# siyi-wind/MDViT

Measured on AMD Instinct MI355X. Metric: 512x512 images/sec MDViT train step (fwd+bwd, two-sweep, AdamW), higher is better.
Workload: dtype bf16x3 (fp32 storage; GEMM operands split hi+lo bf16, fp32 accumulate); 1 GPU; MDViT Sup+MLPFM train step, 4 domain(s) x bs=4 per GPU, 512x512, drop_rate=0.1 drop_path=0.1, bf16x3 GEMMs, data-parallel x1

## Files before the change

include/mdvit_hip.h:

```cpp
#ifndef MDVIT_HIP_H
#define MDVIT_HIP_H

#include <stddef.h>
#include <stdint.h>

#ifdef __cplusplus
extern "C" {
#endif

#define MDVIT_ABI_VERSION 1

enum {
    MDVIT_OK = 0,
    MDVIT_E_SHAPE = 1,
    MDVIT_E_DTYPE = 2,
    MDVIT_E_ALIGN = 3,
    MDVIT_E_WORKSPACE = 4,
    MDVIT_E_HIP = 5
};

enum { MDVIT_EPI_NONE = 0, MDVIT_EPI_GELU_DUAL = 1, MDVIT_EPI_DGELU = 2 };
enum { MDVIT_ACT_NONE = 0, MDVIT_ACT_HSWISH = 1, MDVIT_ACT_RELU = 2 };

const char* mdvit_last_error(void);
int mdvit_version(void);

int mdvit_event_create(void** out_event);
int mdvit_event_destroy(void* event);
int mdvit_event_elapsed_ms(void* start_event, void* stop_event, float* ms);
int mdvit_timing_arm(void* start_event, void* stop_event);

size_t mdvit_partials_ws_bytes(int32_t n_outputs);

typedef struct MdvitGemmDesc {
    const float* A; const float* B; float* C; float* C2;
    int64_t lda, ldb, ldc;
    int32_t M, N, K;
    int32_t trans_a, trans_b;
    const float* bias;
    int32_t epi;
    float e_drop_p; uint32_t e_key0, e_key1;
    const float* e_rowscale; int32_t e_rows_per_scale;
    const float* residual; int64_t ldr;
    const float* gelu_u; int64_t ldu;
    int32_t allow_split;
    void* ws; uint64_t ws_bytes;
    int32_t accumulate;
    float* colsum_a;
    int32_t precision;
    const uint32_t* drop_seed;
    const float* rc_a; int64_t rc_lda; const float* rc_b; int64_t rc_ldb; const float* rc_bias; int32_t rc_k;
    int32_t conv_c, conv_h, conv_w, conv_ho, conv_wo, conv_stride, conv_dilation;
    int32_t conv_up;
    int32_t a_bf16, b_bf16;
    int32_t conv_wgrad_nchw;
} MdvitGemmDesc;
size_t mdvit_gemm_ws_bytes(const MdvitGemmDesc* desc);
#define MDVIT_GEMM_MAX_GROUPS 8
int mdvit_gemm_f32_grouped(const MdvitGemmDesc* desc, int32_t G, const void* const* A, const void* const* B, void* const* C, void* stream);
int mdvit_gemm_f32_grouped_bias(const MdvitGemmDesc* desc, int32_t G, const void* const* A, const void* const* B, void* const* C, const void* const* bias, void* stream);
int mdvit_compose_bias(int32_t n, const void* const* W, int64_t ldw, const void* const* b, void* const* out, int32_t rows, int32_t cols, void* stream);
int mdvit_compose_bias_bwd(int32_t n, const void* const* W, int64_t ldw, const void* const* b, const void* const* dout, void* const* dW, int64_t lddw,
                           void* const* db, int32_t db_accumulate, int32_t rows, int32_t cols, void* stream);
int mdvit_gemm_plan(const MdvitGemmDesc* desc, int32_t* tile_m, int32_t* tile_n, int32_t* splits);
int mdvit_transpose_f32(const float* in, int64_t ld_in, float* out, int32_t rows, int32_t cols, void* stream);
int mdvit_transpose_batch(int32_t n, const void* const* in, const int64_t* ld_in, void* const* out, const int32_t* rows, const int32_t* cols, void* stream);
int mdvit_transpose_many(const void* items_dev, int32_t n, int32_t blocks_per_item, void* stream);
int mdvit_gemm_force_plan(int32_t cfg, int32_t splits);
int mdvit_gemm_kernel_name(const MdvitGemmDesc* d, char* out, int32_t cap);
int mdvit_gemm_tn_config(int32_t enable, int32_t cfg, int32_t splits);
int mdvit_gemm_tn_grid_order(int32_t mode);
int mdvit_gemm_f32(const MdvitGemmDesc* desc, void* stream);
int mdvit_conv_weight_relayout(const float* w, float* out, int32_t Cout, int32_t Cin, int32_t mode, void* stream);
int mdvit_conv_weight_relayout_many(const void* items_dev, int32_t n, int32_t blocks_per_item, void* stream);

typedef struct MdvitPlaneGemmDesc {
    const void* A; int64_t lda; int64_t a_plane; int32_t a_f32;
    const void* B; int64_t ldb; int64_t b_plane;
    int32_t planes;
    int32_t trans;
    int32_t M, N, K;
    float* C; int64_t ldc;
    void* Cp; int64_t ldcp; int64_t c_plane;
    float* U; int64_t ldu_out;
    const float* bias;
    int32_t epi;
    float e_drop_p; uint32_t e_key0, e_key1;
    const float* e_rowscale; int32_t e_rows_per_scale;
    const float* residual; int64_t ldr;
    const float* gelu_u; int64_t ldu;
    const void* rc_a; int64_t rc_lda; int64_t rc_a_plane; const void* rc_b; int64_t rc_ldb; int64_t rc_b_plane; const float* rc_bias; int32_t rc_k;
    int32_t allow_split; void* ws; uint64_t ws_bytes;
    int32_t accumulate;
    const uint32_t* drop_seed;
} MdvitPlaneGemmDesc;
size_t mdvit_gemm_planes_ws_bytes(const MdvitPlaneGemmDesc* desc);
int mdvit_gemm_planes_plan(const MdvitPlaneGemmDesc* desc, int32_t* tile_m, int32_t* tile_n, int32_t* splits);
int mdvit_gemm_planes_force_plan(int32_t cfg, int32_t splits);
int mdvit_gemm_planes(const MdvitPlaneGemmDesc* desc, void* stream);
int mdvit_gemm_ph_prefers(int32_t M, int32_t N, int32_t K, int32_t planes);
int mdvit_gemm_ph_prefers_epi(int32_t M, int32_t N, int32_t K, int32_t planes, int32_t epi_reads);
int mdvit_gemm_ph_config(int32_t mode);
int mdvit_gemm_pm_prefers(int32_t M, int32_t N, int32_t K, int32_t planes, int32_t a_f32);
int mdvit_gemm_pm_config(int32_t mode);
int mdvit_gemm_pm_splits(int32_t M, int32_t N, int32_t K, int32_t planes, int32_t a_f32);
int mdvit_split_planes(const float* in, int64_t ld_in, void* out, int64_t ld_out, int64_t plane_stride, int64_t rows, int32_t cols, int32_t planes, void* stream);
int mdvit_split_planes_t(const float* in, int64_t ld_in, void* out, int64_t ld_out, int64_t plane_stride, int32_t rows, int32_t cols, int32_t transpose,
                         int32_t planes, void* stream);
int mdvit_split_planes_many(const void* items_dev, int32_t n, int32_t blocks_per_item, int32_t planes, void* stream);

int mdvit_mlp_fwd_f32(const float* x, const float* W1, const float* b1, const float* W2, const float* b2, const float* res,
                      const float* rowscale , int32_t rows_per_scale, float* h, float* y, int32_t M, int32_t C, int32_t hidden,
                      float drop_p, uint32_t key1_0, uint32_t key1_1, uint32_t key2_0, uint32_t key2_1, const uint32_t* drop_seed, void* stream);

int mdvit_mlp_config(int32_t wide_min_tokens, int32_t ablate);

int mdvit_mlp_bwd_dgrad_f32(const float* gm, const float* x, const float* W1, const float* b1, const float* W2t, const float* W1t,
                            float* du , float* dx, int32_t M, int32_t C, int32_t hidden, float drop_p,
                            uint32_t key1_0, uint32_t key1_1, const uint32_t* drop_seed, void* stream);

int mdvit_mlp_rc_fwd(const float* x, const void* W1p, const float* b1, const void* W2p, const float* b2, const float* res,
                     const float* rowscale , int32_t rows_per_scale, float* y, int32_t M, int32_t C, int32_t hidden,
                     float drop_p, uint32_t key1_0, uint32_t key1_1, uint32_t key2_0, uint32_t key2_1, const uint32_t* drop_seed, void* stream);
int mdvit_mlp_rc_dgrad(const float* gm, const float* x, const void* W1p, const float* b1, const void* W2tp, const void* W1tp, float* dx,
                       int32_t M, int32_t C, int32_t hidden, float drop_p, uint32_t key1_0, uint32_t key1_1, const uint32_t* drop_seed, void* stream);
int mdvit_linear_rc(const float* x, int64_t lda, const void* Wp, int64_t wplane, const float* bias, float* y, int64_t ldc, int32_t M, int32_t N, int32_t K,
                    float drop_p, uint32_t key0, uint32_t key1, const float* rowscale, int32_t rows_per_scale, const float* residual, int64_t ldr,
                    const uint32_t* drop_seed, void* stream);
int mdvit_linear_rc_ln(const float* x, const float* gamma, const float* beta, int32_t groups, float eps, float* mean, float* rstd, float* ln_out,
                       const void* Wp, int64_t wplane, const float* bias, float* y, int64_t ldc, int32_t M, int32_t N, int32_t K, void* stream);
int mdvit_mlp_rc16_fwd(const float* x, const void* W1p, const float* b1, const void* W2p, const float* b2, const float* res, const float* rowscale,
                       int32_t rows_per_scale, float* h, float* y, int32_t M, int32_t C, int32_t Hd, float drop_p, uint32_t key1_0, uint32_t key1_1,
                       uint32_t key2_0, uint32_t key2_1, const uint32_t* drop_seed, void* stream);
int mdvit_mlp_rc_fwd_ln(const float* x2, const float* gamma, const float* beta, int32_t groups, float eps, float* mean, float* rstd, float* ln_out,
                        const void* W1p, const float* b1, const void* W2p, const float* b2, const float* rowscale, int32_t rows_per_scale, float* h, float* y,
                        int32_t M, int32_t C, int32_t Hd, float drop_p, uint32_t key1_0, uint32_t key1_1, uint32_t key2_0, uint32_t key2_1,
                        const uint32_t* drop_seed, void* stream);
int mdvit_mlp_rc16_dgrad(const float* gm, const float* x, const void* W1p, const float* b1, const void* W2tp, const void* W1tp, float* du, float* dx,
                         int32_t M, int32_t C, int32_t Hd, float drop_p, uint32_t key1_0, uint32_t key1_1, const uint32_t* drop_seed, void* stream);
int mdvit_mlp_rc16_fwd_hbf16(const float* x, const void* W1p, const float* b1, const void* W2p, const float* b2, const float* res, const float* rowscale,
                             int32_t rows_per_scale, float* h, float* y, int32_t M, int32_t C, int32_t Hd, float drop_p, uint32_t key1_0, uint32_t key1_1,
                             uint32_t key2_0, uint32_t key2_1, const uint32_t* drop_seed, void* stream);
int mdvit_mlp_rc_fwd_ln_hbf16(const float* x2, const float* gamma, const float* beta, int32_t groups, float eps, float* mean, float* rstd, float* ln_out,
                              const void* W1p, const float* b1, const void* W2p, const float* b2, const float* rowscale, int32_t rows_per_scale, float* h, float* y,
                              int32_t M, int32_t C, int32_t Hd, float drop_p, uint32_t key1_0, uint32_t key1_1, uint32_t key2_0, uint32_t key2_1,
                              const uint32_t* drop_seed, void* stream);
int mdvit_mlp_rc16_dgrad_hbf16(const float* gm, const float* x, const void* W1p, const float* b1, const void* W2tp, const void* W1tp, float* du, float* dx,
                               int32_t M, int32_t C, int32_t Hd, float drop_p, uint32_t key1_0, uint32_t key1_1, const uint32_t* drop_seed, void* stream);
int mdvit_mlp_rc_bwd(const float* gm, const float* x, const void* W1p, const float* b1, const void* W2tp, const void* W1tp, float* dx_parts, float* dW1, float* db1,
                     float* dW2, void* ws, size_t ws_bytes, int32_t M, int32_t C, int32_t hidden, float drop_p, uint32_t key1_0, uint32_t key1_1,
                     const uint32_t* drop_seed, int32_t accumulate, void* stream);
size_t mdvit_mlp_rc_wgrad_ws_bytes(int32_t M, int32_t C, int32_t hidden);
int mdvit_gemm_ledger(int32_t enable);
int mdvit_gemm_ledger_read(int32_t index, char* name, int32_t cap, int64_t* launches, double* flop, double* bytes);
int mdvit_gemm_sampler(const char* symbol, int32_t stride);
int mdvit_gemm_sampler_read(int32_t index, char* name, int32_t cap, int64_t* seen, int64_t* timed, double* ms);
int mdvit_mlp_rc_config(int32_t fwd_variant);
int mdvit_mlp_rc_planes(int32_t planes);
int mdvit_block_config(int32_t mlp_bwd_fused);
int mdvit_mlp_rc_wgrad(const float* gm, const float* x, const void* W1p, const float* b1, const void* W2tp, float* dW1, float* db1, float* dW2,
                       void* ws, size_t ws_bytes, int32_t M, int32_t C, int32_t hidden, float drop_p, uint32_t key1_0, uint32_t key1_1,
                       const uint32_t* drop_seed, int32_t accumulate, void* stream);

typedef struct MdvitBlockDesc {
    int32_t B, H, W, C, heads, hidden, s3, s5, s7, ln_groups, D, da_hidden, precision;
    float eps, drop_p;
    uint32_t key_proj[2], key_fc1[2], key_fc2[2];
    const uint32_t* drop_seed;
    const float* rowscale1; const float* rowscale2;
    const float* label;
    const float *cpe_w, *cpe_b, *n1_g, *n1_b, *qkv_w, *qkv_b, *w3, *b3, *w5, *b5, *w7, *b7, *da_w1, *da_b1, *da_w2, *da_b2, *proj_w, *proj_b, *n2_g, *n2_b, *fc1_w, *fc1_b,
        *fc2_w, *fc2_b;
    const float *qkv_wt, *proj_wt, *fc1_wt, *fc2_wt;
    const void *fc1_p, *fc2_p, *fc2t_p, *fc1t_p;
    const void *qkv_p, *proj_p, *projt_p, *qkvt_p;
    int32_t store_bf16;
    const float* a_pre;
    int32_t attn_kind;
} MdvitBlockDesc;
typedef struct MdvitBlockGrads {
    float *cpe_w, *cpe_b, *n1_g, *n1_b, *qkv_w, *qkv_b, *w3, *b3, *w5, *b5, *w7, *b7, *da_w1, *da_b1, *da_w2, *da_b2, *proj_w, *proj_b, *n2_g, *n2_b, *fc1_w, *fc1_b, *fc2_w,
        *fc2_b;
    int32_t accumulate, dgrad_only, aux_first;
    int32_t ln_accumulate;
    float* e_out;
} MdvitBlockGrads;
typedef struct MdvitBlockStreams {
    void* main; void* side;
    void** events; int32_t n_events; int32_t* next_event;
} MdvitBlockStreams;
size_t mdvit_block_save_bytes(const MdvitBlockDesc* d);
size_t mdvit_block_fwd_ws_bytes(const MdvitBlockDesc* d);
int mdvit_block_fwd(const MdvitBlockDesc* d, const float* x, float* y, void* save, size_t save_bytes, void* ws, size_t ws_bytes, void* stream);
size_t mdvit_block_bwd_ws_bytes(const MdvitBlockDesc* d, const MdvitBlockGrads* g, int32_t with_side_stream, size_t* side_bytes);
int mdvit_block_bwd(const MdvitBlockDesc* d, const MdvitBlockGrads* g, const MdvitBlockStreams* st, const float* x, const void* save, size_t save_bytes,
                    const float* dy, float* dx , void* ws, size_t ws_bytes, void* ws_side, size_t ws_side_bytes);

int mdvit_rowdot_fwd(const float* x, int64_t ldx, const float* w, const float* b, float* y,
                     int32_t M, int32_t K, int32_t accumulate, void* stream);
int mdvit_rowdot_bwd(const float* x, int64_t ldx, const float* w, const float* dy, float* dx, int64_t lddx,
                     float* dw, float* db, void* ws , size_t ws_bytes, int32_t M, int32_t K, void* stream);

int mdvit_colsum_f32(const float* A, int64_t lda, float* out, float* masked, void* ws , size_t ws_bytes, int32_t M, int32_t N,
                     float drop_p, uint32_t key0, uint32_t key1, const float* rowscale, int32_t rows_per_scale,
                     int32_t accumulate, const uint32_t* drop_seed, void* stream);

int mdvit_layernorm_fwd(const float* x, const float* gamma, const float* beta, float* y, float* mean, float* rstd,
                        int32_t M, int32_t C, int32_t groups, float eps, void* stream);
int mdvit_layernorm_bwd(const float* dy, const float* x, const float* gamma, const float* mean, const float* rstd,
                        const float* add, float* dx, float* dgamma, float* dbeta, void* ws , size_t ws_bytes,
                        int32_t M, int32_t C, int32_t groups, void* stream);
int mdvit_layernorm_bwd_masked(const float* dy, const float* x, const float* gamma, const float* mean, const float* rstd, const float* add, float* dx,
                               float* dx_masked, float* dgamma, float* dbeta, void* ws, size_t ws_bytes, int32_t M, int32_t C, int32_t groups,
                               float drop_p, uint32_t key0, uint32_t key1, const float* rowscale, int32_t rows_per_scale, const uint32_t* seed, void* stream);

int mdvit_dwconv3x3_fwd(const float* x, const float* w, const float* bias, float* y,
                        int32_t B, int32_t Hi, int32_t Wi, int32_t C, int32_t stride, int32_t add_input, void* stream);
int mdvit_dwconv3x3_bwd(const float* dy, const float* x, const float* w, float* dx, float* dw, float* dbias,
                        void* ws , size_t ws_bytes,
                        int32_t B, int32_t Hi, int32_t Wi, int32_t C, int32_t stride, int32_t add_input,
                        int32_t accumulate , void* stream);
int mdvit_gconv2_3x3_fwd(const float* skip, const float* up, const float* w, float* y,
                         int32_t B, int32_t H, int32_t W, int32_t C, void* stream);
int mdvit_gconv2_3x3_bwd(const float* dy, const float* skip, const float* up, const float* w,
                         float* dskip, float* dup, float* dw, void* ws , size_t ws_bytes,
                         int32_t B, int32_t H, int32_t W, int32_t C, int32_t accumulate , void* stream);
int mdvit_im2col3x3(const float* x, float* col, int32_t B, int32_t Hi, int32_t Wi, int32_t Cin, int32_t stride, int32_t dilation, void* stream);
int mdvit_col2im3x3(const float* dcol, float* dx, int32_t B, int32_t Hi, int32_t Wi, int32_t Cin, int32_t stride, int32_t dilation, void* stream);
int mdvit_dropout_f32(const float* x, float* y, int64_t n, float p, uint32_t key0, uint32_t key1, const uint32_t* drop_seed, void* stream);
int mdvit_stemconv_fwd(const float* img, const float* w, float* y, int32_t B, int32_t H, int32_t W, int32_t Cin, int32_t Cout, void* stream);
int mdvit_stemconv_wgrad(const float* img, const float* dy, float* dw, void* ws , size_t ws_bytes,
                         int32_t B, int32_t H, int32_t W, int32_t Cin, int32_t Cout, int32_t accumulate , void* stream);

size_t mdvit_bn_ws_bytes(int32_t M, int32_t C, int32_t groups);
int mdvit_bn_stats(const float* y, void* ws, size_t ws_bytes, float* mean, float* rstd, float* running_mean, float* running_var,
                   int64_t* num_batches_tracked, int32_t M, int32_t C, int32_t groups, int32_t per_group_affine, float eps,
                   float momentum, void* stream);
int mdvit_bn_eval_prep(const float* running_mean, const float* running_var, float* mean, float* rstd, int32_t C, float eps, void* stream);
int mdvit_bn_apply(const float* y, const float* mean, const float* rstd, const float* gamma, const float* beta, float* z,
                   int32_t M, int32_t C, int32_t groups, int32_t per_group_affine, int32_t act, float drop2d_p, uint32_t key0,
                   uint32_t key1, const uint32_t* drop_seed, int32_t rows_per_sample, void* stream);
int mdvit_bn_bwd(const float* dz, const float* y, const float* mean, const float* rstd, const float* gamma, const float* beta,
// ... 144 lines not shown
```

mdvit_amd/_lib.py:

```python
from __future__ import annotations

import ctypes as C
import os
import re
from typing import List

_HERE = os.path.dirname(os.path.abspath(__file__))
LIB_PATH = os.environ.get("MDVIT_HIP_LIB") or os.path.join(_HERE, "lib", "libmdvit_hip.so")
HEADER_PATH = os.path.join(_HERE, "..", "include", "mdvit_hip.h")

EPI_NONE, EPI_GELU_DUAL, EPI_DGELU = 0, 1, 2
ACT_NONE, ACT_HSWISH, ACT_RELU = 0, 1, 2

f32p = C.c_void_p
vp = C.c_void_p
i32 = C.c_int32
i64 = C.c_int64
u32 = C.c_uint32
f32 = C.c_float


class GemmDesc(C.Structure):
    _fields_ = [
        ("A", vp), ("B", vp), ("C", vp), ("C2", vp),
        ("lda", i64), ("ldb", i64), ("ldc", i64),
        ("M", i32), ("N", i32), ("K", i32),
        ("trans_a", i32), ("trans_b", i32),
        ("bias", vp),
        ("epi", i32),
        ("e_drop_p", f32), ("e_key0", u32), ("e_key1", u32),
        ("e_rowscale", vp), ("e_rows_per_scale", i32),
        ("residual", vp), ("ldr", i64),
        ("gelu_u", vp), ("ldu", i64),
        ("allow_split", i32),
        ("ws", vp), ("ws_bytes", C.c_uint64),
        ("accumulate", i32),
        ("colsum_a", vp),
        ("precision", i32),
        ("drop_seed", vp),
        ("rc_a", vp), ("rc_lda", i64), ("rc_b", vp), ("rc_ldb", i64), ("rc_bias", vp), ("rc_k", i32),
        ("conv_c", i32), ("conv_h", i32), ("conv_w", i32), ("conv_ho", i32), ("conv_wo", i32), ("conv_stride", i32), ("conv_dilation", i32),
        ("conv_up", i32),
        ("a_bf16", i32), ("b_bf16", i32), ("conv_wgrad_nchw", i32),
    ]


class PlaneGemmDesc(C.Structure):
    _fields_ = [
        ("A", vp), ("lda", i64), ("a_plane", i64), ("a_f32", i32),
        ("B", vp), ("ldb", i64), ("b_plane", i64),
        ("planes", i32), ("trans", i32),
        ("M", i32), ("N", i32), ("K", i32),
        ("C", vp), ("ldc", i64),
        ("Cp", vp), ("ldcp", i64), ("c_plane", i64),
        ("U", vp), ("ldu_out", i64),
        ("bias", vp),
        ("epi", i32),
        ("e_drop_p", f32), ("e_key0", u32), ("e_key1", u32),
        ("e_rowscale", vp), ("e_rows_per_scale", i32),
        ("residual", vp), ("ldr", i64),
        ("gelu_u", vp), ("ldu", i64),
        ("rc_a", vp), ("rc_lda", i64), ("rc_a_plane", i64), ("rc_b", vp), ("rc_ldb", i64), ("rc_b_plane", i64), ("rc_bias", vp), ("rc_k", i32),
        ("allow_split", i32), ("ws", vp), ("ws_bytes", C.c_uint64),
        ("accumulate", i32),
        ("drop_seed", vp),
    ]


class BlockDesc(C.Structure):
    _fields_ = ([(n, i32) for n in ("B", "H", "W", "C", "heads", "hidden", "s3", "s5", "s7", "ln_groups", "D", "da_hidden", "precision")]
                + [("eps", f32), ("drop_p", f32), ("key_proj", u32 * 2), ("key_fc1", u32 * 2), ("key_fc2", u32 * 2), ("drop_seed", vp),
                   ("rowscale1", vp), ("rowscale2", vp), ("label", vp)]
                + [(n, vp) for n in ("cpe_w", "cpe_b", "n1_g", "n1_b", "qkv_w", "qkv_b", "w3", "b3", "w5", "b5", "w7", "b7", "da_w1", "da_b1", "da_w2", "da_b2",
                                     "proj_w", "proj_b", "n2_g", "n2_b", "fc1_w", "fc1_b", "fc2_w", "fc2_b")]
                + [(n, vp) for n in ("qkv_wt", "proj_wt", "fc1_wt", "fc2_wt", "fc1_p", "fc2_p", "fc2t_p", "fc1t_p", "qkv_p", "proj_p", "projt_p", "qkvt_p")]
                + [("store_bf16", i32), ("a_pre", vp), ("attn_kind", i32)])


BLOCK_PARAMS = ("cpe_w", "cpe_b", "n1_g", "n1_b", "qkv_w", "qkv_b", "w3", "b3", "w5", "b5", "w7", "b7", "da_w1", "da_b1", "da_w2", "da_b2",
                "proj_w", "proj_b", "n2_g", "n2_b", "fc1_w", "fc1_b", "fc2_w", "fc2_b")


DA_MANY_MAX = 32


class DaMany(C.Structure):
    _fields_ = [("n", i32), ("hid", i32 * DA_MANY_MAX), ("C", i32 * DA_MANY_MAX), ("heads", i32 * DA_MANY_MAX), ("W1", vp * DA_MANY_MAX), ("b1", vp * DA_MANY_MAX),
                ("W2", vp * DA_MANY_MAX), ("b2", vp * DA_MANY_MAX), ("a", vp * DA_MANY_MAX)]


class DaManyGrads(C.Structure):
    _fields_ = [("e", vp * DA_MANY_MAX), ("dW1", vp * DA_MANY_MAX), ("db1", vp * DA_MANY_MAX), ("dW2", vp * DA_MANY_MAX), ("db2", vp * DA_MANY_MAX)]


class BlockGrads(C.Structure):
    _fields_ = [(n, vp) for n in BLOCK_PARAMS] + [("accumulate", i32), ("dgrad_only", i32), ("aux_first", i32), ("ln_accumulate", i32), ("e_out", vp)]


class SeAdapterDesc(C.Structure):
    _fields_ = [("kind", i32), ("B", i32), ("N", i32), ("C", i32), ("r", i32), ("W1", vp), ("b1", vp), ("W2", vp), ("b2", vp), ("Wg", vp), ("bg", vp)]


SE_DASE, SE_USE = 0, 1


class BlockStreams(C.Structure):
    _fields_ = [("main", vp), ("side", vp), ("events", C.POINTER(vp)), ("n_events", i32), ("next_event", C.POINTER(i32))]


_SIGS = {
    "mdvit_block_fwd": [C.POINTER(BlockDesc), vp, vp, vp, C.c_size_t, vp, C.c_size_t, vp],
    "mdvit_block_bwd": [C.POINTER(BlockDesc), C.POINTER(BlockGrads), C.POINTER(BlockStreams), vp, vp, C.c_size_t, vp, vp, vp, C.c_size_t, vp, C.c_size_t],
    "mdvit_gemm_planes": [C.POINTER(PlaneGemmDesc), vp],
    "mdvit_gemm_planes_plan": [C.POINTER(PlaneGemmDesc), C.POINTER(i32), C.POINTER(i32), C.POINTER(i32)],
    "mdvit_gemm_planes_force_plan": [i32, i32],
    "mdvit_gemm_ph_config": [i32],
    "mdvit_gemm_pm_config": [i32],
    "mdvit_da_fwd_many": [C.POINTER(DaMany), vp, i32, i32, vp],
    "mdvit_da_bwd_many": [C.POINTER(DaMany), C.POINTER(DaManyGrads), vp, f32, vp, C.c_size_t, i32, i32, vp],
    "mdvit_gemm_pm_prefers": [i32, i32, i32, i32, i32],
    "mdvit_gemm_pm_splits": [i32, i32, i32, i32, i32],
    "mdvit_gemm_f32_grouped": [C.POINTER(GemmDesc), i32, C.POINTER(vp), C.POINTER(vp), C.POINTER(vp), vp],
    "mdvit_gemm_f32_grouped_bias": [C.POINTER(GemmDesc), i32, C.POINTER(vp), C.POINTER(vp), C.POINTER(vp), C.POINTER(vp), vp],
    "mdvit_transpose_batch": [i32, C.POINTER(vp), C.POINTER(i64), C.POINTER(vp), C.POINTER(i32), C.POINTER(i32), vp],
    "mdvit_compose_bias": [i32, C.POINTER(vp), i64, C.POINTER(vp), C.POINTER(vp), i32, i32, vp],
    "mdvit_compose_bias_bwd": [i32, C.POINTER(vp), i64, C.POINTER(vp), C.POINTER(vp), C.POINTER(vp), i64, C.POINTER(vp), i32, i32, i32, vp],
    "mdvit_gemm_ph_prefers": [i32, i32, i32, i32],
    "mdvit_gemm_ph_prefers_epi": [i32, i32, i32, i32, i32],
    "mdvit_mlp_config": [i32, i32],
    "mdvit_mlp_rc_config": [i32],
    "mdvit_mlp_rc_planes": [i32],
    "mdvit_block_config": [i32],
    "mdvit_gemm_ledger": [i32],
    "mdvit_gemm_ledger_read": [i32, C.c_char_p, i32, C.POINTER(i64), C.POINTER(C.c_double), C.POINTER(C.c_double)],
    "mdvit_gemm_sampler": [C.c_char_p, i32],
    "mdvit_gemm_sampler_read": [i32, C.c_char_p, i32, C.POINTER(i64), C.POINTER(i64), C.POINTER(C.c_double)],
    "mdvit_mlp_rc_fwd": [vp, vp, vp, vp, vp, vp, vp, i32, vp, i32, i32, i32, f32, u32, u32, u32, u32, vp, vp],
    "mdvit_linear_rc": [vp, i64, vp, i64, vp, vp, i64, i32, i32, i32, f32, u32, u32, vp, i32, vp, i64, vp, vp],
    "mdvit_linear_rc_ln": [vp, vp, vp, i32, f32, vp, vp, vp, vp, i64, vp, vp, i64, i32, i32, i32, vp],
    "mdvit_mlp_rc_fwd_ln": [vp, vp, vp, i32, f32, vp, vp, vp, vp, vp, vp, vp, vp, i32, vp, vp, i32, i32, i32, f32, u32, u32, u32, u32, vp, vp],
    "mdvit_mlp_rc16_fwd": [vp, vp, vp, vp, vp, vp, vp, i32, vp, vp, i32, i32, i32, f32, u32, u32, u32, u32, vp, vp],
    "mdvit_mlp_rc_dgrad": [vp, vp, vp, vp, vp, vp, vp, i32, i32, i32, f32, u32, u32, vp, vp],
    "mdvit_mlp_rc16_dgrad": [vp, vp, vp, vp, vp, vp, vp, vp, i32, i32, i32, f32, u32, u32, vp, vp],
    "mdvit_mlp_rc_fwd_ln_hbf16": [vp, vp, vp, i32, f32, vp, vp, vp, vp, vp, vp, vp, vp, i32, vp, vp, i32, i32, i32, f32, u32, u32, u32, u32, vp, vp],
    "mdvit_mlp_rc16_fwd_hbf16": [vp, vp, vp, vp, vp, vp, vp, i32, vp, vp, i32, i32, i32, f32, u32, u32, u32, u32, vp, vp],
    "mdvit_mlp_rc16_dgrad_hbf16": [vp, vp, vp, vp, vp, vp, vp, vp, i32, i32, i32, f32, u32, u32, vp, vp],
    "mdvit_mlp_rc_wgrad": [vp, vp, vp, vp, vp, vp, vp, vp, vp, C.c_size_t, i32, i32, i32, f32, u32, u32, vp, i32, vp],
    "mdvit_mlp_rc_bwd": [vp, vp, vp, vp, vp, vp, vp, vp, vp, vp, vp, C.c_size_t, i32, i32, i32, f32, u32, u32, vp, i32, vp],
    "mdvit_imgconv_fwd": [vp, vp, vp, i32, i32, i32, i32, i32, i32, vp],
    "mdvit_imgconv_wgrad": [vp, vp, vp, vp, C.c_size_t, i32, i32, i32, i32, i32, i32, i32, vp],
    "mdvit_maxpool3x3s2_fwd": [vp, vp, vp, i32, i32, i32, i32, vp],
    "mdvit_maxpool3x3s2_bwd": [vp, vp, vp, i32, i32, i32, i32, vp],
    "mdvit_resize_ac_fwd": [vp, vp, i32, i32, i32, i32, i32, i32, vp],
    "mdvit_resize_ac_bwd": [vp, vp, i32, i32, i32, i32, i32, i32, vp],
    "mdvit_ew": [vp, vp, vp, i64, i32, vp],
    "mdvit_add3": [vp, vp, vp, vp, i64, vp],
    "mdvit_add_parts": [vp, vp, C.POINTER(vp), i32, i64, vp, vp],
    "mdvit_add_bcast": [vp, vp, vp, i32, i64, vp],
    "mdvit_sum_batch": [vp, vp, i32, i64, vp],
    "mdvit_gate_fwd": [vp, vp, vp, i32, i64, i32, i32, vp],
    "mdvit_gate_bwd": [vp, vp, vp, vp, vp, vp, C.c_size_t, i32, i64, i32, i32, vp],
    "mdvit_imgconv_im2col": [vp, vp, i32, i32, i32, i32, i32, i32, vp],
    "mdvit_chanpool_fwd": [vp, vp, vp, i64, i32, vp],
    "mdvit_chanpool_bwd": [vp, vp, vp, i64, i32, vp],
    "mdvit_conv7x7_2to1_fwd": [vp, vp, vp, i32, i32, i32, vp],
    "mdvit_conv7x7_2to1_bwd": [vp, vp, vp, vp, vp, i32, i32, i32, vp],
    "mdvit_bn1_fwd": [vp, vp, vp, vp, vp, vp, vp, vp, i64, i32, i32, f32, f32, vp],
    "mdvit_bn1_bwd": [vp, vp, vp, vp, vp, vp, i64, i32, i32, vp],
    "mdvit_subsample2": [vp, vp, i32, i32, i32, i32, i32, vp],
    "mdvit_patchify": [vp, vp, i32, i32, i32, i32, i32, vp],
    "mdvit_dropout2d": [vp, vp, i32, i64, i32, f32, u32, u32, vp, vp],
    "mdvit_sdpa_fwd": [vp, vp, vp, vp, i32, i32, i32, i32, vp],
    "mdvit_sdpa_bwd": [vp, vp, vp, vp, vp, vp, vp, vp, i32, i32, i32, i32, vp],
    "mdvit_sdpa_mfma_fwd": [vp, vp, vp, vp, i32, i32, i32, i32, vp],
    "mdvit_sdpa_mfma_bwd": [vp, vp, vp, vp, vp, vp, vp, vp, i32, i32, i32, i32, vp],
    "mdvit_structure_weight": [vp, vp, vp, i32, i32, i32, vp],
    "mdvit_structure_loss_fwd": [vp, vp, vp, vp, vp, i32, i64, vp],
    "mdvit_structure_loss_bwd": [vp, vp, vp, vp, vp, vp, i32, i64, vp],
    "mdvit_split_planes": [vp, i64, vp, i64, i64, i64, i32, i32, vp],
    "mdvit_split_planes_many": [vp, i32, i32, i32, vp],
    "mdvit_split_planes_t": [vp, i64, vp, i64, i64, i32, i32, i32, i32, vp],
    "mdvit_event_create": [C.POINTER(vp)],
    "mdvit_event_destroy": [vp],
    "mdvit_event_elapsed_ms": [vp, vp, C.POINTER(f32)],
    "mdvit_timing_arm": [vp, vp],
    "mdvit_gemm_f32": [C.POINTER(GemmDesc), vp],
    "mdvit_gemm_plan": [C.POINTER(GemmDesc), C.POINTER(i32), C.POINTER(i32), C.POINTER(i32)],
    "mdvit_gemm_force_plan": [i32, i32],
    "mdvit_conv_weight_relayout": [vp, vp, i32, i32, i32, vp],
    "mdvit_conv_weight_relayout_many": [vp, i32, i32, vp],
    "mdvit_gemm_kernel_name": [vp, C.c_char_p, i32],
    "mdvit_gemm_tn_config": [i32, i32, i32],
    "mdvit_gemm_tn_grid_order": [i32],
    "mdvit_transpose_f32": [vp, i64, vp, i32, i32, vp],
    "mdvit_mlp_bwd_dgrad_f32": [vp, vp, vp, vp, vp, vp, vp, vp, i32, i32, i32, f32, u32, u32, vp, vp],
    "mdvit_mlp_fwd_f32": [vp, vp, vp, vp, vp, vp, vp, i32, vp, vp, i32, i32, i32, f32, u32, u32, u32, u32, vp, vp],
    "mdvit_transpose_many": [vp, i32, i32, vp],
    "mdvit_rowdot_fwd": [vp, i64, vp, vp, vp, i32, i32, i32, vp],
    "mdvit_rowdot_bwd": [vp, i64, vp, vp, vp, i64, vp, vp, vp, C.c_size_t, i32, i32, vp],
    "mdvit_colsum_f32": [vp, i64, vp, vp, vp, C.c_size_t, i32, i32, f32, u32, u32, vp, i32, i32, vp, vp],
    "mdvit_layernorm_fwd": [vp, vp, vp, vp, vp, vp, i32, i32, i32, f32, vp],
    "mdvit_layernorm_bwd": [vp, vp, vp, vp, vp, vp, vp, vp, vp, vp, C.c_size_t, i32, i32, i32, vp],
    "mdvit_layernorm_bwd_masked": [vp, vp, vp, vp, vp, vp, vp, vp, vp, vp, vp, C.c_size_t, i32, i32, i32, f32, u32, u32, vp, i32, vp, vp],
    "mdvit_dwconv3x3_fwd": [vp, vp, vp, vp, i32, i32, i32, i32, i32, i32, vp],
    "mdvit_dwconv3x3_bwd": [vp, vp, vp, vp, vp, vp, vp, C.c_size_t, i32, i32, i32, i32, i32, i32, i32, vp],
    "mdvit_gconv2_3x3_fwd": [vp, vp, vp, vp, i32, i32, i32, i32, vp],
    "mdvit_gconv2_3x3_bwd": [vp, vp, vp, vp, vp, vp, vp, vp, C.c_size_t, i32, i32, i32, i32, i32, vp],
    "mdvit_im2col3x3": [vp, vp, i32, i32, i32, i32, i32, i32, vp],
    "mdvit_col2im3x3": [vp, vp, i32, i32, i32, i32, i32, i32, vp],
    "mdvit_dropout_f32": [vp, vp, i64, f32, u32, u32, vp, vp],
    "mdvit_stemconv_fwd": [vp, vp, vp, i32, i32, i32, i32, i32, vp],
    "mdvit_stemconv_wgrad": [vp, vp, vp, vp, C.c_size_t, i32, i32, i32, i32, i32, i32, vp],
    "mdvit_bn_rowdot_fwd": [vp, vp, vp, vp, vp, vp, vp, vp, i32, i32, i32, f32, u32, u32, vp, i32, vp],
    "mdvit_bn_rowdot_bwd": [vp, vp, vp, vp, vp, vp, vp, vp, vp, vp, vp, vp, vp, C.c_size_t, i32, i32, i32, i32, f32, u32, u32, vp, i32, vp],
    "mdvit_bn_stats": [vp, vp, C.c_size_t, vp, vp, vp, vp, vp, i32, i32, i32, i32, f32, f32, vp],
# ... 13 lines not shown
    "mdvit_seg_losses_fwd": [vp, vp, vp, vp, vp, i64, vp],
    "mdvit_adamw_step": [vp, i32, i32, vp, vp, f32, f32, f32, f32, i32, vp],
    "mdvit_seg_metrics": [vp, vp, vp, vp, vp, i64, vp],
    "mdvit_eval_accumulate": [vp, vp, vp, C.POINTER(i32), C.POINTER(i32), i32, i64, i32, vp, vp, vp, vp, C.c_size_t, vp],
    "mdvit_eval_table": [vp, i32, vp, vp],
    "mdvit_image_normalize_u8": [vp, vp, i32, i32, i32, vp],
    "mdvit_augment_normalize_u8": [vp, vp, vp, vp, vp, vp, i32, i32, i32, vp],
    "mdvit_augment_probe_taps": [f32, f32, i32, i32, C.POINTER(i32), C.POINTER(f32)],
    "mdvit_seg_losses_sums": [vp, vp, vp, vp, i64, vp],
    "mdvit_seg_losses_final": [vp, vp, i64, i32, vp],
    "mdvit_seg_losses_bwd": [vp, vp, vp, vp, vp, vp, vp, i64, f32, vp],
    "mdvit_seg_losses_bwd3": [vp, vp, vp, vp, vp, vp, vp, vp, vp, i64, f32, vp],
    "mdvit_seg_losses_groups_sums": [vp, vp, vp, vp, i64, i32, vp],
    "mdvit_seg_losses_groups_final": [vp, vp, vp, i64, i32, i32, vp],
    "mdvit_seg_losses_groups_bwd": [vp, vp, vp, vp, vp, vp, vp, vp, vp, i64, i32, f32, vp],
    "mdvit_se_adapter_fwd": [C.POINTER(SeAdapterDesc), vp, vp, vp, vp, C.c_size_t, vp],
    "mdvit_se_adapter_bwd": [C.POINTER(SeAdapterDesc)] + [vp] * 10 + [vp, C.c_size_t, vp],
}

_lib = None


class MdvitHipError(RuntimeError):
    pass


def declared_symbols() -> List[str]:
    with open(HEADER_PATH) as f:
        text = f.read()
    text = re.sub(r"/\*.*?\*/", "", text, flags=re.S)
    return sorted(set(re.findall(r"\b(mdvit_[a-z0-9_]+)\s*\(", text)))


_on_load = []


def on_load(fn):
    if _lib is not None:
        fn(_lib)
    else:
        _on_load.append(fn)


def load():
    global _lib
    if _lib is not None:
        return _lib
    if not os.path.exists(LIB_PATH):
        raise MdvitHipError(
            f"{LIB_PATH} is missing: build it with `python -m mdvit_amd.build` (hipcc, gfx950). "
            "mdvit_amd has no CPU or PyTorch fallback.")
    lib = C.CDLL(LIB_PATH)
    try:
        _attach_prototypes(lib)
    except AttributeError as e:
        raise MdvitHipError(f"{LIB_PATH} is stale ({e}): rebuild it with `python -m mdvit_amd.build`.") from None
    _lib = lib
    while _on_load:
        _on_load.pop(0)(lib)
    return lib


def _attach_prototypes(lib):
    lib.mdvit_last_error.restype = C.c_char_p
    lib.mdvit_last_error.argtypes = []
    lib.mdvit_version.restype = C.c_int
    lib.mdvit_version.argtypes = []
    lib.mdvit_factoratt_ws_bytes.restype = C.c_size_t
    lib.mdvit_factoratt_ws_bytes.argtypes = [i32, i32, i32, i32]
    lib.mdvit_gemm_ws_bytes.restype = C.c_size_t
    lib.mdvit_gemm_ws_bytes.argtypes = [C.POINTER(GemmDesc)]
    lib.mdvit_gate_bwd_ws_bytes.restype = C.c_size_t
    lib.mdvit_gate_bwd_ws_bytes.argtypes = [i32, i64, i32, i32]
    lib.mdvit_gemm_planes_ws_bytes.restype = C.c_size_t
    lib.mdvit_gemm_planes_ws_bytes.argtypes = [C.POINTER(PlaneGemmDesc)]
    lib.mdvit_bn_rowdot_ws_bytes.restype = C.c_size_t
    lib.mdvit_bn_rowdot_ws_bytes.argtypes = [i32, i32]
    lib.mdvit_bn_ws_bytes.restype = C.c_size_t
    lib.mdvit_bn_ws_bytes.argtypes = [i32, i32, i32]
    lib.mdvit_upsample_multi_bwd_ws_bytes.restype = C.c_size_t
    lib.mdvit_upsample_multi_bwd_ws_bytes.argtypes = [vp, i32, i32, i32, i32]
    lib.mdvit_upsample_bwd_ws_bytes.restype = C.c_size_t
    lib.mdvit_upsample_bwd_ws_bytes.argtypes = [i32] * 6
    lib.mdvit_partials_ws_bytes.restype = C.c_size_t
    lib.mdvit_partials_ws_bytes.argtypes = [i32]
    lib.mdvit_mlp_rc_wgrad_ws_bytes.restype = C.c_size_t
    lib.mdvit_mlp_rc_wgrad_ws_bytes.argtypes = [i32, i32, i32]
    lib.mdvit_block_save_bytes.restype = C.c_size_t
    lib.mdvit_block_save_bytes.argtypes = [C.POINTER(BlockDesc)]
    lib.mdvit_block_fwd_ws_bytes.restype = C.c_size_t
    lib.mdvit_block_fwd_ws_bytes.argtypes = [C.POINTER(BlockDesc)]
    lib.mdvit_block_bwd_ws_bytes.restype = C.c_size_t
    lib.mdvit_block_bwd_ws_bytes.argtypes = [C.POINTER(BlockDesc), C.POINTER(BlockGrads), i32, C.POINTER(C.c_size_t)]
    lib.mdvit_da_ws_bytes.restype = C.c_size_t
    lib.mdvit_da_ws_bytes.argtypes = [i32, i32, i32]
    lib.mdvit_da_many_ws_bytes.restype = C.c_size_t
    lib.mdvit_da_many_ws_bytes.argtypes = [C.POINTER(DaMany), i32]
    lib.mdvit_se_adapter_save_bytes.restype = C.c_size_t
    lib.mdvit_se_adapter_save_bytes.argtypes = [C.POINTER(SeAdapterDesc)]
    lib.mdvit_se_adapter_ws_bytes.restype = C.c_size_t
    lib.mdvit_se_adapter_ws_bytes.argtypes = [C.POINTER(SeAdapterDesc)]
    lib.mdvit_eval_ws_bytes.restype = C.c_size_t
    lib.mdvit_eval_ws_bytes.argtypes = [i32]
    for name, sig in _SIGS.items():
        try:
            fn = getattr(lib, name)
        except AttributeError:
            raise MdvitHipError(f"{LIB_PATH} is stale: it does not export `{name}` (built from an earlier tree). "
                                "Rebuild it with `python -m mdvit_amd.build`.") from None
        fn.restype = C.c_int
        fn.argtypes = sig


def check(code: int, what: str):
    if code != 0:
        msg = load().mdvit_last_error().decode(errors="replace")
        raise MdvitHipError(f"{what} failed (code {code}): {msg}")


def call(name: str, *args):
    lib = load()
    check(getattr(lib, name)(*args), name)
```

mdvit_amd/blocks.py:

```python
from __future__ import annotations

import math
from typing import Optional, Tuple

import torch
from torch import nn

from . import ops
from ._lib import ACT_HSWISH, ACT_NONE, ACT_RELU


class ConvParams(nn.Module):
    def __init__(self, out_ch, in_per_group, kh, kw, bias=True, groups=1):
        super().__init__()
        self.weight = nn.Parameter(torch.empty(out_ch, in_per_group, kh, kw))
        self.bias = nn.Parameter(torch.empty(out_ch)) if bias else None
        self.kernel_size, self.out_channels, self.groups = (kh, kw), out_ch, groups

    def forward(self, *a, **k):
        raise RuntimeError("ConvParams only holds parameters; compute goes through mdvit_amd.ops (HIP)")


class LinearParams(nn.Module):
    def __init__(self, in_f, out_f, bias=True):
# ... 148 lines not shown
            y = ops.conv3x3_dense(x, self.conv.weight, None, self.stride)
        return _pick(self, "bn", "bns")(y)


class DWConv2d_BN(nn.Module):

    def __init__(self, in_ch, out_ch, kernel_size=3, stride=1, norm_layer=nn.BatchNorm2d, act_layer=nn.Hardswish, dsn=0):
        super().__init__()
        _check_norm(norm_layer)
        assert kernel_size == 3
        self.dwconv = ConvParams(in_ch, 1, 3, 3, bias=False, groups=in_ch)
        self.pwconv = ConvParams(out_ch, in_ch, 1, 1, bias=False)
        if dsn:
            self.bns = _bank(lambda: BatchNormAct(out_ch, ACT_HSWISH), dsn)
        else:
            self.bn = BatchNormAct(out_ch, ACT_HSWISH)
        self.stride = stride

    def forward(self, x):
        t = ops.dwconv3x3(x, self.dwconv.weight, None, self.stride, False)
        return _pick(self, "bn", "bns")(ops.linear(t, self.pwconv.weight))


class DWCPatchEmbed(nn.Module):

    def __init__(self, in_chans=3, embed_dim=768, patch_size=16, stride=1, conv_norm=nn.BatchNorm2d, act_layer=nn.Hardswish, dsn=0):
        super().__init__()
        self.patch_conv = DWConv2d_BN(in_chans, embed_dim, kernel_size=patch_size, stride=stride, norm_layer=conv_norm, act_layer=act_layer,
                                      dsn=dsn)

    def forward(self, x):
        return self.patch_conv(x)


class DecoderDWConv2d_BN(nn.Module):

    def __init__(self, in_ch, out_ch, norm_layer=nn.BatchNorm2d, dsn=0):
        super().__init__()
        _check_norm(norm_layer)
        assert in_ch == 2 * out_ch
        self.dwconv = ConvParams(out_ch, 2, 3, 3, bias=False, groups=out_ch)
        self.pwconv = ConvParams(out_ch, out_ch, 1, 1, bias=False)
        if dsn:
            self.bns = _bank(lambda: BatchNormAct(out_ch, ACT_HSWISH), dsn)
        else:
            self.bn = BatchNormAct(out_ch, ACT_HSWISH)

    def forward(self, skip, up):
        t = ops.gconv2_3x3(skip, up, self.dwconv.weight)
        return _pick(self, "bn", "bns")(ops.linear(t, self.pwconv.weight))


class ConvPosEnc(nn.Module):

    def __init__(self, dim, k=3):
        super().__init__()
        assert k == 3
        self.proj = ConvParams(dim, 1, 3, 3, bias=True, groups=dim)

    def forward(self, x, size: Tuple[int, int]):
        B, N, Cn = x.shape
        H, W = size
        return ops.dwconv3x3(x.view(B, H, W, Cn), self.proj.weight, self.proj.bias, 1, True).view(B, N, Cn)


class ConvRelPosEnc(nn.Module):

    def __init__(self, Ch, h, window):
        super().__init__()
        if isinstance(window, int):
            window = {window: h}
        if sorted(window) != [3, 5, 7] or sum(window.values()) != h:
            raise NotImplementedError("the HIP attention kernel is built for the reference's {3:2, 5:3, 7:3}-style windows")
        self.window = dict(window)
        self.head_splits = [window[3], window[5], window[7]]
        self.conv_list = nn.ModuleList([ConvParams(window[k] * Ch, 1, k, k, bias=True, groups=window[k] * Ch) for k in (3, 5, 7)])

    def params(self):
        c = self.conv_list
        return (c[0].weight, c[0].bias, c[1].weight, c[1].bias, c[2].weight, c[2].bias)


class _FactorAttBase(nn.Module):
    def _attend(self, x, size, domain_label, da_params, res, rowscale):
        B, N, Cn = x.shape
        H, W = size
        qkv = ops.linear(x, self.qkv.weight, self.qkv.bias)
        y = ops.factor_att(qkv, self.crpe.params(), H, W, self.num_heads, self.crpe.head_splits, domain_label, da_params,
                           aux_first=getattr(self, "aux_first", False))
        return ops.linear(y, self.proj.weight, self.proj.bias, residual=res, rowscale=rowscale,
                          drop_p=self.proj_drop_p if self.training else 0.0, rows_per_scale=N)


class FactorAtt_ConvRelPosEnc(_FactorAttBase):

    def __init__(self, dim, num_heads=8, qkv_bias=False, qk_scale=None, attn_drop=0.0, proj_drop=0.0, shared_crpe=None):
        super().__init__()
        if qk_scale is not None:
            raise NotImplementedError("qk_scale override is not built")
        self.num_heads = num_heads
        self.qkv = LinearParams(dim, dim * 3, bias=qkv_bias)
        self.proj = LinearParams(dim, dim)
        self.proj_drop_p = proj_drop
        self.crpe = shared_crpe

    def forward(self, x, size, _res=None, _rowscale=None):
        return self._attend(x, size, None, None, _res, _rowscale)


class FactorAtt_ConvRelPosEnc_Sup(_FactorAttBase):

    def __init__(self, seq_length, dim, num_heads=8, qkv_bias=False, qk_scale=None, attn_drop=0.0, proj_drop=0.0,
                 shared_crpe=None, r=2, num_domains=4):
        super().__init__()
        if qk_scale is not None:
            raise NotImplementedError("qk_scale override is not built")
        self.num_heads = num_heads
        hidden = max(dim // r, 4)
        self.qkv = LinearParams(dim, dim * 3, bias=qkv_bias)
        self.proj = LinearParams(dim, dim)
        self.proj_drop_p = proj_drop
        self.domain_layer = nn.Sequential(LinearParams(num_domains, hidden), _NoParams(), LinearParams(hidden, dim))
        self.crpe = shared_crpe

    def forward(self, x, size, domain_label, _res=None, _rowscale=None):
        d0, d2 = self.domain_layer[0], self.domain_layer[2]
        return self._attend(x, size, domain_label, (d0.weight, d0.bias, d2.weight, d2.bias), _res, _rowscale)


class Mlp(nn.Module):

    def __init__(self, in_features, hidden_features=None, out_features=None, act_layer=nn.GELU, drop=0.0):
        super().__init__()
        out_features = out_features or in_features
        hidden_features = hidden_features or in_features
        assert out_features == in_features and act_layer is nn.GELU
        self.fc1 = LinearParams(in_features, hidden_features)
        self.fc2 = LinearParams(hidden_features, out_features)
        self.drop_p = drop

    def forward(self, x, _res=None, _rowscale=None):
        N = x.shape[1]
        res = _res if _res is not None else torch.zeros_like(x)
        return ops.mlp_residual(x, res, self.fc1.weight, self.fc1.bias, self.fc2.weight, self.fc2.bias, _rowscale,
                                self.drop_p if self.training else 0.0, N)


_droppath_pool = None


class droppath_pool:

    def __init__(self, n_blocks, B, keep, device, enabled=True):
        self.args = (n_blocks, B, keep, device, enabled)

    def __enter__(self):
        global _droppath_pool
        n, B, keep, device, enabled = self.args
        self.prev = _droppath_pool
        if enabled and keep < 1.0:
            m = ops.droppath_scales((n, 2, B), keep, device) if torch.device(device).type == "cuda" else (torch.rand((n, 2, B), device=device) < keep).float() / keep
            _droppath_pool = {"m": m, "keep": keep, "B": B, "next": 0}
        return self

    def __exit__(self, *exc):
        global _droppath_pool
        _droppath_pool = self.prev
        return False


class SerialBlock_adapt(nn.Module):

    def __init__(self, seq_length, dim, num_heads, mlp_ratio=4.0, qkv_bias=False, qk_scale=None, drop=0.0, attn_drop=0.0,
                 drop_path=0.0, act_layer=nn.GELU, norm_layer=None, shared_cpe=None, shared_crpe=None, adapt_method=None,
                 num_domains=4, base_semantics=False, dsn=0):
        super().__init__()
        self.cpe = shared_cpe
        if dsn:
            self.norm1s = _bank(lambda: LayerNormParams(dim, 1e-6), dsn)
        else:
            self.norm1 = LayerNormParams(dim, 1e-6)
        self.adapt_method = adapt_method
        self.base_semantics = base_semantics
        if adapt_method == "Sup":
            self.factoratt_crpe = FactorAtt_ConvRelPosEnc_Sup(seq_length, dim, num_heads=num_heads, qkv_bias=qkv_bias, qk_scale=qk_scale,
                                                              attn_drop=attn_drop, proj_drop=drop, shared_crpe=shared_crpe, num_domains=num_domains)
        else:
            self.factoratt_crpe = FactorAtt_ConvRelPosEnc(dim, num_heads=num_heads, qkv_bias=qkv_bias, qk_scale=qk_scale,
                                                          attn_drop=attn_drop, proj_drop=drop, shared_crpe=shared_crpe)
        self.drop_path_p = drop_path
        if dsn:
            self.norm2s = _bank(lambda: LayerNormParams(dim, 1e-6), dsn)
        else:
            self.norm2 = LayerNormParams(dim, 1e-6)
        self.mlp = Mlp(in_features=dim, hidden_features=int(dim * mlp_ratio), act_layer=act_layer, drop=drop)

    def _droppath_scales(self, B, device):
        if not self.training or self.drop_path_p <= 0.0:
            return None, None
        keep = 1.0 - self.drop_path_p
        pool = _droppath_pool
        if pool is not None and pool["keep"] == keep and pool["B"] == B and pool["next"] < pool["m"].shape[0]:
            m = pool["m"][pool["next"]]
            pool["next"] += 1
            return m[0], m[1]
        m = ops.droppath_scales((2, B), keep, device)
        return m[0], m[1]

    def _block_entry(self, x, size, domain_label, use_da):
        att, mlp = self.factoratt_crpe, self.mlp
        if not x.is_cuda or att.proj_drop_p != mlp.drop_p or att.qkv.bias is None:
            return None
        if not torch.is_grad_enabled():
            return None
        n1, n2 = _pick(self, "norm1", "norm1s"), _pick(self, "norm2", "norm2s")
        if isinstance(n1, _BankLN):
            (g1, b1), (g2, b2) = n1._params(), n2._params()
            groups, eps = g1.shape[0], n1.mods[0].eps
        else:
            g1, b1, g2, b2, groups, eps = n1.weight, n1.bias, n2.weight, n2.bias, 1, n1.eps
        da = [None] * 4
        if use_da:
            d0, d2 = att.domain_layer[0], att.domain_layer[2]
            da = [d0.weight, d0.bias, d2.weight, d2.bias]
        params = [self.cpe.proj.weight, self.cpe.proj.bias, g1, b1, att.qkv.weight, att.qkv.bias, *att.crpe.params(), *da, att.proj.weight, att.proj.bias,
                  g2, b2, mlp.fc1.weight, mlp.fc1.bias, mlp.fc2.weight, mlp.fc2.bias]
        if not ops.block_entry_ok(x.shape[-1], mlp.fc1.weight.shape[0], params):
            return None
        s1, s2 = self._droppath_scales(x.shape[0], x.device)
        meta = (int(size[0]), int(size[1]), att.num_heads, tuple(att.crpe.head_splits), float(eps), float(mlp.drop_p if self.training else 0.0), int(groups),
                bool(getattr(att, "aux_first", False)))
        return ops.serial_block(x, domain_label if use_da else None, s1, s2, meta, params)

    def forward(self, x, size: Tuple[int, int], domain_label=None):
        use_da = (domain_label is not None) if self.base_semantics else (self.adapt_method is not None and domain_label is not None)
        if use_da and not isinstance(self.factoratt_crpe, FactorAtt_ConvRelPosEnc_Sup):
            raise TypeError("forward() got a domain_label but this block was built without adapt_method='Sup' "
                            "(the reference raises here too: mdvit.py:350-351)")
        if not use_da and isinstance(self.factoratt_crpe, FactorAtt_ConvRelPosEnc_Sup):
            raise TypeError("adapt_method='Sup' blocks need a domain_label (mdvit.py:281)")
        y = self._block_entry(x, size, domain_label, use_da)
        if y is not None:
            return y
        x = self.cpe(x, size)
        s1, s2 = self._droppath_scales(x.shape[0], x.device)
        cur, x = _pick(self, "norm1", "norm1s").fork(x)
        if use_da:
            x = self.factoratt_crpe(cur, size, domain_label, _res=x, _rowscale=s1)
        else:
            x = self.factoratt_crpe(cur, size, _res=x, _rowscale=s1)
        cur, x = _pick(self, "norm2", "norm2s").fork(x)
        return self.mlp(cur, _res=x, _rowscale=s2)


class MHSA_stage_adapt(nn.Module):

    def __init__(self, seq_length, dim, num_layers, num_heads, mlp_ratio, qkv_bias=True, qk_scale=None, drop_rate=0.0,
                 attn_drop_rate=0.0, drop_path_rate=0.0, num_domains=4, norm_layer=None, adapt_method=None,
                 crpe_window={3: 2, 5: 3, 7: 3}, base_semantics=False, dsn=0):
        super().__init__()
        self.cpe = ConvPosEnc(dim, k=3)
        self.crpe = ConvRelPosEnc(Ch=dim // num_heads, h=num_heads, window=crpe_window)
        self.mhca_blks = nn.ModuleList([
            SerialBlock_adapt(seq_length, dim, num_heads, mlp_ratio, qkv_bias, qk_scale, drop_rate, attn_drop_rate, drop_path_rate,
                              nn.GELU, norm_layer, self.cpe, self.crpe, adapt_method, num_domains, base_semantics, dsn)
            for _ in range(num_layers)])

    def forward(self, input, H, W, domain_label=None):
        for blk in self.mhca_blks:
            input = blk(input, (H, W), domain_label)
        return input


def init_weights_(module: nn.Module):
    for m in module.modules():
        if isinstance(m, LinearParams):
            nn.init.trunc_normal_(m.weight, std=0.02)
            if m.bias is not None:
                nn.init.zeros_(m.bias)
        elif isinstance(m, LayerNormParams):
            nn.init.ones_(m.weight); nn.init.zeros_(m.bias)
        elif isinstance(m, ConvParams):
            out_ch, in_pg, kh, kw = m.weight.shape
            fan_out = kh * kw * out_ch // m.groups
            nn.init.normal_(m.weight, 0.0, math.sqrt(2.0 / fan_out))
            if m.bias is not None:
                nn.init.zeros_(m.bias)
        elif isinstance(m, BatchNormAct):
            nn.init.ones_(m.weight); nn.init.zeros_(m.bias)
```

mdvit_amd/csrc/block.hip:

```cpp
#include <stdlib.h>
#include "common.h"

namespace {

struct Arena {
    char* base; size_t off, cap; bool dry;
    float* take(size_t floats) {
        const size_t bytes = (floats * sizeof(float) + 255) & ~(size_t)255;
        float* p = dry ? nullptr : reinterpret_cast<float*>(base + off);
        off += bytes;
        return p;
    }
    void* take_bytes(size_t bytes) { return take((bytes + 3) / 4); }
};

enum { MLP_RC = 0, MLP_RECOMP = 1, MLP_STORED = 2 };

inline int mlp_mode(const MdvitBlockDesc& d) {
    if (d.precision == 1 && d.C == 64 && d.hidden % 256 == 0 && d.hidden <= 4096 && d.fc1_p && d.fc2_p && (long)d.B * d.H * d.W * d.hidden < (1L << 32)) return MLP_RC;
    if (d.precision >= 1 && d.C <= 128 && d.C % 32 == 0 && d.hidden % 4 == 0) return MLP_RECOMP;
    return MLP_STORED;
}
inline bool mlp_rc16(const MdvitBlockDesc& d) {
    return mlp_mode(d) == MLP_RECOMP && d.precision == 1 && d.C == 128 && d.hidden % 32 == 0 && d.hidden <= 4096 && d.fc1_p && d.fc2_p && d.fc1_b && d.fc2_b &&
           (long)d.B * d.H * d.W * d.hidden < (1L << 32);
}

inline bool hbf16(const MdvitBlockDesc& d) { return d.store_bf16 && mlp_rc16(d); }

struct Saved {
    float *x1, *mean1, *rstd1, *cur1, *qkv, *a, *att, *U, *kmax, *ksum, *Mmat, *x2, *mean2, *rstd2, *cur2, *h, *u, *lse;
};

inline bool sdpa_kind(const MdvitBlockDesc& d) { return d.attn_kind == 1; }

void layout_saved(const MdvitBlockDesc& d, Arena& A, Saved& s) {
    const long T = (long)d.B * d.H * d.W, C = d.C, Ch = d.C / d.heads;
    const int mode = mlp_mode(d);
    s.lse = nullptr;
    s.x1 = sdpa_kind(d) ? nullptr : A.take(T * C);
    s.mean1 = A.take(T); s.rstd1 = A.take(T); s.cur1 = A.take(T * C);
    s.qkv = A.take(T * 3 * C);
    s.a = d.label ? A.take((long)d.B * C) : nullptr;
    if (d.label && d.a_pre) s.a = const_cast<float*>(d.a_pre);
    s.att = A.take(T * C);
    if (sdpa_kind(d)) { s.U = s.kmax = s.ksum = s.Mmat = nullptr; s.lse = A.take((long)d.B * d.heads * d.H * d.W); }
    else {
    s.U = A.take(T * C);
    s.kmax = A.take((long)d.B * C); s.ksum = A.take((long)d.B * C); s.Mmat = A.take((long)d.B * C * Ch);
    }
    s.x2 = A.take(T * C); s.mean2 = A.take(T); s.rstd2 = A.take(T); s.cur2 = A.take(T * C);
    s.h = mode != MLP_RC ? A.take(hbf16(d) ? (T * d.hidden + 1) / 2 : T * d.hidden) : nullptr;
    s.u = mode == MLP_STORED ? A.take(T * d.hidden) : nullptr;
}

void gemm_init(MdvitGemmDesc& g, const MdvitBlockDesc& d) {
    memset(&g, 0, sizeof(g));
    g.precision = d.precision >= 1 ? 1 : 0;
    g.drop_seed = nullptr;
}

static int g_blk_mlp_bwd = 1;
extern "C" int mdvit_block_config(int32_t mlp_bwd_fused) {
    if (mlp_bwd_fused < 0 || mlp_bwd_fused > 2) return mdvit_set_error(MDVIT_E_SHAPE, "block_config: mlp_bwd_fused in 0..2");
    g_blk_mlp_bwd = mlp_bwd_fused;
    return MDVIT_OK;
}

#define BLK_RUN(call)                         \
    do {                                      \
        if (!A.dry) {                         \
            const int rc__ = (call);          \
            if (rc__ != MDVIT_OK) return rc__; \
        }                                     \
    } while (0)

bool ph_takes(const MdvitBlockDesc& d, const void* planes, int M, int N, int K, int epi_reads) {
    return d.precision == 1 && planes != nullptr && (mdvit_gemm_ph_prefers_epi(M, N, K, 2, epi_reads) != 0 || mdvit_gemm_pm_prefers(M, N, K, 2, 1) != 0);
}
int epi_reads_of(const MdvitGemmDesc& g) { return g.gelu_u != nullptr || g.residual != nullptr || g.accumulate != 0; }
bool pm_split_takes(const MdvitBlockDesc& d, const MdvitGemmDesc& g, const void* planes, int M, int N, int K) {
    return d.precision == 1 && planes != nullptr && g.allow_split && g.epi == MDVIT_EPI_NONE && !epi_reads_of(g) && !(g.e_drop_p > 0.f) && !g.e_rowscale && !g.rc_a &&
           mdvit_gemm_pm_splits(M, N, K, 2, 1) > 1;
}
int gemm_planes_nt(Arena& A, const MdvitGemmDesc& g, const void* planes, hipStream_t s, bool k_splits = false) {
    MdvitPlaneGemmDesc pd;
    memset(&pd, 0, sizeof(pd));
    pd.A = g.A; pd.lda = g.lda; pd.a_f32 = 1;
    pd.B = planes; pd.ldb = g.K; pd.b_plane = (int64_t)g.N * g.K;
    pd.planes = 2; pd.M = g.M; pd.N = g.N; pd.K = g.K;
    if (g.epi == MDVIT_EPI_GELU_DUAL && g.C2) { pd.U = g.C; pd.ldu_out = g.ldc; pd.C = g.C2; pd.ldc = g.ldc; }
    else { pd.C = g.C; pd.ldc = g.ldc; }
    pd.bias = g.bias; pd.epi = g.epi;
    pd.e_drop_p = g.e_drop_p; pd.e_key0 = g.e_key0; pd.e_key1 = g.e_key1; pd.e_rowscale = g.e_rowscale; pd.e_rows_per_scale = g.e_rows_per_scale;
    pd.residual = g.residual; pd.ldr = g.ldr; pd.gelu_u = g.gelu_u; pd.ldu = g.ldu;
    pd.drop_seed = g.drop_seed;
    pd.allow_split = k_splits ? 1 : 0;
    const size_t need = pd.allow_split ? mdvit_gemm_planes_ws_bytes(&pd) : 0;
    pd.ws = need ? A.take_bytes(need) : nullptr; pd.ws_bytes = need;
    BLK_RUN(mdvit_gemm_planes(&pd, s));
    return MDVIT_OK;
}

int gemm_fwd(Arena& A, MdvitGemmDesc& g, hipStream_t s, const MdvitBlockDesc* d = nullptr, const void* planes = nullptr) {
    if (d && ph_takes(*d, planes, g.M, g.N, g.K, epi_reads_of(g))) return gemm_planes_nt(A, g, planes, s);
    g.trans_a = 0; g.trans_b = 1; g.allow_split = 1;
    const size_t need = mdvit_gemm_ws_bytes(&g);
    g.ws = need ? A.take_bytes(need) : nullptr; g.ws_bytes = need;
    BLK_RUN(mdvit_gemm_f32(&g, s));
    return MDVIT_OK;
}

int gemm_dgrad(Arena& A, const MdvitBlockDesc& d, MdvitGemmDesc& g, const float* gy, const float* W, const float* Wt, float* dx, int M, int K, int N, hipStream_t s,
               const void* planes_t = nullptr) {
    g.A = gy; g.C = dx; g.M = M; g.N = K; g.K = N; g.lda = N; g.ldc = K;
    if (ph_takes(d, planes_t, M, K, N, epi_reads_of(g)) && !g.rc_a) return gemm_planes_nt(A, g, planes_t, s);
    if (pm_split_takes(d, g, planes_t, M, K, N)) return gemm_planes_nt(A, g, planes_t, s, true);
    if (d.precision >= 1) { g.B = Wt; g.ldb = N; g.trans_a = 0; g.trans_b = 1; g.precision = 1; }
    else { g.B = W; g.ldb = K; g.trans_a = 0; g.trans_b = 0; g.precision = 0; }
    const size_t need = g.allow_split ? mdvit_gemm_ws_bytes(&g) : 0;
    g.ws = need ? A.take_bytes(need) : nullptr; g.ws_bytes = need;
    BLK_RUN(mdvit_gemm_f32(&g, s));
    return MDVIT_OK;
}

int gemm_wgrad(Arena& A, const MdvitBlockDesc& d, const float* gy, const float* x, float* dW, float* db, int M, int N, int K, int accumulate, hipStream_t s,
               int gy_bf16 = 0, int x_bf16 = 0) {
    MdvitGemmDesc g;
    gemm_init(g, d);
    g.a_bf16 = gy_bf16; g.b_bf16 = x_bf16;
    g.A = gy; g.B = x; g.C = dW; g.M = N; g.N = K; g.K = M; g.lda = N; g.ldb = K; g.ldc = K;
    g.trans_a = 1; g.trans_b = 0; g.allow_split = 1; g.accumulate = accumulate; g.colsum_a = db;
    const size_t need = mdvit_gemm_ws_bytes(&g);
    g.ws = need ? A.take_bytes(need) : nullptr; g.ws_bytes = need;
    BLK_RUN(mdvit_gemm_f32(&g, s));
    return MDVIT_OK;
}

int fork_side(const MdvitBlockDesc& d, const MdvitBlockStreams& st, hipStream_t& side) {
    side = (hipStream_t)st.side;
    if (side == nullptr || side == (hipStream_t)st.main) { side = (hipStream_t)st.main; return MDVIT_OK; }
    if (st.n_events <= 0 || st.events == nullptr) return mdvit_set_error(MDVIT_E_SHAPE, "block: a side stream needs events");
    const int ei = *st.next_event;
    *st.next_event = (ei + 1) % st.n_events;
    hipEvent_t ev = (hipEvent_t)st.events[(ei % st.n_events + st.n_events) % st.n_events];
    hipError_t e = hipEventRecord(ev, (hipStream_t)st.main);
    if (e == hipSuccess) e = hipStreamWaitEvent(side, ev, 0);
    if (e != hipSuccess) return mdvit_set_error(MDVIT_E_HIP, "block: side-stream fork failed: %s", hipGetErrorString(e));
    return MDVIT_OK;
// ... 183 lines not shown
    }
    const bool masked1 = d.drop_p > 0.f || d.rowscale1 != nullptr;
    float* dx2 = masked1 ? A.take(T * C) : S.take(T * C);
    float* gm1 = masked1 ? S.take(T * C) : dx2;
    {
        const bool lnw = want_w || !fast_ln;
        const size_t pb = lnw ? mdvit_partials_ws_bytes(2 * C) : 0;
        void* pw = lnw ? A.take_bytes(pb) : nullptr;
        float* dg = want_w ? G.n2_g : (lnw ? A.take((long)d.ln_groups * C) : nullptr);
        float* db = want_w ? G.n2_b : (lnw ? A.take((long)d.ln_groups * C) : nullptr);
        if (!A.dry) mdvit_layernorm_bwd_next_dy2(dcur2_b);
        if (defer) {
            void* pws = S.take_bytes(pb);
            int nb = 0;
            BLK_RUN(mdvit_layernorm_bwd_parts(dcur2, sv.x2, d.n2_g, sv.mean2, sv.rstd2, dy, dx2, masked1 ? gm1 : nullptr, pws, pb, M, C, d.ln_groups, d.drop_p, d.key_proj[0],
                                              d.key_proj[1], d.rowscale1, N_tok, seed, s, &nb));
            late[n_late++] = Late{(const float*)pws, d.ln_groups, nb, C, dg, C, db};
        } else if (masked1 && fast_ln) {
            BLK_RUN(mdvit_layernorm_bwd_masked(dcur2, sv.x2, d.n2_g, sv.mean2, sv.rstd2, dy, dx2, gm1, dg, db, pw, pb, M, C, d.ln_groups, d.drop_p, d.key_proj[0],
                                               d.key_proj[1], d.rowscale1, N_tok, seed, s));
        } else {
            BLK_RUN(mdvit_layernorm_bwd(dcur2, sv.x2, d.n2_g, sv.mean2, sv.rstd2, dy, dx2, dg, db, pw, pb, M, C, d.ln_groups, s));
            if (masked1) BLK_RUN(mdvit_colsum_f32(dx2, C, nullptr, gm1, nullptr, 0, M, C, d.drop_p, d.key_proj[0], d.key_proj[1], d.rowscale1, N_tok, 0, seed, s));
        }
    }
    float* datt = tmp;
    {
        MdvitGemmDesc g;
        gemm_init(g, d);
        g.allow_split = 1;
        int rc = MDVIT_OK;
        if (d.precision == 1 && (C == 64 || C == 128) && d.projt_p && M >= 1024) {
            BLK_RUN(mdvit_linear_rc(gm1, C, d.projt_p, (long)C * C, nullptr, datt, C, M, C, C, 0.f, 0, 0, nullptr, 1, nullptr, 0, nullptr, s));
        } else {
            rc = gemm_dgrad(A, d, g, gm1, d.proj_w, d.proj_wt, datt, M, C, C, s, d.projt_p);
            if (rc != MDVIT_OK) return rc;
        }
        if (want_w) {
            if (!A.dry) { rc = fork_side(d, st, side); if (rc != MDVIT_OK) return rc; }
            rc = gemm_wgrad(S, d, gm1, sv.att, G.proj_w, G.proj_b, M, C, C, acc, side);
            if (rc != MDVIT_OK) return rc;
        }
    }
    float* e = !d.label ? nullptr : G.e_out ? G.e_out : A.take((long)B * C);
    float* dqkv = nullptr;
    if (sdpa_kind(d)) {
        dqkv = S.take(T * 3 * C);
        float* delta = A.take(2L * B * d.heads * N_tok);
        BLK_RUN(mdvit_sdpa_mfma_bwd(tmp, sv.qkv, sv.lse, sv.att, sv.a, dqkv, e, delta, B, N_tok, C, d.heads, s));
    } else {
    const size_t fab = mdvit_factoratt_ws_bytes(B, N_tok, C, d.heads);
    void* faws = S.take_bytes(fab);
    if (dgrad_only && G.aux_first && d.label) {
        BLK_RUN(mdvit_factoratt_bwd(datt, sv.qkv, sv.att, sv.U, d.w3, d.b3, d.w5, d.b5, d.w7, d.b7, sv.a, sv.kmax, sv.ksum, sv.Mmat, nullptr, e, nullptr, nullptr, nullptr,
                                    nullptr, nullptr, nullptr, faws, fab, B, H, W, C, d.heads, d.s3, d.s5, d.s7, s));
        if (!G.e_out) {
            const size_t dab = mdvit_da_ws_bytes(B, d.da_hidden, C);
            void* daws = A.take_bytes(dab);
            BLK_RUN(mdvit_da_bwd(d.label, d.da_w1, d.da_b1, d.da_w2, d.da_b2, sv.a, e, -1.0f, G.da_w1, G.da_b1, G.da_w2, G.da_b2, daws, dab, B, d.D, d.da_hidden, C, d.heads, s));
        }
        return MDVIT_OK;
    }
    dqkv = S.take(T * 3 * C);
    {
        const bool deferred = want_w && acc && have_side;
        const bool inl = want_w && !deferred;
        BLK_RUN(mdvit_factoratt_bwd(datt, sv.qkv, sv.att, sv.U, d.w3, d.b3, d.w5, d.b5, d.w7, d.b7, sv.a, sv.kmax, sv.ksum, sv.Mmat, dqkv, e, inl ? G.w3 : nullptr,
                                    inl ? G.b3 : nullptr, inl ? G.w5 : nullptr, inl ? G.b5 : nullptr, inl ? G.w7 : nullptr, inl ? G.b7 : nullptr, faws, fab, B, H, W, C,
                                    d.heads, d.s3, d.s5, d.s7, s));
        if (deferred) {
            if (!A.dry) { const int rc = fork_side(d, st, side); if (rc != MDVIT_OK) return rc; }
            BLK_RUN(mdvit_factoratt_wgrad(sv.qkv, faws, fab, G.w3, G.b3, G.w5, G.b5, G.w7, G.b7, B, H, W, C, d.heads, d.s3, d.s5, d.s7, 1, side));
        }
        if (inl && acc) return mdvit_set_error(MDVIT_E_SHAPE, "block_bwd: accumulating window-weight gradients need the side stream");
    }
    }
    if (d.label && !G.e_out) {
        const size_t dab = mdvit_da_ws_bytes(B, d.da_hidden, C);
        void* daws = A.take_bytes(dab);
        BLK_RUN(mdvit_da_bwd(d.label, d.da_w1, d.da_b1, d.da_w2, d.da_b2, sv.a, e, dgrad_only ? -1.0f : 1.0f, G.da_w1, G.da_b1, G.da_w2, G.da_b2, daws, dab, B, d.D,
                             d.da_hidden, C, d.heads, s));
    }
    float* dcur1 = tmp;
    {
        MdvitGemmDesc g;
        gemm_init(g, d);
        g.allow_split = 1;
        int rc = gemm_dgrad(A, d, g, dqkv, d.qkv_w, d.qkv_wt, dcur1, M, C, 3 * C, s, d.qkvt_p);
        if (rc != MDVIT_OK) return rc;
        if (want_w) {
            if (!A.dry) { rc = fork_side(d, st, side); if (rc != MDVIT_OK) return rc; }
            rc = gemm_wgrad(S, d, dqkv, sv.cur1, G.qkv_w, G.qkv_b, M, 3 * C, C, acc, side);
            if (rc != MDVIT_OK) return rc;
        }
    }
    float* dx1 = (sdpa_kind(d) && dx) ? dx : S.take(T * C);
    {
        const bool lnw = want_w || !fast_ln;
        const size_t pb = lnw ? mdvit_partials_ws_bytes(2 * C) : 0;
        void* pw = lnw ? A.take_bytes(pb) : nullptr;
        float* dg = want_w ? G.n1_g : (lnw ? A.take((long)d.ln_groups * C) : nullptr);
        float* db = want_w ? G.n1_b : (lnw ? A.take((long)d.ln_groups * C) : nullptr);
        if (defer) {
            void* pws = S.take_bytes(pb);
            int nb = 0;
            BLK_RUN(mdvit_layernorm_bwd_parts(dcur1, sv.x1, d.n1_g, sv.mean1, sv.rstd1, dx2, dx1, nullptr, pws, pb, M, C, d.ln_groups, 0.f, 0, 0, nullptr, 1, nullptr, s, &nb));
            late[n_late++] = Late{(const float*)pws, d.ln_groups, nb, C, dg, C, db};
        } else {
            BLK_RUN(mdvit_layernorm_bwd(dcur1, sv.x1, d.n1_g, sv.mean1, sv.rstd1, dx2, dx1, dg, db, pw, pb, M, C, d.ln_groups, s));
        }
    }
    if (n_late > 0 && !A.dry) {
        const int rcf = fork_side(d, st, side);
        if (rcf != MDVIT_OK) return rcf;
        for (int i = 0; i < n_late; ++i) {
            const Late& L = late[i];
            const int rc = mdvit_reduce_partials_batched2_acc(L.part, L.batches, L.nblk, L.n0, L.out0, L.n1, L.out1, 1, side);
            if (rc != MDVIT_OK) return rc;
        }
    }
    if (sdpa_kind(d)) return MDVIT_OK;
    if (dx) BLK_RUN(mdvit_dwconv3x3_bwd(dx1, x, d.cpe_w, dx, nullptr, nullptr, nullptr, 0, B, H, W, C, 1, 1, 0, s));
    if (want_w) {
        const size_t pb = mdvit_partials_ws_bytes(10 * C);
        void* pw = S.take_bytes(pb);
        if (acc && !A.dry) { const int rc = fork_side(d, st, side); if (rc != MDVIT_OK) return rc; }
        BLK_RUN(mdvit_dwconv3x3_bwd(dx1, x, d.cpe_w, nullptr, G.cpe_w, G.cpe_b, pw, pb, B, H, W, C, 1, 1, acc, acc ? side : s));
    }
    return MDVIT_OK;
}

int check_desc(const MdvitBlockDesc& d, const char* what) {
    MDVIT_CHECK_ARG(d.B > 0 && d.H > 0 && d.W > 0 && d.C > 0 && d.heads > 0 && d.C % d.heads == 0 && d.hidden > 0 && d.C % 4 == 0, MDVIT_E_SHAPE,
                    "%s: bad geometry B=%d H=%d W=%d C=%d heads=%d hidden=%d", what, d.B, d.H, d.W, d.C, d.heads, d.hidden);
    MDVIT_CHECK_ARG(d.precision == 0 || d.precision == 1, MDVIT_E_SHAPE, "%s: precision %d (0: fp32, 1: bf16x3)", what, d.precision);
    MDVIT_CHECK_ARG(d.ln_groups >= 1 && ((long)d.B * d.H * d.W) % d.ln_groups == 0, MDVIT_E_SHAPE, "%s: %d LayerNorm groups do not divide the rows", what, d.ln_groups);
    MDVIT_CHECK_ARG(d.attn_kind == 0 || d.attn_kind == 1, MDVIT_E_SHAPE, "%s: attn_kind %d (0: SerialBlock_adapt, 1: the DeiT Block_adapt)", what, d.attn_kind);
    if (d.attn_kind == 1)
        MDVIT_CHECK_ARG(d.H * d.W == 256 && d.heads <= 6 && d.C == 64 * d.heads && d.drop_p == 0.f && !d.rowscale1 && !d.rowscale2 && !d.store_bf16, MDVIT_E_SHAPE,
                        "%s: attn_kind 1 is built for 256 tokens, head dimension 64, <= 6 heads, no dropout (H=%d W=%d C=%d heads=%d)", what, d.H, d.W, d.C, d.heads);
    MDVIT_CHECK_ARG((d.attn_kind == 1 || (d.cpe_w && d.cpe_b && d.w3 && d.b3 && d.w5 && d.b5 && d.w7 && d.b7)) && d.n1_g && d.n1_b && d.qkv_w && d.proj_w && d.proj_b && d.n2_g &&
                        d.n2_b && d.fc1_w && d.fc1_b && d.fc2_w && d.fc2_b, MDVIT_E_SHAPE, "%s: null parameter", what);
    MDVIT_CHECK_ARG(!d.label || (d.da_w1 && d.da_b1 && d.da_w2 && d.da_b2 && d.D > 0 && d.da_hidden > 0), MDVIT_E_SHAPE, "%s: a domain label needs the adapter's parameters", what);
    return MDVIT_OK;
}

}

extern "C" size_t mdvit_block_save_bytes(const MdvitBlockDesc* d) {
    if (!d || check_desc(*d, "block_save_bytes") != MDVIT_OK) return 0;
    Arena SV{nullptr, 0, 0, true};
    Saved sv;
    layout_saved(*d, SV, sv);
    return SV.off;
}

extern "C" size_t mdvit_block_fwd_ws_bytes(const MdvitBlockDesc* d) {
    if (!d || check_desc(*d, "block_fwd_ws_bytes") != MDVIT_OK) return 0;
    Arena SV{nullptr, 0, 0, true}, A{nullptr, 0, 0, true};
    if (block_fwd(*d, nullptr, nullptr, SV, A, nullptr) != MDVIT_OK) return 0;
    return A.off + 256;
}

extern "C" int mdvit_block_fwd(const MdvitBlockDesc* d, const float* x, float* y, void* save, size_t save_bytes, void* ws, size_t ws_bytes, void* stream) {
    MDVIT_CHECK_ARG(d && x && y && save, MDVIT_E_SHAPE, "block_fwd: null argument");
    const int rc = check_desc(*d, "block_fwd");
    if (rc != MDVIT_OK) return rc;
    MDVIT_CHECK_ARG(aligned16(x) && aligned16(y) && (reinterpret_cast<uintptr_t>(save) & 255) == 0 && (!ws || (reinterpret_cast<uintptr_t>(ws) & 255) == 0), MDVIT_E_ALIGN,
                    "block_fwd: x / y must be 16-byte, save / ws 256-byte aligned");
    MDVIT_CHECK_ARG(save_bytes >= mdvit_block_save_bytes(d), MDVIT_E_WORKSPACE, "block_fwd: save buffer too small: need %zu bytes (mdvit_block_save_bytes), got %zu",
                    mdvit_block_save_bytes(d), save_bytes);
    const size_t need = mdvit_block_fwd_ws_bytes(d);
    MDVIT_CHECK_ARG(ws_bytes >= need && ws, MDVIT_E_WORKSPACE, "block_fwd: workspace too small: need %zu bytes (mdvit_block_fwd_ws_bytes), got %zu", need, ws_bytes);
    Arena SV{(char*)save, 0, save_bytes, false}, A{(char*)ws, 0, ws_bytes, false};
    return block_fwd(*d, x, y, SV, A, (hipStream_t)stream);
}

extern "C" size_t mdvit_block_bwd_ws_bytes(const MdvitBlockDesc* d, const MdvitBlockGrads* g, int32_t with_side_stream, size_t* side_bytes) {
    if (side_bytes) *side_bytes = 0;
    if (!d || !g || check_desc(*d, "block_bwd_ws_bytes") != MDVIT_OK) return 0;
    Arena SV{nullptr, 0, 0, true}, A{nullptr, 0, 0, true}, S{nullptr, 0, 0, true};
    MdvitBlockStreams st;
    memset(&st, 0, sizeof(st));
    st.main = (void*)1; st.side = with_side_stream ? (void*)2 : (void*)1;
    float dummy = 0.f;
    if (block_bwd(*d, *g, st, nullptr, &dummy, &dummy, SV, A, S) != MDVIT_OK) return 0;
    if (side_bytes) *side_bytes = S.off + 256;
    return A.off + 256;
}

extern "C" int mdvit_block_bwd(const MdvitBlockDesc* d, const MdvitBlockGrads* g, const MdvitBlockStreams* st, const float* x, const void* save, size_t save_bytes,
                               const float* dy, float* dx, void* ws, size_t ws_bytes, void* ws_side, size_t ws_side_bytes) {
    MDVIT_CHECK_ARG(d && g && st && x && save && dy && ws && ws_side, MDVIT_E_SHAPE, "block_bwd: null argument");
    mdvit_layernorm_bwd_next_dy2(nullptr);
    const int rc = check_desc(*d, "block_bwd");
    if (rc != MDVIT_OK) return rc;
    MDVIT_CHECK_ARG(aligned16(x) && aligned16(dy) && (!dx || aligned16(dx)) && (reinterpret_cast<uintptr_t>(save) & 255) == 0 && (reinterpret_cast<uintptr_t>(ws) & 255) == 0 &&
                        (reinterpret_cast<uintptr_t>(ws_side) & 255) == 0, MDVIT_E_ALIGN, "block_bwd: x / dy / dx must be 16-byte, save / ws 256-byte aligned");
    MDVIT_CHECK_ARG(save_bytes >= mdvit_block_save_bytes(d), MDVIT_E_WORKSPACE, "block_bwd: save buffer too small");
    size_t need_side = 0;
    const size_t need = mdvit_block_bwd_ws_bytes(d, g, st->side != nullptr && st->side != st->main, &need_side);
    MDVIT_CHECK_ARG(ws_bytes >= need && ws_side_bytes >= need_side, MDVIT_E_WORKSPACE,
                    "block_bwd: workspace too small: need %zu + %zu bytes (mdvit_block_bwd_ws_bytes), got %zu + %zu", need, need_side, ws_bytes, ws_side_bytes);
    if (!g->dgrad_only) {
        MDVIT_CHECK_ARG((d->attn_kind == 1 || (g->cpe_w && g->cpe_b && g->w3 && g->b3 && g->w5 && g->b5 && g->w7 && g->b7)) && g->n1_g && g->n1_b && g->qkv_w && g->proj_w &&
                            g->proj_b && g->n2_g && g->n2_b && g->fc1_w && g->fc1_b && g->fc2_w && g->fc2_b && (!d->qkv_b || g->qkv_b), MDVIT_E_SHAPE,
                        "block_bwd: null gradient output");
    }
    MDVIT_CHECK_ARG(!d->label || g->e_out || (g->da_w1 && g->da_b1 && g->da_w2 && g->da_b2), MDVIT_E_SHAPE, "block_bwd: the adapter's gradient outputs are missing");
    MDVIT_CHECK_ARG(d->precision == 0 || (d->qkv_wt && d->proj_wt && (mlp_mode(*d) == MLP_RC || (mlp_rc16(*d) && d->fc2t_p && d->fc1t_p) || (d->fc1_wt && d->fc2_wt))), MDVIT_E_SHAPE,
                    "block_bwd: the bf16x3 data-gradient GEMMs need the transposed weights");
    Arena SV{(char*)const_cast<void*>(save), 0, save_bytes, false}, A{(char*)ws, 0, ws_bytes, false}, S{(char*)ws_side, 0, ws_side_bytes, false};
    return block_bwd(*d, *g, *st, x, dy, dx, SV, A, S);
}
```

mdvit_amd/csrc/gemm.hip:

```cpp
#include "common.h"
#include <type_traits>
#ifndef MDVIT_NO_DB
#define MDVIT_NO_DB 0
#endif

typedef float f32x16 __attribute__((ext_vector_type(16)));
typedef __bf16 bf16x8_t __attribute__((ext_vector_type(8)));
typedef __bf16 bf16x2_t __attribute__((ext_vector_type(2)));
typedef float f32x2_t __attribute__((ext_vector_type(2)));

struct GemmGroups { int n; const float* A[MDVIT_GEMM_MAX_GROUPS]; const float* B[MDVIT_GEMM_MAX_GROUPS]; float* C[MDVIT_GEMM_MAX_GROUPS]; const float* bias[MDVIT_GEMM_MAX_GROUPS]; };
static thread_local GemmGroups g_groups = {0, {}, {}, {}, {}};
const GemmGroups* mdvit_gemm_groups_active() { return g_groups.n > 0 ? &g_groups : nullptr; }

namespace {

constexpr int BK = 32;
constexpr int NTHREADS = 256;

struct GemmArgs {
    const float* A; const float* B; float* C; float* C2;
    long lda, ldb, ldc;
    int M, N, K;
    const float* bias;
    int epi;
    int e_drop; uint32_t e_k0, e_k1, e_thresh; float e_inv_keep;
    const float* e_rowscale; int e_rows_per_scale;
    const float* residual; long ldr;
    const float* gelu_u; long ldu;
    const float* rc_a; long rc_lda; const float* rc_b; long rc_ldb; const float* rc_bias; int rc_k;
    int splits; int k_per_split;
    float* slab;
    int accumulate;
    float* colsum;
    int vec;
    const uint32_t* seed;
    int tiles_m, tiles_n;
    int conv_c, conv_h, conv_w, conv_ho, conv_wo, conv_stride, conv_dil, conv_up, conv_phase;
    int ngroups; const float* gA[MDVIT_GEMM_MAX_GROUPS]; const float* gB[MDVIT_GEMM_MAX_GROUPS]; float* gC[MDVIT_GEMM_MAX_GROUPS]; const float* gBias[MDVIT_GEMM_MAX_GROUPS];
};



__device__ __forceinline__ int xcd_remap(int bid, int nwg) {
    const int q = nwg >> 3, r = nwg & 7, xcd = bid & 7, idx = bid >> 3;
    return (xcd < r ? xcd * (q + 1) : r * (q + 1) + (xcd - r) * q) + idx;
}

enum { EPI_PLAIN = 0, EPI_GELU2 = 1, EPI_DGELU = 2, EPI_FULL = 3, EPI_DGELU_RC = 4 };

__device__ __forceinline__ void split_bf16x3(const float4 x, uint2& hi, uint2& lo) {
    f32x2_t a = {x.x, x.y}, b = {x.z, x.w};
    const bf16x2_t ha = __builtin_convertvector(a, bf16x2_t), hb = __builtin_convertvector(b, bf16x2_t);
    const uint32_t hau = __builtin_bit_cast(uint32_t, ha), hbu = __builtin_bit_cast(uint32_t, hb);
    f32x2_t la = {x.x - __uint_as_float(hau << 16), x.y - __uint_as_float(hau & 0xffff0000u)};
    f32x2_t lb = {x.z - __uint_as_float(hbu << 16), x.w - __uint_as_float(hbu & 0xffff0000u)};
    const bf16x2_t lab = __builtin_convertvector(la, bf16x2_t), lbb = __builtin_convertvector(lb, bf16x2_t);
    hi = make_uint2(hau, hbu);
    lo = make_uint2(__builtin_bit_cast(uint32_t, lab), __builtin_bit_cast(uint32_t, lbb));
}

__device__ __forceinline__ void split_pair_bf16x3(float x0, float x1, uint32_t& hi, uint32_t& lo) {
    f32x2_t a = {x0, x1};
    const uint32_t h = __builtin_bit_cast(uint32_t, __builtin_convertvector(a, bf16x2_t));
    f32x2_t l = {x0 - __uint_as_float(h << 16), x1 - __uint_as_float(h & 0xffff0000u)};
    hi = h;
    lo = __builtin_bit_cast(uint32_t, __builtin_convertvector(l, bf16x2_t));
}

template <int BM, int BN, int WAVES_M, int WAVES_N, bool TA, bool TB, int EPI, bool BF3>
__global__ __launch_bounds__(NTHREADS) __attribute__((amdgpu_waves_per_eu((BM == 256 && TA) ? 2 : 3, 8))) void gemm_f32_kernel(GemmArgs p) {
    constexpr bool CONV = false;
#include "gemm_body.inc"
}

template <int BM, int BN, int WAVES_M, int WAVES_N>
__global__ __launch_bounds__(NTHREADS) __attribute__((amdgpu_waves_per_eu(3, 8))) void gemm_conv3x3_kernel(GemmArgs p) {
    constexpr bool CONV = true, TA = false, TB = true, BF3 = true;
    constexpr int EPI = EPI_PLAIN;
#include "gemm_body.inc"
}

template <int R>
__global__ __launch_bounds__(256) void gemm_splitk_reduce_kernel(const float* __restrict__ slab, const float* __restrict__ bias,
                                                                 float* __restrict__ C, long ldc, int M, int N, int splits, int accumulate, int perm_cin) {
    const int NQ = N >> 2;
    const long total = (long)M * NQ, MN = (long)M * N;
    const int r = threadIdx.x % R;
    const long stride = (long)gridDim.x * blockDim.x / R;
    for (long e = ((long)blockIdx.x * blockDim.x + threadIdx.x) / R; e < total; e += stride) {
        const long m = e / NQ;
        const int n = (int)(e % NQ) * 4;
        float4 acc = make_float4(0.f, 0.f, 0.f, 0.f);
        const float* src = slab + m * N + n;
        for (int sidx = r; sidx < splits; sidx += R) {
            const float4 v = *reinterpret_cast<const float4*>(src + (long)sidx * MN);
            acc.x += v.x; acc.y += v.y; acc.z += v.z; acc.w += v.w;
        }
#pragma unroll
        for (int off = R / 2; off > 0; off >>= 1) {
            acc.x += __shfl_down(acc.x, off, R); acc.y += __shfl_down(acc.y, off, R);
            acc.z += __shfl_down(acc.z, off, R); acc.w += __shfl_down(acc.w, off, R);
        }
        if (r == 0) {
            if (bias) { acc.x += bias[n]; acc.y += bias[n + 1]; acc.z += bias[n + 2]; acc.w += bias[n + 3]; }
            if (perm_cin > 0) {
                const float a4[4] = {acc.x, acc.y, acc.z, acc.w};
#pragma unroll
                for (int j = 0; j < 4; ++j) {
                    const int nn = n + j, tap = nn / perm_cin, ci = nn - tap * perm_cin;
                    float* d1 = C + m * ldc + (long)ci * 9 + tap;
                    *d1 = accumulate ? *d1 + a4[j] : a4[j];
                }
                continue;
            }
            float* dst = C + m * ldc + n;
            if (accumulate) { acc.x += dst[0]; acc.y += dst[1]; acc.z += dst[2]; acc.w += dst[3]; }
            if (((ldc & 3) == 0) && ((reinterpret_cast<uintptr_t>(C) & 15) == 0)) *reinterpret_cast<float4*>(dst) = acc;
            else { dst[0] = acc.x; dst[1] = acc.y; dst[2] = acc.z; dst[3] = acc.w; }
        }
    }
}

template <int BM, int BN, int WM, int WN>
int launch_cfg(const GemmArgs& a, int ta, int tb, int epi, int bf3, hipStream_t s) {
    dim3 grid(a.tiles_m * a.tiles_n, a.splits, a.ngroups > 0 ? a.ngroups : 1), block(NTHREADS);
#define MDVIT_GEMM_LAUNCH(TA_, TB_, EPI_, BF3_) \
    MDVIT_TIMED_LAUNCH((gemm_f32_kernel<BM, BN, WM, WN, TA_, TB_, EPI_, BF3_>), grid, block, 0, s, a)
    if (a.conv_c > 0) {
        if (ta || !tb || !bf3 || epi != EPI_PLAIN) return 1;
        MDVIT_TIMED_LAUNCH((gemm_conv3x3_kernel<BM, BN, WM, WN>), grid, block, 0, s, a);
        return 0;
    }
    if (!ta && tb) {
        if (bf3) {
            if (epi == EPI_GELU2) MDVIT_GEMM_LAUNCH(false, true, EPI_GELU2, true);
            else if (epi == EPI_DGELU) MDVIT_GEMM_LAUNCH(false, true, EPI_DGELU, true);
            else if (epi == EPI_DGELU_RC) { if (BM == 64 && BN == 64) MDVIT_GEMM_LAUNCH(false, true, (BM == 64 && BN == 64 ? EPI_DGELU_RC : EPI_DGELU), true); else return 1; }
            else if (epi == EPI_FULL) MDVIT_GEMM_LAUNCH(false, true, EPI_FULL, true);
            else if (epi == EPI_PLAIN) MDVIT_GEMM_LAUNCH(false, true, EPI_PLAIN, true);
            else return 1;
        } else {
            if (epi == EPI_GELU2) MDVIT_GEMM_LAUNCH(false, true, EPI_GELU2, false);
            else if (epi == EPI_DGELU_RC) { if (BM == 64 && BN == 64) MDVIT_GEMM_LAUNCH(false, true, (BM == 64 && BN == 64 ? EPI_DGELU_RC : EPI_GELU2), false); else return 1; }
            else if (epi == EPI_FULL) MDVIT_GEMM_LAUNCH(false, true, EPI_FULL, false);
            else if (epi == EPI_PLAIN) MDVIT_GEMM_LAUNCH(false, true, EPI_PLAIN, false);
            else return 1;
        }
    } else if (bf3) {
        if (ta && !tb && epi == EPI_PLAIN) MDVIT_GEMM_LAUNCH(true, false, EPI_PLAIN, true);
        else return 1;
    } else if (!ta && !tb) {
        if (epi == EPI_DGELU) MDVIT_GEMM_LAUNCH(false, false, EPI_DGELU, false);
        else if (epi == EPI_PLAIN) MDVIT_GEMM_LAUNCH(false, false, EPI_PLAIN, false);
        else if (epi == EPI_FULL) MDVIT_GEMM_LAUNCH(false, false, EPI_FULL, false);
        else return 1;
    } else if (ta && !tb) {
        if (epi != EPI_PLAIN) return 1;
        MDVIT_GEMM_LAUNCH(true, false, EPI_PLAIN, false);
    } else {
        return 1;
    }
#undef MDVIT_GEMM_LAUNCH
    return 0;
}

struct GemmPlan { int cfg, tiles_m, tiles_n, splits, kps; };

int g_force_cfg = -1, g_force_splits = 0;

static const double g_split_penalty = [] { const char* e = getenv("MDVIT_SPLIT_PENALTY"); return e ? atof(e) : 12000.0; }();

GemmPlan plan_gemm(const MdvitGemmDesc* d) {
    static const int BMs[3] = {128, 256, 64}, BNs[3] = {128, 64, 64}, OCC[3] = {2, 2, 4};
    static const double EFF[3] = {0.8, 0.8, 1.0};
    static const int SPLITS[] = {1, 2, 3, 4, 6, 8, 12, 16, 24, 32, 48, 64, 96, 128, 192, 256};
    const bool plain = d->epi == MDVIT_EPI_NONE && !(d->e_drop_p > 0.f) && !d->e_rowscale && !d->residual;
    const bool can_split = d->allow_split && plain && d->K >= 512 && (d->N % 4 == 0);
    GemmPlan best; best.cfg = 0; best.tiles_m = cdiv(d->M, 128); best.tiles_n = cdiv(d->N, 128); best.splits = 1;
    best.kps = cdiv(d->K, BK) * BK;
    static const bool conv_rule = [] { const char* e = getenv("MDVIT_CONV_SPLIT_PLAN"); return !(e && e[0] == '0'); }();
    if (conv_rule && g_force_cfg < 0 && g_force_splits == 0 && d->conv_c > 0 && d->conv_up <= 1 && d->conv_stride == 1 && !d->trans_a && can_split && d->K >= 2304 && !d->rc_a) {
        const long tiles = (long)cdiv(d->M, 128) * cdiv(d->N, 128);
        if (tiles >= 64 && tiles <= 256) {
            const int want = (int)max(1L, min(4L, (512 + tiles / 2) / tiles));
            best.kps = cdiv(cdiv(d->K, want), BK) * BK;
            best.splits = cdiv(d->K, best.kps);
            return best;
        }
    }
    double best_cost = 1e300;
    for (int c = 0; c < 3; ++c) {
        if (g_force_cfg >= 0 && c != g_force_cfg && !d->rc_a) continue;
        if (d->rc_a && c != 2) continue;
        const long tm = cdiv(d->M, BMs[c]), tn = cdiv(d->N, BNs[c]);
        const long tiles = tm * tn;
        for (int si = 0; si < (int)(sizeof(SPLITS) / sizeof(int)); ++si) {
            const int want = SPLITS[si];
            if (want > 1 && (!can_split || want > d->K / 256)) break;
            if (g_force_splits > 0 && can_split && want != g_force_splits) continue;
            const int kps = cdiv(cdiv(d->K, want), BK) * BK;
            const int splits = cdiv(d->K, kps);
            const long wgs = tiles * splits;
            const long slots = 256L * OCC[c];
            const double rounds = wgs <= slots ? 1.0 : (double)wgs / (double)slots;
            const bool loads_epi = (d->epi == MDVIT_EPI_DGELU && !d->rc_a) || d->residual != nullptr;
            const double epi_cycles = (loads_epi && c != 2 ? 30.0 : 6.0) * BMs[c] * BNs[c] / 64.0;
            const double wg_cycles = d->precision == 1
                ? 0.0015 * BMs[c] * BNs[c] * (double)kps + (d->trans_a ? 0.12 : 0.06) * (BMs[c] + BNs[c]) * (double)kps + 800.0 + epi_cycles
                : 2.0 * BMs[c] * BNs[c] * (double)kps / (180.0 * EFF[c]) + 800.0 + epi_cycles;
            double cost = rounds * OCC[c] * wg_cycles;
            if (splits > 1) cost += g_split_penalty + (double)(splits + 1) * d->M * d->N * 8.0 / 1250.0;
            if (cost < best_cost) {
                best_cost = cost;
                best.cfg = c; best.tiles_m = (int)tm; best.tiles_n = (int)tn; best.splits = splits; best.kps = kps;
            }
        }
    }
    return best;
}

}

int mdvit_gemm_splitk_reduce_perm(const float* slab, const float* bias, float* C, long ldc, int M, int N, int splits, int accumulate, int perm_cin, hipStream_t s);
int mdvit_gemm_splitk_reduce(const float* slab, const float* bias, float* C, long ldc, int M, int N, int splits, int accumulate, hipStream_t s) {
    return mdvit_gemm_splitk_reduce_perm(slab, bias, C, ldc, M, N, splits, accumulate, 0, s);
}
int mdvit_gemm_splitk_reduce_perm(const float* slab, const float* bias, float* C, long ldc, int M, int N, int splits, int accumulate, int perm_cin, hipStream_t s) {
    const long total = (long)M * N / 4;
#define MDVIT_REDUCE_LAUNCH(R_) \
    hipLaunchKernelGGL((gemm_splitk_reduce_kernel<R_>), dim3((int)min((total * R_ + 255) / 256, 4096L)), dim3(256), 0, s, \
                       slab, bias, C, ldc, M, N, splits, accumulate, perm_cin)
    if (total >= 65536 || splits < 4) MDVIT_REDUCE_LAUNCH(1);
    else if (total >= 16384 || splits < 16) MDVIT_REDUCE_LAUNCH(4);
    else if (total >= 4096 || splits < 64) MDVIT_REDUCE_LAUNCH(16);
    else MDVIT_REDUCE_LAUNCH(64);
#undef MDVIT_REDUCE_LAUNCH
    MDVIT_LAUNCH_CHECK();
    return MDVIT_OK;
}

bool mdvit_gemm_tn_applies(const MdvitGemmDesc* d);
size_t mdvit_gemm_tn_ws_bytes(const MdvitGemmDesc* d);
void mdvit_gemm_tn_plan(const MdvitGemmDesc* d, int* tile_m, int* tile_n, int* splits);
int mdvit_gemm_tn_launch(const MdvitGemmDesc* d, hipStream_t s);

#include <mutex>
namespace {
struct LedgerRow { char name[160]; long launches; double flop, bytes; };
constexpr int LEDGER_ROWS = 512;
LedgerRow g_ledger[LEDGER_ROWS];
int g_ledger_n = 0;
bool g_ledger_on = false, g_ledger_shapes = false;
std::mutex g_ledger_mu;
}
extern "C" int mdvit_gemm_kernel_name(const MdvitGemmDesc* d, char* out, int32_t cap);
extern "C" int mdvit_gemm_ledger(int32_t enable) {
    std::lock_guard<std::mutex> lk(g_ledger_mu);
    if (enable) g_ledger_n = 0;
    g_ledger_on = enable != 0;
    g_ledger_shapes = enable == 2;
    return MDVIT_OK;
}
extern "C" int mdvit_gemm_ledger_read(int32_t index, char* name, int32_t cap, int64_t* launches, double* flop, double* bytes) {
    std::lock_guard<std::mutex> lk(g_ledger_mu);
    MDVIT_CHECK_ARG(name && cap > 0 && launches && flop && bytes, MDVIT_E_SHAPE, "gemm_ledger_read: null argument");
    if (index < 0 || index >= g_ledger_n) return MDVIT_E_SHAPE;
    snprintf(name, cap, "%s", g_ledger[index].name);
    *launches = g_ledger[index].launches; *flop = g_ledger[index].flop; *bytes = g_ledger[index].bytes;
    return MDVIT_OK;
}
static void ledger_note(const MdvitGemmDesc* d) {
    char nm[160];
    if (mdvit_gemm_kernel_name(d, nm, sizeof(nm)) != MDVIT_OK) return;
    if (char* plus = strchr(nm, '+')) *plus = 0;
    std::lock_guard<std::mutex> lk(g_ledger_mu);
    if (g_ledger_shapes) {
        const size_t n = strlen(nm);
        snprintf(nm + n, sizeof(nm) - n, " M=%d N=%d K=%d ta=%d tb=%d%s%s%s%s", d->M, d->N, d->K, (int)d->trans_a, (int)d->trans_b, d->C2 ? " +C2" : "", d->residual ? " +res" : "",
                 d->gelu_u ? " +u" : "", d->rc_a ? " +rc" : "");
    }
    int i = 0;
    while (i < g_ledger_n && strcmp(g_ledger[i].name, nm) != 0) ++i;
    if (i == g_ledger_n) {
        if (g_ledger_n == LEDGER_ROWS) return;
        snprintf(g_ledger[i].name, sizeof(g_ledger[i].name), "%s", nm);
        g_ledger[i].launches = 0; g_ledger[i].flop = 0.0; g_ledger[i].bytes = 0.0;
        ++g_ledger_n;
    }
    const double M = d->M, N = d->N, K = d->K;
    g_ledger[i].launches += 1;
    g_ledger[i].flop += 2.0 * M * N * K;
    g_ledger[i].bytes += 4.0 * (M * K + N * K + M * N * (1 + (d->C2 != nullptr) + (d->residual != nullptr) + (d->gelu_u != nullptr))) + (d->rc_a ? 4.0 * (M + N) * d->rc_k : 0.0);
}

namespace {
constexpr int SAMP_MAX = 4096, SAMP_SYMS = 128;
struct SampSym { char name[160]; long seen, timed; double ms; };
SampSym g_samp_sym[SAMP_SYMS];
int g_samp_nsym = 0, g_samp_stride = 0, g_samp_n = 0;
char g_samp_only[160] = {0};
hipEvent_t g_samp_ev[SAMP_MAX][2];
int g_samp_ev_made = 0, g_samp_of[SAMP_MAX];
bool g_samp_folded = true;
}
extern "C" int mdvit_gemm_sampler(const char* symbol, int32_t stride) {
    g_samp_stride = stride > 0 ? stride : 0;
    g_samp_nsym = 0; g_samp_n = 0; g_samp_folded = false;
    snprintf(g_samp_only, sizeof(g_samp_only), "%s", symbol ? symbol : "");
    return MDVIT_OK;
}
extern "C" int mdvit_gemm_sampler_read(int32_t index, char* name, int32_t cap, int64_t* seen, int64_t* timed, double* ms) {
    MDVIT_CHECK_ARG(name && cap > 0 && seen && timed && ms, MDVIT_E_SHAPE, "gemm_sampler_read: null argument");
    if (!g_samp_folded) {
        g_samp_stride = 0;
        for (int i = 0; i < g_samp_n; ++i) {
            float t = 0.f;
            if (hipEventSynchronize(g_samp_ev[i][1]) != hipSuccess || hipEventElapsedTime(&t, g_samp_ev[i][0], g_samp_ev[i][1]) != hipSuccess) { (void)hipGetLastError(); continue; }
            g_samp_sym[g_samp_of[i]].timed += 1; g_samp_sym[g_samp_of[i]].ms += t;
        }
        g_samp_folded = true;
    }
    if (index < 0 || index >= g_samp_nsym) return MDVIT_E_SHAPE;
    snprintf(name, cap, "%s", g_samp_sym[index].name);
    *seen = g_samp_sym[index].seen; *timed = g_samp_sym[index].timed; *ms = g_samp_sym[index].ms;
    return MDVIT_OK;
}
static void sampler_note(const MdvitGemmDesc* d) {
    char nm[160];
    if (mdvit_gemm_kernel_name(d, nm, sizeof(nm)) != MDVIT_OK) return;
    if (char* plus = strchr(nm, '+')) *plus = 0;
    if (g_samp_only[0] && strcmp(g_samp_only, nm) != 0) return;
    int i = 0;
    while (i < g_samp_nsym && strcmp(g_samp_sym[i].name, nm) != 0) ++i;
    if (i == g_samp_nsym) {
        if (g_samp_nsym == SAMP_SYMS) return;
        snprintf(g_samp_sym[i].name, sizeof(g_samp_sym[i].name), "%s", nm);
        g_samp_sym[i].seen = 0; g_samp_sym[i].timed = 0; g_samp_sym[i].ms = 0.0;
        ++g_samp_nsym;
    }
    const long n = g_samp_sym[i].seen++;
    if (g_samp_n >= SAMP_MAX || (g_samp_stride > 1 && (((unsigned long)n * 2654435761UL) >> 7) % (unsigned long)g_samp_stride != 0)) return;
    if (g_samp_n >= g_samp_ev_made) {
        if (hipEventCreate(&g_samp_ev[g_samp_n][0]) != hipSuccess || hipEventCreate(&g_samp_ev[g_samp_n][1]) != hipSuccess) { (void)hipGetLastError(); return; }
        g_samp_ev_made = g_samp_n + 1;
    }
    g_samp_of[g_samp_n] = i;
    g_mdvit_t0 = g_samp_ev[g_samp_n][0]; g_mdvit_t1 = g_samp_ev[g_samp_n][1];
    ++g_samp_n;
}

extern "C" int mdvit_gemm_f32(const MdvitGemmDesc* d, void* stream) {
    hipStream_t s = (hipStream_t)stream;
    MDVIT_CHECK_ARG(d != nullptr, MDVIT_E_SHAPE, "gemm: null descriptor");
    MDVIT_CHECK_ARG(d->M > 0 && d->N > 0 && d->K > 0, MDVIT_E_SHAPE, "gemm: bad shape M=%d N=%d K=%d", d->M, d->N, d->K);
    if (g_ledger_on) ledger_note(d);
    if (g_samp_stride > 0 && d->A && d->B && d->C) sampler_note(d);
    MDVIT_CHECK_ARG(d->A && d->B && d->C, MDVIT_E_SHAPE, "gemm: null operand");
    MDVIT_CHECK_ARG(aligned16(d->A) && aligned16(d->B) && (d->lda % 4 == 0) && (d->ldb % 4 == 0), MDVIT_E_ALIGN,
                    "gemm: operands must be 16-byte aligned with leading dimensions %% 4 == 0 (lda=%ld ldb=%ld)", d->lda, d->ldb);
    MDVIT_CHECK_ARG(d->trans_a ? (d->M % 4 == 0) : (d->K % 4 == 0), MDVIT_E_ALIGN, "gemm: contiguous extent of A must be %% 4 (M=%d K=%d ta=%d)", d->M, d->K, d->trans_a);
    MDVIT_CHECK_ARG(d->trans_b ? (d->K % 4 == 0) : (d->N % 4 == 0), MDVIT_E_ALIGN, "gemm: contiguous extent of B must be %% 4 (N=%d K=%d tb=%d)", d->N, d->K, d->trans_b);
    MDVIT_CHECK_ARG(d->epi != MDVIT_EPI_DGELU || d->gelu_u || d->rc_a, MDVIT_E_SHAPE, "gemm: DGELU needs gelu_u (or rc_a/rc_b to recompute it)");
    if (d->rc_a) {
        MDVIT_CHECK_ARG(d->epi == MDVIT_EPI_DGELU && !d->gelu_u && d->rc_b && d->rc_k > 0 && !d->trans_a && d->trans_b, MDVIT_E_SHAPE,
                        "gemm: rc_a/rc_b (recomputed pre-activation) go with the NT DGELU epilogue and no gelu_u");
        MDVIT_CHECK_ARG(aligned16(d->rc_a) && aligned16(d->rc_b) && d->rc_lda % 4 == 0 && d->rc_ldb % 4 == 0 && d->rc_k % BK == 0 &&
                        (!d->rc_bias || aligned16(d->rc_bias)), MDVIT_E_ALIGN, "gemm: rc operands must be 16-byte aligned, leading dimensions %% 4 == 0, rc_k %% 32 == 0");
    }
    MDVIT_CHECK_ARG(!(d->e_drop_p > 0.f) || (long)d->M * d->N < (1L << 32), MDVIT_E_SHAPE, "gemm: dropout index space exceeds 2^32");

    GemmArgs a;
    memset(&a, 0, sizeof(a));
    a.A = d->A; a.B = d->B; a.C = d->C; a.C2 = d->C2;
    a.lda = d->lda; a.ldb = d->ldb; a.ldc = d->ldc; a.M = d->M; a.N = d->N; a.K = d->K;
    a.bias = d->bias;
    a.epi = d->epi;
    a.e_drop = d->e_drop_p > 0.f; a.e_k0 = d->e_key0; a.e_k1 = d->e_key1;
    a.e_thresh = mdvit_drop_thresh(d->e_drop_p); a.e_inv_keep = 1.f / (1.f - d->e_drop_p);
    a.e_rowscale = d->e_rowscale; a.e_rows_per_scale = d->e_rows_per_scale > 0 ? d->e_rows_per_scale : 1;
    a.residual = d->residual; a.ldr = d->ldr; a.gelu_u = d->gelu_u; a.ldu = d->ldu;
    a.rc_a = d->rc_a; a.rc_lda = d->rc_lda; a.rc_b = d->rc_b; a.rc_ldb = d->rc_ldb; a.rc_bias = d->rc_bias; a.rc_k = d->rc_k;
    a.accumulate = d->accumulate;
    a.colsum = d->colsum_a;
    MDVIT_CHECK_ARG(!d->colsum_a || (d->trans_a && !d->trans_b), MDVIT_E_SHAPE, "gemm: colsum_a rides on the TN (wgrad) layout only");
    a.seed = d->drop_seed;
    if (d->conv_c > 0) {
        MDVIT_CHECK_ARG(d->precision >= 1 && d->epi == MDVIT_EPI_NONE && !(d->e_drop_p > 0.f) && !d->e_rowscale && !d->residual && !d->rc_a, MDVIT_E_SHAPE,
                        "gemm: the implicit 3x3 convolution is built for precision >= 1 and the plain epilogue");
        MDVIT_CHECK_ARG(d->conv_c % BK == 0 && d->conv_h > 0 && d->conv_w > 0 && d->conv_ho > 0 && d->conv_wo > 0 && d->conv_stride >= 1 && d->conv_dilation >= 1,
                        MDVIT_E_SHAPE, "gemm: implicit convolution needs conv_c %% 32 == 0 and positive extents (conv_c=%d)", d->conv_c);
        if (d->trans_a && !d->trans_b) {
            MDVIT_CHECK_ARG(d->N == 9 * d->conv_c && d->K % (d->conv_ho * d->conv_wo) == 0 && mdvit_gemm_tn_applies(d), MDVIT_E_SHAPE,
                            "gemm: implicit-convolution weight gradient needs N == 9 conv_c, K == B conv_ho conv_wo (N=%d K=%d conv_c=%d)", d->N, d->K, d->conv_c);
        } else {
            MDVIT_CHECK_ARG(!d->trans_a && d->trans_b && d->K == 9 * d->conv_c && d->M % (d->conv_ho * d->conv_wo) == 0, MDVIT_E_SHAPE,
                            "gemm: implicit convolution (NT) needs K == 9 conv_c, M == B conv_ho conv_wo (M=%d K=%d conv_c=%d)", d->M, d->K, d->conv_c);
            a.conv_c = d->conv_c; a.conv_h = d->conv_h; a.conv_w = d->conv_w; a.conv_ho = d->conv_ho; a.conv_wo = d->conv_wo;
            a.conv_stride = d->conv_stride; a.conv_dil = d->conv_dilation; a.conv_up = d->conv_up > 1 ? d->conv_up : 1;
            MDVIT_CHECK_ARG(a.conv_up == 1 || d->conv_stride == 1, MDVIT_E_SHAPE, "gemm: conv_up (transposed convolution) goes with conv_stride == 1");
        }
    }
    if (mdvit_gemm_tn_applies(d)) return mdvit_gemm_tn_launch(d, s);
    MDVIT_CHECK_ARG(!d->a_bf16 && !d->b_bf16, MDVIT_E_SHAPE, "gemm: bf16-stored operands are a layout of the weight-gradient (TN, precision 1) kernel only");

    const GemmPlan pl = plan_gemm(d);
    a.tiles_m = pl.tiles_m; a.tiles_n = pl.tiles_n; a.splits = pl.splits; a.k_per_split = pl.kps;
    if (g_groups.n > 0) {
        MDVIT_CHECK_ARG(pl.splits == 1 && d->epi == MDVIT_EPI_NONE && !d->residual && !d->rc_a && d->conv_c <= 0 && !(d->e_drop_p > 0.f) && !d->e_rowscale,
                        MDVIT_E_SHAPE, "gemm (grouped): one K range, plain epilogue");
        a.ngroups = g_groups.n;
        for (int g = 0; g < g_groups.n; ++g) { a.gA[g] = g_groups.A[g]; a.gB[g] = g_groups.B[g]; a.gC[g] = g_groups.C[g]; a.gBias[g] = g_groups.bias[g]; }
    }
    if (pl.splits > 1) {
        const size_t need = sizeof(float) * (size_t)pl.splits * d->M * d->N;
        MDVIT_CHECK_ARG(d->ws != nullptr && d->ws_bytes >= need, MDVIT_E_WORKSPACE,
                        "gemm: split reduction needs %zu bytes of workspace (mdvit_gemm_ws_bytes), got %zu", need, (size_t)d->ws_bytes);
        a.slab = (float*)d->ws;
        a.bias = nullptr;
    }
    int epi = EPI_PLAIN;
    if (d->epi == MDVIT_EPI_GELU_DUAL) epi = EPI_GELU2;
    else if (d->epi == MDVIT_EPI_DGELU) epi = d->rc_a ? EPI_DGELU_RC : EPI_DGELU;
    else if (a.e_drop || d->e_rowscale || d->residual) epi = EPI_FULL;
    a.vec = ((d->N & 3) == 0) && ((d->ldc & 3) == 0) && aligned16(d->C);
    if (epi != EPI_PLAIN) {
        MDVIT_CHECK_ARG(a.vec && (!d->bias || aligned16(d->bias)) && (!d->C2 || aligned16(d->C2)) &&
                        (!d->residual || (aligned16(d->residual) && d->ldr % 4 == 0)) && (!d->gelu_u || (aligned16(d->gelu_u) && d->ldu % 4 == 0)),
                        MDVIT_E_ALIGN, "gemm: fused epilogues need N %% 4 == 0 and 16-byte aligned C / bias / residual / gelu_u rows");
        MDVIT_CHECK_ARG(!d->accumulate, MDVIT_E_SHAPE, "gemm: accumulate is only defined for the plain epilogue");
    } else if (d->bias && !aligned16(d->bias)) {
        a.vec = 0;
    }
    bool conv_phase_on = d->conv_c > 0 && a.conv_up == 2;
    if (conv_phase_on) { const char* e = getenv("MDVIT_CONV_PHASE"); conv_phase_on = !(e && e[0] == '0'); }
    a.conv_phase = (conv_phase_on && a.conv_ho == 2 * a.conv_h && a.conv_wo == 2 * a.conv_w && (d->M & 3) == 0 && (d->M >> 2) % 256 == 0 &&
                    pl.splits == 1 && a.vec && !d->accumulate) ? 1 : 0;
    int rc;
    if (pl.cfg == 0) rc = launch_cfg<128, 128, 2, 2>(a, d->trans_a, d->trans_b, epi, d->precision, s);
    else if (pl.cfg == 1) rc = launch_cfg<256, 64, 4, 1>(a, d->trans_a, d->trans_b, epi, d->precision, s);
    else rc = launch_cfg<64, 64, 2, 2>(a, d->trans_a, d->trans_b, epi, d->precision, s);
    MDVIT_CHECK_ARG(rc == 0, MDVIT_E_SHAPE, "gemm: this (trans_a=%d, trans_b=%d, epilogue=%d, precision=%d) combination is not built", d->trans_a, d->trans_b, epi, d->precision);
    if (pl.splits > 1) {
        const long total = (long)d->M * d->N / 4;
#define MDVIT_REDUCE_LAUNCH(R_) \
    hipLaunchKernelGGL((gemm_splitk_reduce_kernel<R_>), dim3((int)min((total * R_ + 255) / 256, 4096L)), dim3(256), 0, s, \
                       a.slab, d->bias, d->C, (long)d->ldc, d->M, d->N, pl.splits, d->accumulate, 0)
        if (total >= 65536 || pl.splits < 4) MDVIT_REDUCE_LAUNCH(1);
        else if (total >= 16384 || pl.splits < 16) MDVIT_REDUCE_LAUNCH(4);
        else if (total >= 4096 || pl.splits < 64) MDVIT_REDUCE_LAUNCH(16);
        else MDVIT_REDUCE_LAUNCH(64);
#undef MDVIT_REDUCE_LAUNCH
    }
    MDVIT_LAUNCH_CHECK();
    return MDVIT_OK;
}

__global__ __launch_bounds__(256) void conv_weight_relayout_kernel(const float* __restrict__ w, float* __restrict__ out, int Cout, int Cin, int mode) {
    const long total = (long)Cout * Cin * 9;
    for (long e = (long)blockIdx.x * blockDim.x + threadIdx.x; e < total; e += (long)gridDim.x * blockDim.x) {
        if (mode == 0) {
            const int ci = (int)(e % Cin); const int t = (int)((e / Cin) % 9); const int co = (int)(e / (9L * Cin));
            out[e] = w[((long)co * Cin + ci) * 9 + t];
        } else if (mode == 1) {
            const int co = (int)(e % Cout); const int t = (int)((e / Cout) % 9); const int ci = (int)(e / (9L * Cout));
            out[e] = w[((long)co * Cin + ci) * 9 + (8 - t)];
        } else {
            const int t = (int)(e % 9); const int ci = (int)((e / 9) % Cin); const int co = (int)(e / (9L * Cin));
            const float v = w[((long)co * 9 + t) * Cin + ci];
            out[e] = mode == 3 ? out[e] + v : v;
        }
    }
}

__global__ __launch_bounds__(256) void conv_weight_relayout_many_kernel(const long long* __restrict__ items) {
    __shared__ float s_t[32 * 73];
    const long long* it = items + 5 * (long)blockIdx.y;
    const float* w = reinterpret_cast<const float*>(it[0]);
    float* out = reinterpret_cast<float*>(it[1]);
    const int Cout = (int)it[2], Cin = (int)it[3], mode = (int)it[4];
    const int tid = threadIdx.x;
    if (mode == 0) {
        const int nch = (Cin + 255) / 256, ntiles = Cout * nch;
        for (int tile = blockIdx.x; tile < ntiles; tile += gridDim.x) {
            const int co = tile / nch, ci0 = (tile % nch) * 256, nci = min(256, Cin - ci0);
            const float* src = w + ((long)co * Cin + ci0) * 9;
            for (int i = tid; i < nci * 9; i += 256) s_t[i] = src[i];
            __syncthreads();
            for (int i = tid; i < nci * 9; i += 256) {
                const int t = i / nci, c = i - t * nci;
                out[((long)co * 9 + t) * Cin + ci0 + c] = s_t[c * 9 + t];
            }
            __syncthreads();
        }
    } else {
        const int ncb = (Cout + 31) / 32, nib = (Cin + 7) / 8, ntiles = ncb * nib;
        for (int tile = blockIdx.x; tile < ntiles; tile += gridDim.x) {
            const int co0 = (tile / nib) * 32, ci0 = (tile % nib) * 8, ncl = min(32, Cout - co0), run = min(8, Cin - ci0) * 9;
            for (int i = tid; i < ncl * 72; i += 256) {
                const int c = i / 72, r = i - c * 72;
                if (r < run) s_t[c * 73 + r] = w[((long)(co0 + c) * Cin + ci0) * 9 + r];
            }
            __syncthreads();
            for (int i = tid; i < 72 * 32; i += 256) {
                const int c = i & 31, r = i >> 5, k = r / 9, tp = r - k * 9;
                if (c < ncl && k * 9 < run) out[((long)(ci0 + k) * 9 + tp) * Cout + co0 + c] = s_t[c * 73 + k * 9 + 8 - tp];
            }
            __syncthreads();
// ... 62 lines not shown
extern "C" int mdvit_transpose_many(const void* items_dev, int32_t n, int32_t blocks_per_item, void* stream) {
    MDVIT_CHECK_ARG(items_dev && n > 0 && blocks_per_item > 0, MDVIT_E_SHAPE, "transpose_many: bad arguments");
    hipLaunchKernelGGL(transpose_many_kernel, dim3(blocks_per_item, n), dim3(256), 0, (hipStream_t)stream, (const long long*)items_dev);
    MDVIT_LAUNCH_CHECK();
    return MDVIT_OK;
}

namespace {
constexpr int TB_MAX = 24;
struct TransposeBatchArgs { const float* in[TB_MAX]; float* out[TB_MAX]; long ld[TB_MAX]; int rows[TB_MAX]; int cols[TB_MAX]; };
__global__ __launch_bounds__(256) void transpose_batch_kernel(TransposeBatchArgs a) {
    __shared__ float tile[32][33];
    const float* in = a.in[0]; float* out = a.out[0]; long ld_in = a.ld[0]; int rows = a.rows[0], cols = a.cols[0];
    const int y = blockIdx.y;
#pragma unroll
    for (int i = 1; i < TB_MAX; ++i)
        if (y == i) { in = a.in[i]; out = a.out[i]; ld_in = a.ld[i]; rows = a.rows[i]; cols = a.cols[i]; }
    const int tiles_x = (cols + 31) / 32, tiles_y = (rows + 31) / 32;
    const int tx = threadIdx.x & 31, ty = threadIdx.x >> 5;
    for (int tidx = blockIdx.x; tidx < tiles_x * tiles_y; tidx += gridDim.x) {
        const int r0 = (tidx / tiles_x) * 32, c0 = (tidx % tiles_x) * 32;
#pragma unroll
        for (int i = 0; i < 4; ++i) {
            const int r = r0 + ty + 8 * i, c = c0 + tx;
            tile[ty + 8 * i][tx] = (r < rows && c < cols) ? in[(long)r * ld_in + c] : 0.f;
        }
        __syncthreads();
#pragma unroll
        for (int i = 0; i < 4; ++i) {
            const int c = c0 + ty + 8 * i, r = r0 + tx;
            if (c < cols && r < rows) out[(long)c * rows + r] = tile[tx][ty + 8 * i];
        }
        __syncthreads();
    }
}
}

extern "C" int mdvit_transpose_batch(int32_t n, const void* const* in, const int64_t* ld_in, void* const* out, const int32_t* rows, const int32_t* cols, void* stream) {
    MDVIT_CHECK_ARG(n >= 1 && n <= TB_MAX && in && ld_in && out && rows && cols, MDVIT_E_SHAPE, "transpose_batch: 1 <= n <= %d items", TB_MAX);
    TransposeBatchArgs a; memset(&a, 0, sizeof(a));
    int tiles = 1;
    for (int i = 0; i < n; ++i) {
        MDVIT_CHECK_ARG(in[i] && out[i] && rows[i] > 0 && cols[i] > 0 && ld_in[i] >= cols[i], MDVIT_E_SHAPE, "transpose_batch: item %d: bad shape", i);
        a.in[i] = (const float*)in[i]; a.out[i] = (float*)out[i]; a.ld[i] = (long)ld_in[i]; a.rows[i] = rows[i]; a.cols[i] = cols[i];
        tiles = max(tiles, cdiv(rows[i], 32) * cdiv(cols[i], 32));
    }
    hipLaunchKernelGGL(transpose_batch_kernel, dim3(min(tiles, 64), n), dim3(256), 0, (hipStream_t)stream, a);
    MDVIT_LAUNCH_CHECK();
    return MDVIT_OK;
}

extern "C" int mdvit_transpose_f32(const float* in, int64_t ld_in, float* out, int32_t rows, int32_t cols, void* stream) {
    MDVIT_CHECK_ARG(in && out && rows > 0 && cols > 0 && ld_in >= cols, MDVIT_E_SHAPE, "transpose: bad shape rows=%d cols=%d ld=%ld", rows, cols, (long)ld_in);
    hipLaunchKernelGGL(transpose_kernel, dim3(cdiv(cols, 32), cdiv(rows, 32)), dim3(256), 0, (hipStream_t)stream, in, (long)ld_in, out, rows, cols);
    MDVIT_LAUNCH_CHECK();
    return MDVIT_OK;
}

extern "C" int mdvit_gemm_force_plan(int32_t cfg, int32_t splits) {
    g_force_cfg = (cfg >= 0 && cfg <= 2) ? cfg : -1;
    g_force_splits = splits > 0 ? splits : 0;
    return MDVIT_OK;
}

extern "C" int mdvit_gemm_plan(const MdvitGemmDesc* d, int32_t* tile_m, int32_t* tile_n, int32_t* splits) {
    MDVIT_CHECK_ARG(d != nullptr && d->M > 0 && d->N > 0 && d->K > 0, MDVIT_E_SHAPE, "gemm_plan: bad descriptor");
    if (mdvit_gemm_tn_applies(d)) { mdvit_gemm_tn_plan(d, tile_m, tile_n, splits); return MDVIT_OK; }
    const GemmPlan pl = plan_gemm(d);
    if (tile_m) *tile_m = pl.cfg == 0 ? 128 : (pl.cfg == 1 ? 256 : 64);
    if (tile_n) *tile_n = pl.cfg == 0 ? 128 : 64;
    if (splits) *splits = pl.splits;
    return MDVIT_OK;
}

void mdvit_gemm_tn_name(const MdvitGemmDesc* d, char* out, int cap);
extern "C" int mdvit_gemm_kernel_name(const MdvitGemmDesc* d, char* out, int32_t cap) {
    MDVIT_CHECK_ARG(d != nullptr && out != nullptr && cap > 0 && d->M > 0 && d->N > 0 && d->K > 0, MDVIT_E_SHAPE, "gemm_kernel_name: bad arguments");
    if (mdvit_gemm_tn_applies(d)) { mdvit_gemm_tn_name(d, out, cap); return MDVIT_OK; }
    const GemmPlan pl = plan_gemm(d);
    const bool drop = d->e_drop_p > 0.f;
    int epi = EPI_PLAIN;
    if (d->epi == MDVIT_EPI_GELU_DUAL) epi = EPI_GELU2;
    else if (d->epi == MDVIT_EPI_DGELU) epi = d->rc_a ? EPI_DGELU_RC : EPI_DGELU;
    else if (drop || d->e_rowscale || d->residual) epi = EPI_FULL;
    const int bm = pl.cfg == 0 ? 128 : (pl.cfg == 1 ? 256 : 64), bn = pl.cfg == 0 ? 128 : 64;
    if (d->conv_c > 0) {
        snprintf(out, cap, "gemm_conv3x3_kernel<%d, %d, %s>%s", bm, bn, pl.cfg == 1 ? "4, 1" : "2, 2", pl.splits > 1 ? "+splitk_reduce" : "");
        return MDVIT_OK;
    }
    snprintf(out, cap, "gemm_f32_kernel<%d, %d, %s, %s, %s, %d, %s>%s", bm, bn, pl.cfg == 1 ? "4, 1" : "2, 2", d->trans_a ? "true" : "false",
             d->trans_b ? "true" : "false", epi, d->precision ? "true" : "false", pl.splits > 1 ? "+splitk_reduce" : "");
    return MDVIT_OK;
}

extern "C" size_t mdvit_gemm_ws_bytes(const MdvitGemmDesc* d) {
    if (d == nullptr || d->M <= 0 || d->N <= 0 || d->K <= 0) return 0;
    if (mdvit_gemm_tn_applies(d)) return mdvit_gemm_tn_ws_bytes(d);
    const GemmPlan pl = plan_gemm(d);
    return pl.splits > 1 ? sizeof(float) * (size_t)pl.splits * d->M * d->N : 0;
}

extern "C" int mdvit_gemm_f32_grouped(const MdvitGemmDesc* desc, int32_t G, const void* const* A, const void* const* B, void* const* C, void* stream) {
    MDVIT_CHECK_ARG(desc != nullptr && G >= 1 && G <= MDVIT_GEMM_MAX_GROUPS && A && B && C, MDVIT_E_SHAPE, "gemm (grouped): 1 <= G <= %d operand triples", MDVIT_GEMM_MAX_GROUPS);
    MdvitGemmDesc d = *desc;
    d.allow_split = 0; d.ws = nullptr; d.ws_bytes = 0;
    d.A = (const float*)A[0]; d.B = (const float*)B[0]; d.C = (float*)C[0];
    for (int g = 0; g < G; ++g) {
        MDVIT_CHECK_ARG(A[g] && B[g] && C[g] && aligned16(A[g]) && aligned16(B[g]), MDVIT_E_ALIGN, "gemm (grouped): group %d: null or unaligned operand", g);
        MDVIT_CHECK_ARG(aligned16(C[g]) == aligned16(C[0]), MDVIT_E_ALIGN, "gemm (grouped): the outputs must share their 16-byte alignment class");
        g_groups.A[g] = (const float*)A[g]; g_groups.B[g] = (const float*)B[g]; g_groups.C[g] = (float*)C[g];
    }
    for (int g = 0; g < G; ++g) g_groups.bias[g] = nullptr;
    g_groups.n = G;
    const int rc = mdvit_gemm_f32(&d, stream);
    g_groups.n = 0;
    return rc;
}

extern "C" int mdvit_gemm_f32_grouped_bias(const MdvitGemmDesc* desc, int32_t G, const void* const* A, const void* const* B, void* const* C, const void* const* bias,
                                           void* stream) {
    MDVIT_CHECK_ARG(desc != nullptr && G >= 1 && G <= MDVIT_GEMM_MAX_GROUPS && A && B && C && bias, MDVIT_E_SHAPE, "gemm (grouped): 1 <= G <= %d operand triples", MDVIT_GEMM_MAX_GROUPS);
    MDVIT_CHECK_ARG(!desc->trans_a, MDVIT_E_SHAPE, "gemm (grouped, bias): NN / NT only");
    MdvitGemmDesc d = *desc;
    d.allow_split = 0; d.ws = nullptr; d.ws_bytes = 0; d.bias = nullptr;
    d.A = (const float*)A[0]; d.B = (const float*)B[0]; d.C = (float*)C[0];
    for (int g = 0; g < G; ++g) {
        MDVIT_CHECK_ARG(A[g] && B[g] && C[g] && bias[g] && aligned16(A[g]) && aligned16(B[g]) && aligned16(bias[g]), MDVIT_E_ALIGN, "gemm (grouped): group %d: null or unaligned operand", g);
        MDVIT_CHECK_ARG(aligned16(C[g]) == aligned16(C[0]), MDVIT_E_ALIGN, "gemm (grouped): the outputs must share their 16-byte alignment class");
        g_groups.A[g] = (const float*)A[g]; g_groups.B[g] = (const float*)B[g]; g_groups.C[g] = (float*)C[g]; g_groups.bias[g] = (const float*)bias[g];
    }
    g_groups.n = G;
    const int rc = mdvit_gemm_f32(&d, stream);
    g_groups.n = 0;
    return rc;
}
```

mdvit_amd/csrc/gemm_body.inc:

```
    constexpr bool A_PAIR = BF3 && TA, B_PAIR = BF3 && !TB;
    static_assert(!BF3 || !(TA && TB), "bf16x3: TT is not a layout of this model");
    constexpr int LDSA = TA ? BM + 4 : BM + 1, LDSB = TB ? BN + 1 : BN + 4;
    constexpr int LDKB = 80;
    constexpr int SMEM_FLOATS = BF3 ? (BM + BN) * 2 * LDKB / 4 : BK * LDSA + BK * LDSB;
    constexpr int WTM = BM / WAVES_M / 32, WTN = BN / WAVES_N / 32;
    constexpr int A_V4 = BM * BK / 4 / NTHREADS, B_V4 = BN * BK / 4 / NTHREADS;
    constexpr int KT = BK / 4;
    constexpr bool DB = (BM == 64 && BN == 64 && !TA) && !MDVIT_NO_DB;
    __shared__ __attribute__((aligned(16))) float smem[DB ? 2 * SMEM_FLOATS : SMEM_FLOATS];
    float* As = smem;
    float* Bs = smem + BK * LDSA;
    char* sb = reinterpret_cast<char*>(smem);
    char* Ahi = sb; char* Alo = sb + BM * LDKB; char* Bhi = sb + 2 * BM * LDKB; char* Blo = Bhi + BN * LDKB;
    auto stage = [&](int b) {
        float* base = smem + b * SMEM_FLOATS;
        As = base; Bs = base + BK * LDSA;
        sb = reinterpret_cast<char*>(base);
        Ahi = sb; Alo = sb + BM * LDKB; Bhi = sb + 2 * BM * LDKB; Blo = Bhi + BN * LDKB;
    };

    const int tid = threadIdx.x, lane = tid & 63, wave = tid >> 6;
    uint32_t s0 = 0, s1 = 0;
    if (p.seed) { s0 = p.seed[0]; s1 = p.seed[1]; }
    const uint32_t ek0 = p.e_k0 ^ s0, ek1 = p.e_k1 + s1;
// ... 348 lines not shown
            mma_into(acc);
        }
    };
    if (DB && !PF2) {
        int buf = 0;
        load_a(kbeg, SET0{}); load_b(kbeg, SET0{});
        store_smem(SET0{}, kbeg);
        __syncthreads();
        if (kbeg + BK < kend) { load_a(kbeg + BK, SET0{}); load_b(kbeg + BK, SET0{}); }
        for (int k0 = kbeg; k0 < kend; k0 += BK) {
            if (k0 + BK < kend) {
                stage(buf ^ 1);
                store_smem(SET0{}, k0 + BK);
                stage(buf);
                if (k0 + 2 * BK < kend) { load_a(k0 + 2 * BK, SET0{}); load_b(k0 + 2 * BK, SET0{}); }
            }
            mma(k0);
            __syncthreads();
            buf ^= 1;
            stage(buf);
        }
        stage(0);
    } else if (DB) {
        int buf = 0;
        load_a(kbeg, SET0{}); load_b(kbeg, SET0{});
        using SETB = std::integral_constant<int, PF2 ? 1 : 0>;
        load_a(kbeg + BK, SETB{}); load_b(kbeg + BK, SETB{});
        store_smem(SET0{}, kbeg);
        __syncthreads();
        load_a(kbeg + 2 * BK, SET0{}); load_b(kbeg + 2 * BK, SET0{});
        auto step = [&](int k0, auto setc) __attribute__((always_inline)) {
            stage(buf ^ 1);
            store_smem(setc, k0 + BK);
            stage(buf);
            load_a(k0 + 3 * BK, setc); load_b(k0 + 3 * BK, setc);
            __builtin_amdgcn_sched_barrier(0);
            mma(k0);
            __syncthreads();
            buf ^= 1;
            stage(buf);
        };
        for (int k0 = kbeg; k0 < kend; k0 += 2 * BK) {
            step(k0, SETB{});
            step(k0 + BK, SET0{});
        }
        stage(0);
    } else {
        load_a(kbeg, SET0{}); load_b(kbeg, SET0{});
        store_smem(SET0{}, kbeg);
        __syncthreads();
        for (int k0 = kbeg; k0 < kend; k0 += BK) {
            const bool more = (k0 + BK) < kend;
            if (more) { load_a(k0 + BK, SET0{}); load_b(k0 + BK, SET0{}); }
            mma(k0);
            __syncthreads();
            if (more) {
                store_smem(SET0{}, k0 + BK);
                __syncthreads();
            }
        }
    }

    if (TA && do_cs) {
        float* s_cs = smem;
        for (int i = tid; i < BM; i += NTHREADS) s_cs[i] = 0.f;
        __syncthreads();
        if (A_PAIR) {
#pragma unroll
            for (int v = 0; v < A_V4 / 2; ++v) {
                const int mq = (tid >> 4) + 16 * v;
                atomicAdd(&s_cs[4 * mq + 0], cs[v].x); atomicAdd(&s_cs[4 * mq + 1], cs[v].y);
                atomicAdd(&s_cs[4 * mq + 2], cs[v].z); atomicAdd(&s_cs[4 * mq + 3], cs[v].w);
            }
        } else {
            const int c = (tid % (BM / 4)) * 4;
            atomicAdd(&s_cs[c + 0], cs[0].x); atomicAdd(&s_cs[c + 1], cs[0].y);
            atomicAdd(&s_cs[c + 2], cs[0].z); atomicAdd(&s_cs[c + 3], cs[0].w);
        }
        __syncthreads();
        for (int i = tid; i < BM; i += NTHREADS)
            if (m0 + i < p.M) atomicAdd(&p.colsum[m0 + i], s_cs[i]);
    }

    const bool split = (EPI == EPI_PLAIN) && p.splits > 1;
    float* slab = split ? p.slab + (long)blockIdx.y * p.M * p.N : nullptr;
    if (EPI == EPI_PLAIN && !split && !p.vec) {
#pragma unroll
        for (int i = 0; i < WTM; ++i) {
            const int row = m0 + wm0 + i * 32 + l31;
            if (row >= p.M) continue;
#pragma unroll
            for (int j = 0; j < WTN; ++j) {
#pragma unroll
                for (int q = 0; q < 4; ++q) {
                    const int col = n0 + wn0 + j * 32 + 8 * q + 4 * lhi;
                    if (col >= p.N) continue;
                    float* dst = gC + (long)row * p.ldc + col;
                    const float vv[4] = {acc[i][j][4 * q + 0], acc[i][j][4 * q + 1], acc[i][j][4 * q + 2], acc[i][j][4 * q + 3]};
                    const int nv = min(4, p.N - col);
#pragma unroll 1
                    for (int t = 0; t < nv; ++t) {
                        float o = vv[t] + (gBias ? gBias[col + t] : 0.f);
                        if (p.accumulate) o += dst[t];
                        dst[t] = o;
                    }
                }
            }
        }
        return;
    }
    const float* any_p = reinterpret_cast<const float*>(gB);
    const bool use_bias = gBias != nullptr;
    const float* bias_p = use_bias ? gBias : any_p;
    float4 bq[WTN][4];
#pragma unroll
    for (int j = 0; j < WTN; ++j)
#pragma unroll
        for (int q = 0; q < 4; ++q) {
            const int col = min(n0 + wn0 + j * 32 + 8 * q + 4 * lhi, p.N - 4);
            const float4 b4 = *reinterpret_cast<const float4*>(bias_p + (use_bias ? col : 0));
            bq[j][q] = use_bias ? b4 : make_float4(0.f, 0.f, 0.f, 0.f);
        }
    float rscs[WTM];
#pragma unroll
    for (int i = 0; i < WTM; ++i) rscs[i] = 1.f;
    if constexpr (EPI == EPI_FULL) {
        const bool use_rs = p.e_rowscale != nullptr;
        const float* rs_p = use_rs ? p.e_rowscale : any_p;
#pragma unroll
        for (int i = 0; i < WTM; ++i) {
            const int row = min(m0 + wm0 + i * 32 + l31, p.M - 1);
            const float v = rs_p[use_rs ? row / p.e_rows_per_scale : 0];
            rscs[i] = use_rs ? v : 1.f;
        }
    }
    constexpr bool HAS_IN = EPI == EPI_PLAIN || ((EPI == EPI_DGELU || EPI == EPI_FULL) && !EPRE);
    const bool use_in = EPI == EPI_PLAIN ? (p.accumulate != 0 && !split) : (EPI == EPI_DGELU ? true : p.residual != nullptr);
    const float* in_p = EPI == EPI_PLAIN ? gC : (EPI == EPI_DGELU ? p.gelu_u : p.residual);
    const long in_ld = EPI == EPI_PLAIN ? p.ldc : (EPI == EPI_DGELU ? p.ldu : p.ldr);
    if (!use_in || in_p == nullptr) in_p = any_p;
    float4 inq[2][4];
    auto load_in = [&](int ij) __attribute__((always_inline)) {
        if constexpr (HAS_IN) {
            const int i = ij / WTN, j = ij % WTN;
            const int row = min(m0 + wm0 + i * 32 + l31, p.M - 1);
#pragma unroll
            for (int q = 0; q < 4; ++q) {
                const int col = min(n0 + wn0 + j * 32 + 8 * q + 4 * lhi, p.N - 4);
                inq[ij & 1][q] = *reinterpret_cast<const float4*>(in_p + (use_in ? (long)row * in_ld + col : 0L));
            }
        }
    };
    load_in(0);
#pragma unroll
    for (int ij = 0; ij < WTM * WTN; ++ij) {
        const int i = ij / WTN, j = ij % WTN;
        if (ij + 1 < WTM * WTN) load_in(ij + 1);
        const int row = m0 + wm0 + i * 32 + l31;
        const bool row_ok = row < p.M;
#pragma unroll
        for (int q = 0; q < 4; ++q) {
            const int col = n0 + wn0 + j * 32 + 8 * q + 4 * lhi;
            const bool ok = row_ok && col < p.N;
            float4 v = make_float4(acc[i][j][4 * q + 0], acc[i][j][4 * q + 1], acc[i][j][4 * q + 2], acc[i][j][4 * q + 3]);
            float* dst = gC + (long)out_row(row) * p.ldc + col;
            if (split) { if (ok) *reinterpret_cast<float4*>(slab + (long)row * p.N + col) = v; continue; }
// ... 44 lines not shown
```

mdvit_amd/ops.py:

```python
from __future__ import annotations

import ctypes as C
import itertools
import os
import weakref
from typing import Optional, Tuple

import torch

from . import _lib
from ._lib import GemmDesc, call

_key_counter = itertools.count(1)
_POISON = os.environ.get("MDVIT_POISON", "0") == "1"


def _empty(*a, **k):
    t = torch.empty(*a, **k)
    if _POISON and t.is_floating_point():
        t.fill_(float("nan"))
    return t


def _empty_like(x):
    t = torch.empty_like(x)
    if _POISON and t.is_floating_point():
        t.fill_(float("nan"))
    return t


def _next_key() -> Tuple[int, int]:
    n = next(_key_counter)
    seed = torch.initial_seed() & 0xFFFFFFFF
    k0 = (seed * 2654435761 + n * 0x9E3779B1) & 0xFFFFFFFF
    k1 = ((n * 0x85EBCA6B) ^ (seed >> 3) ^ 0xC2B2AE35) & 0xFFFFFFFF
    return k0, k1


_seed_buf = None


def enable_device_seed(flag: bool = True):
    global _seed_buf
    global _SEED_STEP
    _seed_buf = torch.tensor([0x1234567, 0x89ABCDE], dtype=torch.int32, device="cuda") if flag else None
    _SEED_STEP = torch.tensor([-1640531527, 2135587861], dtype=torch.int32, device="cuda") if flag else None


def bump_seed():
    if _seed_buf is not None:
        _seed_buf.add_(_SEED_STEP)


_SEED_STEP = None


def _seed_ptr():
    return None if _seed_buf is None else C.c_void_p(_seed_buf.data_ptr())


def _p(t: Optional[torch.Tensor]):
    return None if t is None else t.data_ptr()


def _partials_ws(n: int, device):
    nbytes = _lib.load().mdvit_partials_ws_bytes(int(n))
    t = torch.empty((nbytes // 4,), device=device, dtype=torch.float32)
    return C.c_void_p(t.data_ptr()), nbytes, t


_raw_stream = torch._C._cuda_getCurrentRawStream
_cur_device = torch._C._cuda_getDevice


def _stream():
    return _raw_stream(_cur_device())


_set_stream_raw = torch._C._cuda_setStream
_get_stream_raw = torch._C._cuda_getCurrentStream
_stream_objs = {}
_ev_ring, _ev_next = [], 0


def current_stream_obj():
    sid, di, dt = _get_stream_raw(_cur_device())
    st = _stream_objs.get((sid, di))
# ... 653 lines not shown
    torch.cuda.synchronize()
    table = {}
    ms = C.c_float()
    for name, flop, nbytes, e0, e1 in ev:
        r = table.setdefault(name, {"n": 0, "ms": 0.0, "flop": 0.0, "bytes": 0.0, "timer": "event pair around the launch"})
        r["n"] += 1
        if isinstance(e0, int):
            call("mdvit_event_elapsed_ms", e0, e1, C.byref(ms))
            r["ms"] += ms.value
            r["timer"] = "kernel begin/end timestamps (hipExtLaunchKernelGGL start/stop events)"
        else:
            r["ms"] += e0.elapsed_time(e1)
        r["flop"] += flop
        r["bytes"] += nbytes
    _lib_events_release()
    ovh = event_pair_overhead_ms()
    for name, r in table.items():
        r["launches"] = _events_seen.get(name, r["n"])
        r["event_pair_overhead_ms"] = ovh if r["timer"].startswith("event pair") else 0.0
    return table


_lib_event_pool = []


def _lib_event() -> int:
    h = C.c_void_p()
    call("mdvit_event_create", C.byref(h))
    _lib_event_pool.append(h.value)
    return h.value


def _lib_events_release():
    while _lib_event_pool:
        call("mdvit_event_destroy", _lib_event_pool.pop())


def event_pair_overhead_ms(n: int = 32) -> float:
    torch.cuda.synchronize()
    pairs = []
    for _ in range(n):
        e0, e1 = torch.cuda.Event(enable_timing=True), torch.cuda.Event(enable_timing=True)
        e0.record(); e1.record()
        pairs.append((e0, e1))
    torch.cuda.synchronize()
    v = sorted(a.elapsed_time(b) for a, b in pairs)
    return v[len(v) // 2]


def _ld_view(t: torch.Tensor) -> Tuple[int, int, int]:
    if t.dim() == 4 and t.is_contiguous():
        return t.shape[0], t.numel() // t.shape[0], t.numel() // t.shape[0]
    if t.dim() != 2 or t.stride(1) != 1:
        raise _lib.MdvitHipError("expected a 2-D row-contiguous tensor")
    return t.shape[0], t.shape[1], t.stride(0)


class _Linear(torch.autograd.Function):
    @staticmethod
    def forward(ctx, x, W, b, residual, rowscale, drop_p, rows_per_scale):
        ctx.set_materialize_grads(False)
        _chk(x, b, residual, rowscale)
        M, K = x.shape
        N, K2, ldb = _ld_view(W)
        assert K == K2
        y = _empty((M, N), device=x.device, dtype=torch.float32)
        key = _next_key() if drop_p > 0 else (0, 0)
        if _lin_rc_ok(M, N, K) and ldb == K and (residual is not None or (drop_p == 0 and rowscale is None)):
            _linear_rc(x, W, False, b, y, M, N, K, drop_p, key, rowscale, rows_per_scale, residual)
        elif _plane_ok(M, N, K, residual is not None):
            gemm_nt(x, W, y, M, N, K, bias=b, e_drop=drop_p, e_key=key, e_rowscale=rowscale, e_rows_per_scale=rows_per_scale,
                    residual=residual, allow_split=True)
        else:
            gemm(_p(x), _p(W), _p(y), M, N, K, lda=K, ldb=ldb, ldc=N, bias=_p(b),
                 e_drop=drop_p, e_key=key, e_rowscale=_p(rowscale), e_rows_per_scale=rows_per_scale,
                 residual=_p(residual), ldr=N, allow_split=True)
        ctx.save_for_backward(x, W, rowscale)
        ctx.meta = (drop_p, key, rows_per_scale, b is not None, residual is not None)
        ctx.bias_ref = b if (b is not None and b.grad_fn is None) else None
        return y

    @staticmethod
    def backward(ctx, g):
        if g is None:
            return (None,) * 7
        x, W, rowscale = ctx.saved_tensors
        drop_p, key, rps, has_b, has_res = ctx.meta
        g = _c(g)
        M, K = x.shape
        N, _, ldb = _ld_view(W)
        dx = dW = db = None
        want_w = not _dgrad_only and (ctx.needs_input_grad[1] or (has_b and ctx.needs_input_grad[2]))
        sW = sb = None
        if want_w:
            sW = _sink_of(W)
            sb = _sink_of(ctx.bias_ref) if has_b else None
        sunk = want_w and sW is not None and (not has_b or sb is not None)
        want_b = want_w and has_b and (sunk or ctx.needs_input_grad[2])
        ride = want_b and (sunk or ctx.needs_input_grad[1])
        if want_b and not sunk:
            db = _zeros_once(N, x.device) if ride else _empty((N,), device=x.device, dtype=torch.float32)
        masked = drop_p > 0 or rowscale is not None
        gm = _empty_like(g) if masked else g
        if masked or (want_b and not ride):
            sums = want_b and not ride
            wsp, wsb, _keep = _partials_ws(N, g.device) if sums else (None, 0, None)
            call("mdvit_colsum_f32", _p(g), N, _p(sb if sunk else db) if sums else None, _p(gm) if masked else None, wsp, wsb, M, N,
                 drop_p, key[0], key[1], _p(rowscale), rps, int(sunk), _seed_ptr() if drop_p > 0 else None, _stream())
        if ctx.needs_input_grad[0]:
            dx = _empty_like(x)
            _dgrad(gm, W, dx, M, K, N, ldb, allow_split=True)
        if want_w:
            if sunk:
                with _on_side(gm, x):
                    gemm(_p(gm), _p(x), _p(sW), N, K, M, lda=N, ldb=K, ldc=K, trans_a=True, trans_b=False, allow_split=True, accumulate=True,
                         colsum_a=_p(sb) if ride else None)
                db = None
            elif ctx.needs_input_grad[1]:
                dW = _empty(tuple(W.shape) if W.dim() == 4 else (N, K), device=x.device, dtype=torch.float32)
                gemm(_p(gm), _p(x), _p(dW), N, K, M, lda=N, ldb=K, ldc=K, trans_a=True, trans_b=False, allow_split=True,
                     colsum_a=_p(db) if ride else None)
        return dx, dW, db, (g if has_res else None), None, None, None


def linear(x, W, b=None, residual=None, rowscale=None, drop_p: float = 0.0, rows_per_scale: int = 1):
    shp = x.shape
    x2 = _c(x).view(-1, shp[-1])
    if W.dim() == 4 and not W.is_contiguous():
        W = W.reshape(W.shape[0], -1)
    r2 = None if residual is None else _c(residual).view(-1, W.shape[0])
    y = _Linear.apply(x2, W, b, r2, rowscale, float(drop_p), int(rows_per_scale))
    return y.view(*shp[:-1], W.shape[0])


class _MatMul(torch.autograd.Function):

    @staticmethod
    def forward(ctx, A, B):
        ctx.set_materialize_grads(False)
        M, K, lda = _ld_view(A)
        K2, N, ldb = _ld_view(B)
        assert K == K2
        out = _empty((M, N), device=A.device, dtype=torch.float32)
        gemm(_p(A), _p(B), _p(out), M, N, K, lda=lda, ldb=ldb, ldc=N, trans_b=False, allow_split=True)
        ctx.save_for_backward(A, B)
        return out

    @staticmethod
    def backward(ctx, g):
        if g is None:
            return (None,) * 2
        if _dgrad_only:
            return None, None
        A, B = ctx.saved_tensors
        g = _c(g)
        M, K, lda = _ld_view(A)
        _, N, ldb = _ld_view(B)
        dA = dB = None
        if ctx.needs_input_grad[0]:
            dA = _empty((M, K), device=A.device, dtype=torch.float32)
            gemm(_p(g), _p(B), _p(dA), M, K, N, lda=N, ldb=ldb, ldc=K, trans_b=True, allow_split=True)
        if ctx.needs_input_grad[1]:
            dB = _empty((K, N), device=A.device, dtype=torch.float32)
            gemm(_p(A), _p(g), _p(dB), K, N, M, lda=lda, ldb=N, ldc=N, trans_a=True, trans_b=False, allow_split=True)
        return dA, dB


def matmul(A, B):
    return _MatMul.apply(A, B)


_zero_slab = [None, 0, None, None]


def _zeros_once(n: int, device):
    if torch.cuda.is_current_stream_capturing() or n > 16384:
        return torch.zeros((n,), device=device, dtype=torch.float32)
    slab, off, ev, fs = _zero_slab
    n4 = (n + 3) & ~3
    cur = current_stream_obj()
    if slab is None or slab.device != device or off + n4 > slab.numel():
        slab, off = torch.zeros((65536,), device=device, dtype=torch.float32), 0
        ev = torch.cuda.Event()
        ev.record(cur)
        fs = cur.cuda_stream
    elif ev is not None:
        if ev.query():
            ev = None
        elif cur.cuda_stream != fs:
            cur.wait_event(ev)
    if slab is not None and cur.cuda_stream != fs:
        slab.record_stream(cur)
# ... 331 lines not shown
        elif u is None and _mlp_rc16_ok(Cin, Hd, ctx.b1_ref, W1, W2, M):
            du = None if _dgrad_only else _empty_like(h)
            W1p, W2tp, W1tp = _wplanes(W1, False, 2), _wplanes(W2, True, 2), _wplanes(W1, True, 2)
            call("mdvit_mlp_rc16_dgrad", _p(gm), _p(x), _p(W1p), _p(ctx.b1_ref), _p(W2tp), _p(W1tp), _p(du), _p(dx), M, Cin, Hd,
                 drop_p, k1[0], k1[1], _seed_ptr() if drop_p > 0 else None, _stream())
            del W1p, W2tp, W1tp
        else:
            du = _empty_like(h)
            if u is None and (_plane_rc or _gemm_precision == 2) and _use_plane_gemm and Cin % 32 == 0 and W1.is_contiguous() and W2.is_contiguous():
                gemm_nt(to_planes(gm), W2, du, M, Hd, Cin, w_transposed=True, epi=_lib.EPI_DGELU, rc=(to_planes(x), W1, ctx.b1_ref, Cin),
                        e_drop=drop_p, e_key=k1)
            elif u is None:
                _dgrad(gm, W2, du, M, Hd, Cin, Hd, epi=_lib.EPI_DGELU, rc=(_p(x), Cin, _p(W1), Cin, _p(ctx.b1_ref), Cin), e_drop=drop_p, e_key=k1)
            else:
                _dgrad(gm, W2, du, M, Hd, Cin, Hd, epi=_lib.EPI_DGELU, gelu_u=_p(u), ldu=Hd, e_drop=drop_p, e_key=k1)
            _dgrad(du, W1, dx, M, Cin, Hd, Cin, allow_split=True)
        if not _dgrad_only:
            if sunk:
                dW1_, db1_, dW2_, _ = sinks
                with _on_side(gm, h, du, x):
                    gemm(_p(gm), _p(h), _p(dW2_), Cin, Hd, M, lda=Cin, ldb=Hd, ldc=Hd, trans_a=True, trans_b=False, allow_split=True, accumulate=True,
                         colsum_a=_p(sinks[3]))
                    gemm(_p(du), _p(x), _p(dW1_), Hd, Cin, M, lda=Hd, ldb=Cin, ldc=Cin, trans_a=True, trans_b=False, allow_split=True, accumulate=True,
                         colsum_a=_p(db1_))
                db2 = None
            else:
                dW2 = _empty_like(W2)
                gemm(_p(gm), _p(h), _p(dW2), Cin, Hd, M, lda=Cin, ldb=Hd, ldc=Hd, trans_a=True, trans_b=False, allow_split=True, colsum_a=_p(db2))
                dW1 = _empty_like(W1)
                db1 = torch.zeros((Hd,), device=dev, dtype=torch.float32)
                gemm(_p(du), _p(x), _p(dW1), Hd, Cin, M, lda=Hd, ldb=Cin, ldc=Cin, trans_a=True, trans_b=False, allow_split=True, colsum_a=_p(db1))
        return dx, g, dW1, db1, dW2, db2, None, None, None


def mlp_residual(x, res, W1, b1, W2, b2, rowscale=None, drop_p=0.0, rows_per_scale=1):
    shp = res.shape
    out = _MlpResidual.apply(_c(x).view(-1, shp[-1]), _c(res).view(-1, shp[-1]), W1, b1, W2, b2, rowscale,
                             float(drop_p), int(rows_per_scale))
    return out.view(shp)


class _LayerNorm(torch.autograd.Function):

    @staticmethod
    def forward(ctx, x, gamma, beta, eps, fork):
        ctx.set_materialize_grads(False)
        _chk(x, gamma, beta)
        M, Cn = x.shape
        groups = gamma.shape[0] if gamma.dim() == 2 else 1
        if M % groups:
            raise ValueError(f"layer_norm: {M} rows are not {groups} equal groups")
        y = _empty_like(x)
        mean = _empty((M,), device=x.device, dtype=torch.float32)
        rstd = _empty_like(mean)
        call("mdvit_layernorm_fwd", _p(x), _p(gamma), _p(beta), _p(y), _p(mean), _p(rstd), M, Cn, groups, eps, _stream())
        ctx.save_for_backward(x, gamma, mean, rstd)
        if fork:
            return y, x.view_as(x)
        return y

    @staticmethod
    def backward(ctx, g, g_pass=None):
        if g is None:
            return g_pass, None, None, None, None
        x, gamma, mean, rstd = ctx.saved_tensors
        g = _c(g)
        M, Cn = x.shape
        dx = _empty_like(x)
        gp = None if g_pass is None else _c(g_pass)
        fast = Cn in (64, 128, 320, 512)
        if _dgrad_only and fast:
            call("mdvit_layernorm_bwd", _p(g), _p(x), _p(gamma), _p(mean), _p(rstd), _p(gp), _p(dx), None, None, None, 0, M, Cn,
                 gamma.shape[0] if gamma.dim() == 2 else 1, _stream())
            return dx, None, None, None, None
        dg, db = _flat_like(gamma, gamma)
        wsp, wsb, _keep = _partials_ws(2 * Cn, x.device)
        call("mdvit_layernorm_bwd", _p(g), _p(x), _p(gamma), _p(mean), _p(rstd), _p(gp), _p(dx), _p(dg), _p(db), wsp, wsb, M, Cn,
             gamma.shape[0] if gamma.dim() == 2 else 1, _stream())
        if _dgrad_only:
            return dx, None, None, None, None
        return dx, dg, db, None, None


def layer_norm(x, gamma, beta, eps=1e-6):
    shp = x.shape
    return _LayerNorm.apply(_c(x).view(-1, shp[-1]), _c(gamma), _c(beta), float(eps), False).view(shp)


def layer_norm_fork(x, gamma, beta, eps=1e-6):
    shp = x.shape
    y, xr = _LayerNorm.apply(_c(x).view(-1, shp[-1]), _c(gamma), _c(beta), float(eps), True)
    return y.view(shp), xr.view(shp)


class _DwConv3x3(torch.autograd.Function):
    @staticmethod
    def forward(ctx, x, w, bias, stride, add_input):
        ctx.set_materialize_grads(False)
        _chk(x, w, bias)
        B, H, W_, Cn = x.shape
        Ho, Wo = (H - 1) // stride + 1, (W_ - 1) // stride + 1
        y = _empty((B, Ho, Wo, Cn), device=x.device, dtype=torch.float32)
        call("mdvit_dwconv3x3_fwd", _p(x), _p(w), _p(bias), _p(y), B, H, W_, Cn, stride, int(add_input), _stream())
        ctx.save_for_backward(x, w)
        ctx.meta = (stride, add_input, bias is not None)
        ctx.bias_ref = bias if (bias is not None and bias.grad_fn is None) else None
        return y

    @staticmethod
    def backward(ctx, g):
        if g is None:
            return (None,) * 5
        x, w = ctx.saved_tensors
        stride, add_input, has_b = ctx.meta
        g = _c(g)
        B, H, W_, Cn = x.shape
        dx = _empty_like(x) if ctx.needs_input_grad[0] else None
        dw = db = None
        if dx is not None:
            call("mdvit_dwconv3x3_bwd", _p(g), _p(x), _p(w), _p(dx), None, None, None, 0, B, H, W_, Cn, stride, int(add_input), 0, _stream())
        if not _dgrad_only:
            sw = _sink_of(w) if _side_stream is not None else None
            sb = _sink_of(ctx.bias_ref) if (has_b and sw is not None) else None
            if sw is not None and (not has_b or sb is not None):
                with _on_side(g, x) as _:
                    wsp, wsb, keep = _partials_ws(10 * Cn, x.device)
                    call("mdvit_dwconv3x3_bwd", _p(g), _p(x), _p(w), None, _p(sw), _p(sb), wsp, wsb, B, H, W_, Cn, stride, int(add_input), 1, _stream())
            else:
                dw, db = _flat_like(w, (Cn,) if has_b else None)
                wsp, wsb, _keep = _partials_ws(10 * Cn, x.device)
                call("mdvit_dwconv3x3_bwd", _p(g), _p(x), _p(w), None, _p(dw), _p(db), wsp, wsb, B, H, W_, Cn, stride, int(add_input), 0, _stream())
        return dx, dw, db, None, None


def dwconv3x3(x, w, bias=None, stride=1, add_input=False):
    return _DwConv3x3.apply(_c(x), w, bias, int(stride), bool(add_input))


class _GConv2(torch.autograd.Function):
    @staticmethod
    def forward(ctx, skip, up, w):
        ctx.set_materialize_grads(False)
        _chk(skip, up, w)
        B, H, W_, Cn = skip.shape
        y = _empty_like(skip)
        call("mdvit_gconv2_3x3_fwd", _p(skip), _p(up), _p(w), _p(y), B, H, W_, Cn, _stream())
        ctx.save_for_backward(skip, up, w)
        return y

    @staticmethod
    def backward(ctx, g):
        if g is None:
            return (None,) * 3
        skip, up, w = ctx.saved_tensors
        g = _c(g)
        B, H, W_, Cn = skip.shape
        dskip, dup = _empty_like(skip), _empty_like(up)
        sw = _sink_of(w) if (_side_stream is not None and not _dgrad_only) else None
        dw = None if (_dgrad_only or sw is not None) else _empty_like(w)
        wsp, wsb, _keep = _partials_ws(18 * Cn, g.device) if dw is not None else (None, 0, None)
        call("mdvit_gconv2_3x3_bwd", _p(g), _p(skip), _p(up), _p(w), _p(dskip), _p(dup), _p(dw), wsp, wsb, B, H, W_, Cn, 0, _stream())
        if sw is not None:
            with _on_side(g, skip, up):
                wsp, wsb, keep = _partials_ws(18 * Cn, g.device)
                call("mdvit_gconv2_3x3_bwd", _p(g), _p(skip), _p(up), _p(w), None, None, _p(sw), wsp, wsb, B, H, W_, Cn, 1, _stream())
        return dskip, dup, dw
# ... 1489 lines not shown
```

Before: 519.0 images/s.

## Fuse LayerNorm backward into QKV dgrad GEMM epilogue for small channel widths

```diff
diff --git a/include/mdvit_hip.h b/include/mdvit_hip.h
--- a/include/mdvit_hip.h
+++ b/include/mdvit_hip.h
@@ -19,7 +19,7 @@
     MDVIT_E_HIP = 5
 };
 
-enum { MDVIT_EPI_NONE = 0, MDVIT_EPI_GELU_DUAL = 1, MDVIT_EPI_DGELU = 2 };
+enum { MDVIT_EPI_NONE = 0, MDVIT_EPI_GELU_DUAL = 1, MDVIT_EPI_DGELU = 2, MDVIT_EPI_LN_BWD = 3 };
 enum { MDVIT_ACT_NONE = 0, MDVIT_ACT_HSWISH = 1, MDVIT_ACT_RELU = 2 };
 
 const char* mdvit_last_error(void);
@@ -54,8 +54,13 @@
     int32_t conv_up;
     int32_t a_bf16, b_bf16;
     int32_t conv_wgrad_nchw;
+    const float* ln_x; int64_t ln_ldx; const float* ln_mean; const float* ln_rstd; const float* ln_gamma; float* ln_part;
 } MdvitGemmDesc;
 size_t mdvit_gemm_ws_bytes(const MdvitGemmDesc* desc);
+int32_t mdvit_gemm_ln_bwd_rows(const MdvitGemmDesc* desc);
+size_t mdvit_qkv_ln_bwd_ws_bytes(int32_t M, int32_t C, int32_t want_params);
+int mdvit_qkv_ln_bwd(const float* dqkv, const float* Wt, const float* x, const float* mean, const float* rstd, const float* gamma, const float* add, float* dx1,
+                     float* dgamma, float* dbeta, void* ws, size_t ws_bytes, int32_t M, int32_t C, int32_t accumulate, void* stream);
 #define MDVIT_GEMM_MAX_GROUPS 8
 int mdvit_gemm_f32_grouped(const MdvitGemmDesc* desc, int32_t G, const void* const* A, const void* const* B, void* const* C, void* stream);
 int mdvit_gemm_f32_grouped_bias(const MdvitGemmDesc* desc, int32_t G, const void* const* A, const void* const* B, void* const* C, const void* const* bias, void* stream);
@@ -158,6 +163,7 @@
 int mdvit_mlp_rc_config(int32_t fwd_variant);
 int mdvit_mlp_rc_planes(int32_t planes);
 int mdvit_block_config(int32_t mlp_bwd_fused);
+int mdvit_block_qkv_ln(int32_t enable);
 int mdvit_mlp_rc_wgrad(const float* gm, const float* x, const void* W1p, const float* b1, const void* W2tp, float* dW1, float* db1, float* dW2,
                        void* ws, size_t ws_bytes, int32_t M, int32_t C, int32_t hidden, float drop_p, uint32_t key1_0, uint32_t key1_1,
                        const uint32_t* drop_seed, int32_t accumulate, void* stream);
diff --git a/mdvit_amd/_lib.py b/mdvit_amd/_lib.py
--- a/mdvit_amd/_lib.py
+++ b/mdvit_amd/_lib.py
@@ -9,7 +9,7 @@
 LIB_PATH = os.environ.get("MDVIT_HIP_LIB") or os.path.join(_HERE, "lib", "libmdvit_hip.so")
 HEADER_PATH = os.path.join(_HERE, "..", "include", "mdvit_hip.h")
 
-EPI_NONE, EPI_GELU_DUAL, EPI_DGELU = 0, 1, 2
+EPI_NONE, EPI_GELU_DUAL, EPI_DGELU, EPI_LN_BWD = 0, 1, 2, 3
 ACT_NONE, ACT_HSWISH, ACT_RELU = 0, 1, 2
 
 f32p = C.c_void_p
@@ -42,6 +42,7 @@
         ("conv_c", i32), ("conv_h", i32), ("conv_w", i32), ("conv_ho", i32), ("conv_wo", i32), ("conv_stride", i32), ("conv_dilation", i32),
         ("conv_up", i32),
         ("a_bf16", i32), ("b_bf16", i32), ("conv_wgrad_nchw", i32),
+        ("ln_x", vp), ("ln_ldx", i64), ("ln_mean", vp), ("ln_rstd", vp), ("ln_gamma", vp), ("ln_part", vp),
     ]
 
 
@@ -131,6 +132,8 @@
     "mdvit_mlp_rc_config": [i32],
     "mdvit_mlp_rc_planes": [i32],
     "mdvit_block_config": [i32],
+    "mdvit_block_qkv_ln": [i32],
+    "mdvit_qkv_ln_bwd": [vp, vp, vp, vp, vp, vp, vp, vp, vp, vp, vp, C.c_size_t, i32, i32, i32, vp],
     "mdvit_gemm_ledger": [i32],
     "mdvit_gemm_ledger_read": [i32, C.c_char_p, i32, C.POINTER(i64), C.POINTER(C.c_double), C.POINTER(C.c_double)],
     "mdvit_gemm_sampler": [C.c_char_p, i32],
@@ -310,6 +313,10 @@
     lib.mdvit_upsample_multi_bwd_ws_bytes.argtypes = [vp, i32, i32, i32, i32]
     lib.mdvit_upsample_bwd_ws_bytes.restype = C.c_size_t
     lib.mdvit_upsample_bwd_ws_bytes.argtypes = [i32] * 6
+    lib.mdvit_gemm_ln_bwd_rows.restype = i32
+    lib.mdvit_gemm_ln_bwd_rows.argtypes = [C.POINTER(GemmDesc)]
+    lib.mdvit_qkv_ln_bwd_ws_bytes.restype = C.c_size_t
+    lib.mdvit_qkv_ln_bwd_ws_bytes.argtypes = [i32, i32, i32]
     lib.mdvit_partials_ws_bytes.restype = C.c_size_t
     lib.mdvit_partials_ws_bytes.argtypes = [i32]
     lib.mdvit_mlp_rc_wgrad_ws_bytes.restype = C.c_size_t
diff --git a/mdvit_amd/blocks.py b/mdvit_amd/blocks.py
--- a/mdvit_amd/blocks.py
+++ b/mdvit_amd/blocks.py
@@ -254,10 +254,11 @@
 
 
 class _FactorAttBase(nn.Module):
-    def _attend(self, x, size, domain_label, da_params, res, rowscale):
-        B, N, Cn = x.shape
+    def _attend(self, x, size, domain_label, da_params, res, rowscale, qkv=None):
         H, W = size
-        qkv = ops.linear(x, self.qkv.weight, self.qkv.bias)
+        if qkv is None:
+            qkv = ops.linear(x, self.qkv.weight, self.qkv.bias)
+        N = qkv.shape[1]
         y = ops.factor_att(qkv, self.crpe.params(), H, W, self.num_heads, self.crpe.head_splits, domain_label, da_params,
                            aux_first=getattr(self, "aux_first", False))
         return ops.linear(y, self.proj.weight, self.proj.bias, residual=res, rowscale=rowscale,
@@ -276,8 +277,8 @@
         self.proj_drop_p = proj_drop
         self.crpe = shared_crpe
 
-    def forward(self, x, size, _res=None, _rowscale=None):
-        return self._attend(x, size, None, None, _res, _rowscale)
+    def forward(self, x, size, _res=None, _rowscale=None, _qkv=None):
+        return self._attend(x, size, None, None, _res, _rowscale, _qkv)
 
 
 class FactorAtt_ConvRelPosEnc_Sup(_FactorAttBase):
@@ -295,9 +296,9 @@
         self.domain_layer = nn.Sequential(LinearParams(num_domains, hidden), _NoParams(), LinearParams(hidden, dim))
         self.crpe = shared_crpe
 
-    def forward(self, x, size, domain_label, _res=None, _rowscale=None):
+    def forward(self, x, size, domain_label, _res=None, _rowscale=None, _qkv=None):
         d0, d2 = self.domain_layer[0], self.domain_layer[2]
-        return self._attend(x, size, domain_label, (d0.weight, d0.bias, d2.weight, d2.bias), _res, _rowscale)
+        return self._attend(x, size, domain_label, (d0.weight, d0.bias, d2.weight, d2.bias), _res, _rowscale, _qkv)
 
 
 class Mlp(nn.Module):
@@ -416,11 +417,16 @@
             return y
         x = self.cpe(x, size)
         s1, s2 = self._droppath_scales(x.shape[0], x.device)
-        cur, x = _pick(self, "norm1", "norm1s").fork(x)
+        n1, att = _pick(self, "norm1", "norm1s"), self.factoratt_crpe
+        cur = qkv = None
+        if isinstance(n1, LayerNormParams) and ops.ln_linear_ok(x, n1.weight, att.qkv.weight):
+            qkv, x = ops.ln_linear_fork(x, n1.weight, n1.bias, att.qkv.weight, att.qkv.bias, n1.eps)
+        else:
+            cur, x = n1.fork(x)
         if use_da:
-            x = self.factoratt_crpe(cur, size, domain_label, _res=x, _rowscale=s1)
-        else:
-            x = self.factoratt_crpe(cur, size, _res=x, _rowscale=s1)
+            x = att(cur, size, domain_label, _res=x, _rowscale=s1, _qkv=qkv)
+        else:
+            x = att(cur, size, _res=x, _rowscale=s1, _qkv=qkv)
         cur, x = _pick(self, "norm2", "norm2s").fork(x)
         return self.mlp(cur, _res=x, _rowscale=s2)
 
diff --git a/mdvit_amd/csrc/block.hip b/mdvit_amd/csrc/block.hip
--- a/mdvit_amd/csrc/block.hip
+++ b/mdvit_amd/csrc/block.hip
@@ -65,6 +65,25 @@
     if (mlp_bwd_fused < 0 || mlp_bwd_fused > 2) return mdvit_set_error(MDVIT_E_SHAPE, "block_config: mlp_bwd_fused in 0..2");
     g_blk_mlp_bwd = mlp_bwd_fused;
     return MDVIT_OK;
+}
+
+static int g_blk_qkv_ln = -1;
+static bool qkv_ln_on() {
+    static const bool env_on = [] { const char* e = getenv("MDVIT_BLK_QKV_LN"); return !(e && e[0] == '0'); }();
+    return g_blk_qkv_ln < 0 ? env_on : g_blk_qkv_ln != 0;
+}
+extern "C" int mdvit_block_qkv_ln(int32_t enable) {
+    if (enable < -1 || enable > 1) return mdvit_set_error(MDVIT_E_SHAPE, "block_qkv_ln: enable in -1..1");
+    g_blk_qkv_ln = enable;
+    return MDVIT_OK;
+}
+void qkv_ln_desc(MdvitGemmDesc& g, const float* dqkv, const float* Wt, const float* x, const float* mean, const float* rstd, const float* gamma, const float* add,
+                 float* dx1, float* part, int M, int C) {
+    memset(&g, 0, sizeof(g));
+    g.precision = 1; g.epi = MDVIT_EPI_LN_BWD;
+    g.A = dqkv; g.lda = 3 * C; g.B = Wt; g.ldb = 3 * C; g.C = dx1; g.ldc = C; g.M = M; g.N = C; g.K = 3 * C; g.trans_a = 0; g.trans_b = 1;
+    g.residual = add; g.ldr = C;
+    g.ln_x = x; g.ln_ldx = C; g.ln_mean = mean; g.ln_rstd = rstd; g.ln_gamma = gamma; g.ln_part = part;
 }
 
 #define BLK_RUN(call)                         \
@@ -414,11 +433,19 @@
                              d.da_hidden, C, d.heads, s));
     }
     float* dcur1 = tmp;
+    bool fuse_ln1 = false;
+    int ln1_rows = 0;
     {
         MdvitGemmDesc g;
         gemm_init(g, d);
         g.allow_split = 1;
-        int rc = gemm_dgrad(A, d, g, dqkv, d.qkv_w, d.qkv_wt, dcur1, M, C, 3 * C, s, d.qkvt_p);
+        if (qkv_ln_on() && (C == 64 || C == 128) && d.precision == 1 && d.ln_groups == 1 && !ph_takes(d, d.qkvt_p, M, C, 3 * C, 0) && !pm_split_takes(d, g, d.qkvt_p, M, C, 3 * C)) {
+            MdvitGemmDesc f;
+            qkv_ln_desc(f, nullptr, nullptr, nullptr, nullptr, nullptr, nullptr, nullptr, nullptr, nullptr, M, C);
+            ln1_rows = mdvit_gemm_ln_bwd_rows(&f);
+            fuse_ln1 = ln1_rows > 0 && (!want_w || ln1_rows <= MDVIT_MAX_PARTIAL_ROWS);
+        }
+        int rc = fuse_ln1 ? MDVIT_OK : gemm_dgrad(A, d, g, dqkv, d.qkv_w, d.qkv_wt, dcur1, M, C, 3 * C, s, d.qkvt_p);
         if (rc != MDVIT_OK) return rc;
         if (want_w) {
             if (!A.dry) { rc = fork_side(d, st, side); if (rc != MDVIT_OK) return rc; }
@@ -433,7 +460,14 @@
         void* pw = lnw ? A.take_bytes(pb) : nullptr;
         float* dg = want_w ? G.n1_g : (lnw ? A.take((long)d.ln_groups * C) : nullptr);
         float* db = want_w ? G.n1_b : (lnw ? A.take((long)d.ln_groups * C) : nullptr);
-        if (defer) {
+        if (fuse_ln1) {
+            void* pws = defer ? S.take_bytes(pb) : pw;
+            MdvitGemmDesc f;
+            qkv_ln_desc(f, dqkv, d.qkv_wt, sv.x1, sv.mean1, sv.rstd1, d.n1_g, dx2, dx1, want_w ? (float*)pws : nullptr, M, C);
+            BLK_RUN(mdvit_gemm_f32(&f, s));
+            if (defer) late[n_late++] = Late{(const float*)pws, 1, ln1_rows, C, dg, C, db};
+            else if (want_w) BLK_RUN(mdvit_reduce_partials_batched2((const float*)pws, 1, ln1_rows, C, dg, C, db, s));
+        } else if (defer) {
             void* pws = S.take_bytes(pb);
             int nb = 0;
             BLK_RUN(mdvit_layernorm_bwd_parts(dcur1, sv.x1, d.n1_g, sv.mean1, sv.rstd1, dx2, dx1, nullptr, pws, pb, M, C, d.ln_groups, 0.f, 0, 0, nullptr, 1, nullptr, s, &nb));
@@ -477,6 +511,42 @@
     return MDVIT_OK;
 }
 
+}
+
+extern "C" size_t mdvit_qkv_ln_bwd_ws_bytes(int32_t M, int32_t C, int32_t want_params) {
+    if (M <= 0 || C <= 0) return 0;
+    return (((size_t)M * C * sizeof(float) + 255) & ~(size_t)255) + (want_params ? mdvit_partials_ws_bytes(2 * C) : 0);
+}
+
+extern "C" int mdvit_qkv_ln_bwd(const float* dqkv, const float* Wt, const float* x, const float* mean, const float* rstd, const float* gamma, const float* add, float* dx1,
+                                float* dgamma, float* dbeta, void* ws, size_t ws_bytes, int32_t M, int32_t C, int32_t accumulate, void* stream) {
+    hipStream_t s = (hipStream_t)stream;
+    MDVIT_CHECK_ARG(dqkv && Wt && x && mean && rstd && gamma && dx1 && M > 0 && C > 0 && C % 4 == 0, MDVIT_E_SHAPE, "qkv_ln_bwd: null argument or bad shape (M=%d C=%d)", M, C);
+    MDVIT_CHECK_ARG((dgamma == nullptr) == (dbeta == nullptr), MDVIT_E_SHAPE, "qkv_ln_bwd: dgamma and dbeta go together");
+    const bool want = dgamma != nullptr;
+    MDVIT_CHECK_ARG(ws && (reinterpret_cast<uintptr_t>(ws) & 255) == 0 && ws_bytes >= mdvit_qkv_ln_bwd_ws_bytes(M, C, want), MDVIT_E_WORKSPACE,
+                    "qkv_ln_bwd: workspace too small or not 256-byte aligned: need %zu bytes (mdvit_qkv_ln_bwd_ws_bytes), got %zu", mdvit_qkv_ln_bwd_ws_bytes(M, C, want), ws_bytes);
+    float* dcur1 = (float*)ws;
+    const size_t pb = want ? mdvit_partials_ws_bytes(2 * C) : 0;
+    float* part = want ? reinterpret_cast<float*>((char*)ws + (((size_t)M * C * sizeof(float) + 255) & ~(size_t)255)) : nullptr;
+    MdvitGemmDesc g;
+    qkv_ln_desc(g, dqkv, Wt, x, mean, rstd, gamma, add, dx1, part, M, C);
+    const int rows = (qkv_ln_on() && (C == 64 || C == 128)) ? mdvit_gemm_ln_bwd_rows(&g) : 0;
+    if (rows > 0 && (!want || rows <= MDVIT_MAX_PARTIAL_ROWS)) {
+        const int rc = mdvit_gemm_f32(&g, s);
+        if (rc != MDVIT_OK || !want) return rc;
+        return mdvit_reduce_partials_batched2_acc(part, 1, rows, C, dgamma, C, dbeta, accumulate, s);
+    }
+    memset(&g, 0, sizeof(g));
+    g.precision = 1;
+    g.A = dqkv; g.lda = 3 * C; g.B = Wt; g.ldb = 3 * C; g.C = dcur1; g.ldc = C; g.M = M; g.N = C; g.K = 3 * C; g.trans_a = 0; g.trans_b = 1;
+    int rc = mdvit_gemm_f32(&g, s);
+    if (rc != MDVIT_OK) return rc;
+    if (!want) return mdvit_layernorm_bwd(dcur1, x, gamma, mean, rstd, add, dx1, nullptr, nullptr, nullptr, 0, M, C, 1, s);
+    int nb = 0;
+    rc = mdvit_layernorm_bwd_parts(dcur1, x, gamma, mean, rstd, add, dx1, nullptr, part, pb, M, C, 1, 0.f, 0, 0, nullptr, 1, nullptr, s, &nb);
+    if (rc != MDVIT_OK) return rc;
+    return mdvit_reduce_partials_batched2_acc(part, 1, nb, C, dgamma, C, dbeta, accumulate, s);
 }
 
 extern "C" size_t mdvit_block_save_bytes(const MdvitBlockDesc* d) {
diff --git a/mdvit_amd/csrc/gemm.hip b/mdvit_amd/csrc/gemm.hip
--- a/mdvit_amd/csrc/gemm.hip
+++ b/mdvit_amd/csrc/gemm.hip
@@ -29,6 +29,7 @@
     const float* residual; long ldr;
     const float* gelu_u; long ldu;
     const float* rc_a; long rc_lda; const float* rc_b; long rc_ldb; const float* rc_bias; int rc_k;
+    const float* ln_x; long ln_ldx; const float* ln_mean; const float* ln_rstd; const float* ln_gamma; float* ln_part;
     int splits; int k_per_split;
     float* slab;
     int accumulate;
@@ -47,7 +48,7 @@
     return (xcd < r ? xcd * (q + 1) : r * (q + 1) + (xcd - r) * q) + idx;
 }
 
-enum { EPI_PLAIN = 0, EPI_GELU2 = 1, EPI_DGELU = 2, EPI_FULL = 3, EPI_DGELU_RC = 4 };
+enum { EPI_PLAIN = 0, EPI_GELU2 = 1, EPI_DGELU = 2, EPI_FULL = 3, EPI_DGELU_RC = 4, EPI_LNBWD = 5 };
 
 __device__ __forceinline__ void split_bf16x3(const float4 x, uint2& hi, uint2& lo) {
     f32x2_t a = {x.x, x.y}, b = {x.z, x.w};
@@ -138,6 +139,7 @@
             else if (epi == EPI_DGELU) MDVIT_GEMM_LAUNCH(false, true, EPI_DGELU, true);
             else if (epi == EPI_DGELU_RC) { if (BM == 64 && BN == 64) MDVIT_GEMM_LAUNCH(false, true, (BM == 64 && BN == 64 ? EPI_DGELU_RC : EPI_DGELU), true); else return 1; }
             else if (epi == EPI_FULL) MDVIT_GEMM_LAUNCH(false, true, EPI_FULL, true);
+            else if (epi == EPI_LNBWD) MDVIT_GEMM_LAUNCH(false, true, EPI_LNBWD, true);
             else if (epi == EPI_PLAIN) MDVIT_GEMM_LAUNCH(false, true, EPI_PLAIN, true);
             else return 1;
         } else {
@@ -179,6 +181,7 @@
     const bool can_split = d->allow_split && plain && d->K >= 512 && (d->N % 4 == 0);
     GemmPlan best; best.cfg = 0; best.tiles_m = cdiv(d->M, 128); best.tiles_n = cdiv(d->N, 128); best.splits = 1;
     best.kps = cdiv(d->K, BK) * BK;
+    if (d->epi == MDVIT_EPI_LN_BWD && d->N != 128) { best.cfg = 1; best.tiles_m = cdiv(d->M, 256); best.tiles_n = cdiv(d->N, 64); }
     static const bool conv_rule = [] { const char* e = getenv("MDVIT_CONV_SPLIT_PLAN"); return !(e && e[0] == '0'); }();
     if (conv_rule && g_force_cfg < 0 && g_force_splits == 0 && d->conv_c > 0 && d->conv_up <= 1 && d->conv_stride == 1 && !d->trans_a && can_split && d->K >= 2304 && !d->rc_a) {
         const long tiles = (long)cdiv(d->M, 128) * cdiv(d->N, 128);
@@ -191,8 +194,9 @@
     }
     double best_cost = 1e300;
     for (int c = 0; c < 3; ++c) {
-        if (g_force_cfg >= 0 && c != g_force_cfg && !d->rc_a) continue;
+        if (g_force_cfg >= 0 && c != g_force_cfg && !d->rc_a && d->epi != MDVIT_EPI_LN_BWD) continue;
         if (d->rc_a && c != 2) continue;
+        if (d->epi == MDVIT_EPI_LN_BWD && BNs[c] != d->N) continue;
         const long tm = cdiv(d->M, BMs[c]), tn = cdiv(d->N, BNs[c]);
         const long tiles = tm * tn;
         for (int si = 0; si < (int)(sizeof(SPLITS) / sizeof(int)); ++si) {
@@ -204,7 +208,7 @@
             const long wgs = tiles * splits;
             const long slots = 256L * OCC[c];
             const double rounds = wgs <= slots ? 1.0 : (double)wgs / (double)slots;
-            const bool loads_epi = (d->epi == MDVIT_EPI_DGELU && !d->rc_a) || d->residual != nullptr;
+            const bool loads_epi = ((d->epi == MDVIT_EPI_DGELU && !d->rc_a) || d->residual != nullptr) && d->epi != MDVIT_EPI_LN_BWD;
             const double epi_cycles = (loads_epi && c != 2 ? 30.0 : 6.0) * BMs[c] * BNs[c] / 64.0;
             const double wg_cycles = d->precision == 1
                 ? 0.0015 * BMs[c] * BNs[c] * (double)kps + (d->trans_a ? 0.12 : 0.06) * (BMs[c] + BNs[c]) * (double)kps + 800.0 + epi_cycles
@@ -369,6 +373,14 @@
                         (!d->rc_bias || aligned16(d->rc_bias)), MDVIT_E_ALIGN, "gemm: rc operands must be 16-byte aligned, leading dimensions %% 4 == 0, rc_k %% 32 == 0");
     }
     MDVIT_CHECK_ARG(!(d->e_drop_p > 0.f) || (long)d->M * d->N < (1L << 32), MDVIT_E_SHAPE, "gemm: dropout index space exceeds 2^32");
+    if (d->epi == MDVIT_EPI_LN_BWD) {
+        MDVIT_CHECK_ARG(!d->trans_a && d->trans_b && d->precision == 1 && (d->N == 64 || d->N == 128) && !d->bias && !(d->e_drop_p > 0.f) && !d->e_rowscale && !d->accumulate &&
+                        d->conv_c <= 0 && g_groups.n == 0 && !d->rc_a && !d->gelu_u && !d->C2, MDVIT_E_SHAPE,
+                        "gemm: the LayerNorm-backward epilogue is built for the NT bf16x3 product with N = 64 / 128 and no other epilogue operand (N=%d)", d->N);
+        MDVIT_CHECK_ARG(d->ln_x && d->ln_mean && d->ln_rstd && d->ln_gamma, MDVIT_E_SHAPE, "gemm: the LayerNorm-backward epilogue needs ln_x / ln_mean / ln_rstd / ln_gamma");
+        MDVIT_CHECK_ARG(aligned16(d->ln_x) && d->ln_ldx % 4 == 0 && aligned16(d->ln_gamma) && (!d->ln_part || aligned16(d->ln_part)), MDVIT_E_ALIGN,
+                        "gemm: ln_x / ln_gamma / ln_part must be 16-byte aligned, ln_ldx %% 4 == 0");
+    }
 
     GemmArgs a;
     memset(&a, 0, sizeof(a));
@@ -381,6 +393,7 @@
     a.e_rowscale = d->e_rowscale; a.e_rows_per_scale = d->e_rows_per_scale > 0 ? d->e_rows_per_scale : 1;
     a.residual = d->residual; a.ldr = d->ldr; a.gelu_u = d->gelu_u; a.ldu = d->ldu;
     a.rc_a = d->rc_a; a.rc_lda = d->rc_lda; a.rc_b = d->rc_b; a.rc_ldb = d->rc_ldb; a.rc_bias = d->rc_bias; a.rc_k = d->rc_k;
+    if (d->epi == MDVIT_EPI_LN_BWD) { a.ln_x = d->ln_x; a.ln_ldx = d->ln_ldx; a.ln_mean = d->ln_mean; a.ln_rstd = d->ln_rstd; a.ln_gamma = d->ln_gamma; a.ln_part = d->ln_part; }
     a.accumulate = d->accumulate;
     a.colsum = d->colsum_a;
     MDVIT_CHECK_ARG(!d->colsum_a || (d->trans_a && !d->trans_b), MDVIT_E_SHAPE, "gemm: colsum_a rides on the TN (wgrad) layout only");
@@ -422,8 +435,10 @@
     int epi = EPI_PLAIN;
     if (d->epi == MDVIT_EPI_GELU_DUAL) epi = EPI_GELU2;
     else if (d->epi == MDVIT_EPI_DGELU) epi = d->rc_a ? EPI_DGELU_RC : EPI_DGELU;
+    else if (d->epi == MDVIT_EPI_LN_BWD) epi = EPI_LNBWD;
     else if (a.e_drop || d->e_rowscale || d->residual) epi = EPI_FULL;
     a.vec = ((d->N & 3) == 0) && ((d->ldc & 3) == 0) && aligned16(d->C);
+    MDVIT_CHECK_ARG(epi != EPI_LNBWD || (pl.tiles_n == 1 && pl.splits == 1 && (pl.cfg == 0 ? 128 : 64) == d->N), MDVIT_E_SHAPE, "gemm: the LayerNorm-backward epilogue needs one tile across the row in one K range");
     if (epi != EPI_PLAIN) {
         MDVIT_CHECK_ARG(a.vec && (!d->bias || aligned16(d->bias)) && (!d->C2 || aligned16(d->C2)) &&
                         (!d->residual || (aligned16(d->residual) && d->ldr % 4 == 0)) && (!d->gelu_u || (aligned16(d->gelu_u) && d->ldu % 4 == 0)),
@@ -652,6 +667,7 @@
     int epi = EPI_PLAIN;
     if (d->epi == MDVIT_EPI_GELU_DUAL) epi = EPI_GELU2;
     else if (d->epi == MDVIT_EPI_DGELU) epi = d->rc_a ? EPI_DGELU_RC : EPI_DGELU;
+    else if (d->epi == MDVIT_EPI_LN_BWD) epi = EPI_LNBWD;
     else if (drop || d->e_rowscale || d->residual) epi = EPI_FULL;
     const int bm = pl.cfg == 0 ? 128 : (pl.cfg == 1 ? 256 : 64), bn = pl.cfg == 0 ? 128 : 64;
     if (d->conv_c > 0) {
@@ -661,6 +677,11 @@
     snprintf(out, cap, "gemm_f32_kernel<%d, %d, %s, %s, %s, %d, %s>%s", bm, bn, pl.cfg == 1 ? "4, 1" : "2, 2", d->trans_a ? "true" : "false",
              d->trans_b ? "true" : "false", epi, d->precision ? "true" : "false", pl.splits > 1 ? "+splitk_reduce" : "");
     return MDVIT_OK;
+}
+
+extern "C" int32_t mdvit_gemm_ln_bwd_rows(const MdvitGemmDesc* d) {
+    if (d == nullptr || d->M <= 0 || d->K <= 0 || d->epi != MDVIT_EPI_LN_BWD || (d->N != 64 && d->N != 128)) return 0;
+    return plan_gemm(d).tiles_m;
 }
 
 extern "C" size_t mdvit_gemm_ws_bytes(const MdvitGemmDesc* d) {
diff --git a/mdvit_amd/csrc/gemm_body.inc b/mdvit_amd/csrc/gemm_body.inc
--- a/mdvit_amd/csrc/gemm_body.inc
+++ b/mdvit_amd/csrc/gemm_body.inc
@@ -454,6 +454,108 @@
             if (m0 + i < p.M) atomicAdd(&p.colsum[m0 + i], s_cs[i]);
     }
 
+    if constexpr (EPI == EPI_LNBWD) {
+        constexpr int WCOLS = BN / WAVES_N, CSLD = WCOLS + 4;
+        constexpr int RS_FLOATS = WAVES_N * BM * 2, CS_FLOATS = (NTHREADS / 64) * 32 * CSLD, PT_FLOATS = WAVES_M * 2 * BN;
+        static_assert(RS_FLOATS + CS_FLOATS + PT_FLOATS <= (DB ? 2 : 1) * SMEM_FLOATS, "LNBWD: the epilogue's LDS must fit the staging buffers");
+        float* s_rs = smem;
+        float* s_cs = smem + RS_FLOATS + wave * 32 * CSLD;
+        float* s_pt = smem + RS_FLOATS + CS_FLOATS;
+        const bool parts = p.ln_part != nullptr, use_res = p.residual != nullptr;
+        const float* res_p = use_res ? p.residual : gB;
+        const int wv_n = wave % WAVES_N, wv_m = wave / WAVES_N;
+        float cg = 0.f, cb = 0.f;
+#pragma unroll
+        for (int i = 0; i < WTM; ++i) {
+            const int rt = wm0 + i * 32 + l31, row = m0 + rt;
+            const bool row_ok = row < p.M;
+            const long rc = min(row, p.M - 1);
+            const float mu = p.ln_mean[rc], rs = p.ln_rstd[rc];
+            float4 xh[WTN][4], rq[WTN][4];
+#pragma unroll
+            for (int j = 0; j < WTN; ++j)
+#pragma unroll
+                for (int q = 0; q < 4; ++q) {
+                    const int col = n0 + wn0 + j * 32 + 8 * q + 4 * lhi;
+                    xh[j][q] = *reinterpret_cast<const float4*>(p.ln_x + rc * p.ln_ldx + col);
+                    rq[j][q] = *reinterpret_cast<const float4*>(res_p + (use_res ? rc * p.ldr + col : 0L));
+                }
+#pragma unroll
+            for (int j = 0; j < WTN; ++j)
+#pragma unroll
+                for (int q = 0; q < 4; ++q) {
+                    const float4 x4 = xh[j][q];
+                    xh[j][q] = make_float4((x4.x - mu) * rs, (x4.y - mu) * rs, (x4.z - mu) * rs, (x4.w - mu) * rs);
+                    if (!row_ok) { acc[i][j][4 * q + 0] = 0.f; acc[i][j][4 * q + 1] = 0.f; acc[i][j][4 * q + 2] = 0.f; acc[i][j][4 * q + 3] = 0.f; }
+                }
+            if (parts) {
+#pragma unroll
+                for (int pass = 0; pass < 2; ++pass) {
+#pragma unroll
+                    for (int j = 0; j < WTN; ++j)
+#pragma unroll
+                        for (int q = 0; q < 4; ++q) {
+                            float4 v = make_float4(acc[i][j][4 * q + 0], acc[i][j][4 * q + 1], acc[i][j][4 * q + 2], acc[i][j][4 * q + 3]);
+                            if (pass == 0) { v.x *= xh[j][q].x; v.y *= xh[j][q].y; v.z *= xh[j][q].z; v.w *= xh[j][q].w; }
+                            *reinterpret_cast<float4*>(&s_cs[l31 * CSLD + j * 32 + 8 * q + 4 * lhi]) = v;
+                        }
+                    __syncthreads();
+                    if (lane < WCOLS) {
+                        float sacc = 0.f;
+#pragma unroll 8
+                        for (int r = 0; r < 32; ++r) sacc += s_cs[r * CSLD + lane];
+                        if (pass == 0) cg += sacc; else cb += sacc;
+                    }
+                    __syncthreads();
+                }
+            }
+            float s1 = 0.f, s2 = 0.f;
+#pragma unroll
+            for (int j = 0; j < WTN; ++j)
+#pragma unroll
+                for (int q = 0; q < 4; ++q) {
+                    const int col = n0 + wn0 + j * 32 + 8 * q + 4 * lhi;
+                    const float4 ga = *reinterpret_cast<const float4*>(p.ln_gamma + col);
+                    const float4 d4 = make_float4(acc[i][j][4 * q + 0] * ga.x, acc[i][j][4 * q + 1] * ga.y, acc[i][j][4 * q + 2] * ga.z, acc[i][j][4 * q + 3] * ga.w);
+                    acc[i][j][4 * q + 0] = d4.x; acc[i][j][4 * q + 1] = d4.y; acc[i][j][4 * q + 2] = d4.z; acc[i][j][4 * q + 3] = d4.w;
+                    s1 += (d4.x + d4.y) + (d4.z + d4.w);
+                    s2 += (d4.x * xh[j][q].x + d4.y * xh[j][q].y) + (d4.z * xh[j][q].z + d4.w * xh[j][q].w);
+                }
+            s1 += __shfl_xor(s1, 32, 64);
+            s2 += __shfl_xor(s2, 32, 64);
+            if (WAVES_N > 1) {
+                if (lhi == 0) { s_rs[(wv_n * BM + rt) * 2 + 0] = s1; s_rs[(wv_n * BM + rt) * 2 + 1] = s2; }
+                __syncthreads();
+                s1 = 0.f; s2 = 0.f;
+#pragma unroll
+                for (int w = 0; w < WAVES_N; ++w) { s1 += s_rs[(w * BM + rt) * 2 + 0]; s2 += s_rs[(w * BM + rt) * 2 + 1]; }
+            }
+            const float c1 = s1 * (1.0f / BN), c2 = s2 * (1.0f / BN);
+#pragma unroll
+            for (int j = 0; j < WTN; ++j)
+#pragma unroll
+                for (int q = 0; q < 4; ++q) {
+                    const int col = n0 + wn0 + j * 32 + 8 * q + 4 * lhi;
+                    const float4 h4 = xh[j][q];
+                    float4 o = make_float4(rs * (acc[i][j][4 * q + 0] - c1 - h4.x * c2), rs * (acc[i][j][4 * q + 1] - c1 - h4.y * c2),
+                                           rs * (acc[i][j][4 * q + 2] - c1 - h4.z * c2), rs * (acc[i][j][4 * q + 3] - c1 - h4.w * c2));
+                    if (use_res) { o.x += rq[j][q].x; o.y += rq[j][q].y; o.z += rq[j][q].z; o.w += rq[j][q].w; }
+                    if (row_ok) *reinterpret_cast<float4*>(gC + (long)row * p.ldc + col) = o;
+                }
+            __builtin_amdgcn_sched_barrier(0);
+        }
+        if (parts) {
+            if (lane < WCOLS) { s_pt[wv_m * 2 * BN + wn0 + lane] = cg; s_pt[wv_m * 2 * BN + BN + wn0 + lane] = cb; }
+            __syncthreads();
+            for (int c = tid; c < 2 * BN; c += NTHREADS) {
+                float v = 0.f;
+#pragma unroll
+                for (int w = 0; w < WAVES_M; ++w) v += s_pt[w * 2 * BN + c];
+                p.ln_part[(long)tm * 2 * BN + c] = v;
+            }
+        }
+        return;
+    }
     const bool split = (EPI == EPI_PLAIN) && p.splits > 1;
     float* slab = split ? p.slab + (long)blockIdx.y * p.M * p.N : nullptr;
     if (EPI == EPI_PLAIN && !split && !p.vec) {
diff --git a/mdvit_amd/ops.py b/mdvit_amd/ops.py
--- a/mdvit_amd/ops.py
+++ b/mdvit_amd/ops.py
@@ -3,6 +3,7 @@
 import ctypes as C
 import itertools
 import os
+import types
 import weakref
 from typing import Optional, Tuple
 
@@ -822,6 +823,10 @@
 
     @staticmethod
     def backward(ctx, g):
+        return _linear_backward(ctx, g)
+
+
+def _linear_backward(ctx, g):
         if g is None:
             return (None,) * 7
         x, W, rowscale = ctx.saved_tensors
@@ -847,7 +852,9 @@
             wsp, wsb, _keep = _partials_ws(N, g.device) if sums else (None, 0, None)
             call("mdvit_colsum_f32", _p(g), N, _p(sb if sunk else db) if sums else None, _p(gm) if masked else None, wsp, wsb, M, N,
                  drop_p, key[0], key[1], _p(rowscale), rps, int(sunk), _seed_ptr() if drop_p > 0 else None, _stream())
-        if ctx.needs_input_grad[0]:
+        if getattr(ctx, "dgrad", None) is not None:
+            dx = ctx.dgrad(gm)
+        elif ctx.needs_input_grad[0]:
             dx = _empty_like(x)
             _dgrad(gm, W, dx, M, K, N, ldb, allow_split=True)
         if want_w:
@@ -1345,6 +1352,69 @@
         return dx, dg, db, None, None
 
 
+class _LnLinear(torch.autograd.Function):
+
+    @staticmethod
+    def forward(ctx, x, gamma, beta, eps, W, b):
+        ctx.set_materialize_grads(False)
+        _chk(x, gamma, beta, b)
+        M, Cn = x.shape
+        N = W.shape[0]
+        cur = _empty_like(x)
+        mean = _empty((M,), device=x.device, dtype=torch.float32)
+        rstd = _empty_like(mean)
+        call("mdvit_layernorm_fwd", _p(x), _p(gamma), _p(beta), _p(cur), _p(mean), _p(rstd), M, Cn, 1, eps, _stream())
+        y = _empty((M, N), device=x.device, dtype=torch.float32)
+        if _lin_rc_ok(M, N, Cn):
+            _linear_rc(cur, W, False, b, y, M, N, Cn)
+        elif _plane_ok(M, N, Cn, False):
+            gemm_nt(cur, W, y, M, N, Cn, bias=b, allow_split=True)
+        else:
+            gemm(_p(cur), _p(W), _p(y), M, N, Cn, lda=Cn, ldb=Cn, ldc=N, bias=_p(b), allow_split=True)
+        ctx.save_for_backward(x, gamma, mean, rstd, cur, W)
+        ctx.has_b = b is not None
+        ctx.bias_ref = b if (b is not None and b.grad_fn is None) else None
+        return y, x.view_as(x)
+
+    @staticmethod
+    def backward(ctx, g, g_pass=None):
+        if g is None:
+            return g_pass, None, None, None, None, None
+        x, gamma, mean, rstd, cur, W = ctx.saved_tensors
+        M, Cn = x.shape
+        ln = {}
+
+        def dgrad(gm):
+            dx = _empty_like(x)
+            gp = None if g_pass is None else _c(g_pass)
+            dg, db = (None, None) if _dgrad_only else _flat_like(gamma, gamma)
+            wsb = _lib.load().mdvit_qkv_ln_bwd_ws_bytes(M, Cn, int(dg is not None))
+            ws = _empty(((wsb + 3) // 4,), device=x.device, dtype=torch.float32)
+            Wt = wt(W)
+            call("mdvit_qkv_ln_bwd", _p(gm), _p(Wt), _p(x), _p(mean), _p(rstd), _p(gamma), _p(gp), _p(dx), _p(dg), _p(db), _p(ws), wsb, M, Cn, 0, _stream())
+            del Wt
+            ln["dg"], ln["db"] = dg, db
+            return dx
+
+        shim = types.SimpleNamespace(saved_tensors=(cur, W, None), meta=(0.0, (0, 0), 1, ctx.has_b, False), bias_ref=ctx.bias_ref,
+                                     needs_input_grad=(True, ctx.needs_input_grad[4], ctx.needs_input_grad[5]), dgrad=dgrad)
+        dx, dW, dbias = _linear_backward(shim, g)[:3]
+        return dx, ln.get("dg"), ln.get("db"), None, dW, dbias
+
+
+def ln_linear_ok(x, gamma, W) -> bool:
+    Cn = x.shape[-1]
+    M = x.numel() // Cn
+    return (x.is_cuda and _gemm_precision == 1 and Cn in (64, 128) and gamma.dim() == 1 and tuple(W.shape) == (3 * Cn, Cn) and W.is_contiguous()
+            and not _plane_ok(M, Cn, 3 * Cn, False, plain=True))
+
+
+def ln_linear_fork(x, gamma, beta, W, b, eps=1e-6):
+    shp = x.shape
+    y, xr = _LnLinear.apply(_c(x).view(-1, shp[-1]), _c(gamma), _c(beta), float(eps), W, b)
+    return y.view(*shp[:-1], W.shape[0]), xr.view(shp)
+
+
 def layer_norm(x, gamma, beta, eps=1e-6):
     shp = x.shape
     return _LayerNorm.apply(_c(x).view(-1, shp[-1]), _c(gamma), _c(beta), float(eps), False).view(shp)
```

Result: no change. 519.9 images/s (median of 6 runs) (+0.2%).
